# eth-cscs/conflux

Measured on NVIDIA H100. Metric: LU GFLOP/s (FP64, (2/3)N^3), higher is better.
Workload: dtype f64

## Files before the change

conflux_b200/__init__.py:

```python
import ctypes

import numpy as np

from ._lib import ConfluxError, LIB_PATH, SYMBOLS, ShareLayout, check, lib

__all__ = ["pinned_empty", "pinned_free", "Comm", "lu_params", "LU_rep", "LU_rep_fixed", "rbt_multipliers", "LU_rep_rbt", "lu_rbt_solve", "lu_rbt_apply_local", "residual", "validate", "lu_solve", "lu_rcond", "lu_refine", "lu_refine_x", "lu_equilibrate", "lu_svx", "lu_equilibrate_b", "lu_svxx", "lu_inverse", "lu_det", "rhs_local_cols", "lu_solve_local", "timeline", "auto_grid", "lu_dims", "init_matrix_host", "ConfluxError", "dbg", "cholesky", "chol_dims", "chol_auto_grid"]


def auto_grid(M, N, P):
    px, py, pz = ctypes.c_int(), ctypes.c_int(), ctypes.c_int()
    check(lib().cflx_auto_grid(int(M), int(N), int(P), ctypes.byref(px), ctypes.byref(py), ctypes.byref(pz)), "auto_grid")
    return px.value, py.value, pz.value


def lu_dims(M, N, v, Px, Py, Pz):
    o = (ctypes.c_int * 8)()
    check(lib().cflx_lu_dims(int(M), int(N), int(v), int(Px), int(Py), int(Pz), o), "lu_dims")
    return dict(M=o[0], N=o[1], Ml=o[2], Nl=o[3], Nt=o[4], nlayr=o[5], Mt=o[6], P=o[7])


def init_matrix_host(M, N, v, Px, Py, Pz, rank, seed=42, out=None):
    d = lu_dims(M, N, v, Px, Py, Pz)
    if out is None:
        out = np.empty((d["Ml"], d["Nl"]), dtype=np.float64)
# ... 540 lines not shown
            self.finalize()
        except Exception:
            pass


def chol_dims(N, v, Px, Py, Pz):
    o = (ctypes.c_int * 6)()
    check(lib().cflx_chol_dims(int(N), int(v), int(Px), int(Py), int(Pz), o), "chol_dims")
    return dict(N=o[0], Kappa=o[1], Ml=o[2], Nl=o[3], l=o[4], P=o[5])


def chol_auto_grid(P, N):
    g = (ctypes.c_int * 3)()
    check(lib().cflx_chol_auto_grid(int(P), int(N), g), "chol_auto_grid")
    return tuple(g)


def _ptr(a):
    return a.ctypes.data if a is not None else None


def _tiles(n, v):
    return int(n) // max(int(v), 1)


def _share(v, Ml, Nl, grid=(1, 1), pos=(0, 0), Kappa=None, M=None):
    Px, Py = (int(x) for x in grid)
    M = int(M) if M is not None else _tiles(Ml, v) * Px * int(v)
    return ShareLayout(M, int(v), int(Kappa if Kappa is not None else 1 << 30), int(Ml), int(Nl), Px, Py, int(pos[0]),
                       int(pos[1]))


class dbg:

    @staticmethod
    def gemm_tn(AT, B, C=None, alpha=1.0, beta=0.0, reps=1):
        AT = np.asarray(AT, dtype=np.float64)
        B = np.asarray(B, dtype=np.float64)
        K, M = AT.shape
        N = B.shape[1]
        M2, N2 = M + (M & 1), N + (N & 1)
        ATp = np.zeros((K, M2))
        ATp[:, :M] = AT
        Bp = np.zeros((K, N2))
        Bp[:, :N] = B
        Cp = np.zeros((M, N2))
        if C is not None:
            Cp[:, :N] = C
        D, _, ms = dbg.gemm_tn_window(ATp, Bp, Cp, M, N2, K, alpha, beta, in_place=False, reps=reps)
        return D[:, :N], ms

    @staticmethod
    def gemm_tn_window(AT, B, C, M, N, K, alpha=1.0, beta=0.0, at_off=(0, 0), b_off=(0, 0), c_off=(0, 0), in_place=True,
                       reps=1):
        AT = np.ascontiguousarray(AT, dtype=np.float64)
        B = np.ascontiguousarray(B, dtype=np.float64)
        C = np.ascontiguousarray(C, dtype=np.float64)
        D = np.empty_like(C)
        Cout = D if in_place else np.empty_like(C)
        ms = ctypes.c_double()
        check(lib().cflx_dbg_gemm_tn(int(M), int(N), int(K), AT.ctypes.data, AT.shape[0], AT.shape[1],
                                     at_off[0] * AT.shape[1] + at_off[1], B.ctypes.data, B.shape[0], B.shape[1],
                                     b_off[0] * B.shape[1] + b_off[1], C.ctypes.data, C.shape[0], C.shape[1],
                                     int(c_off[0]), int(c_off[1]), float(alpha), float(beta), 1 if in_place else 0,
                                     D.ctypes.data, Cout.ctypes.data, int(reps), ctypes.byref(ms)), "dbg_gemm_tn")
        return D, Cout, ms.value

    @staticmethod
    def gemm_narrow(A, B, C=None, alpha=1.0, beta=0.0, reps=1, out=None):
        A = np.ascontiguousarray(A, dtype=np.float64)
        B = np.ascontiguousarray(B, dtype=np.float64)
        M, K = A.shape
        N = B.shape[1]
        Cp = None
        if C is not None:
            assert C.dtype == np.float64 and C.flags.c_contiguous and C.shape == (M, N)
            Cp = C.ctypes.data
        D = np.empty((M, N)) if out is None else out
        assert D.dtype == np.float64 and D.flags.c_contiguous and D.shape == (M, N)
        ms = ctypes.c_double()
        check(lib().cflx_dbg_gemm_narrow(M, N, K, A.ctypes.data, B.ctypes.data, Cp, float(alpha), float(beta), D.ctypes.data,
                                         int(reps), ctypes.byref(ms)), "dbg_gemm_narrow")
        return D, ms.value

    @staticmethod
    def gemm_narrow_tn(AT, B, C=None, alpha=1.0, beta=0.0, reps=1, out=None):
        AT = np.ascontiguousarray(AT, dtype=np.float64)
        B = np.ascontiguousarray(B, dtype=np.float64)
        K, M = AT.shape
        if B.ndim != 2 or B.shape[0] != K:
            raise ValueError(f"gemm_narrow_tn: B must have {K} rows, got shape {B.shape}")
        N = B.shape[1]
        Cp = None
        if C is not None:
            assert C.dtype == np.float64 and C.flags.c_contiguous and C.shape == (M, N)
            Cp = C.ctypes.data
        D = np.empty((M, N)) if out is None else out
        assert D.dtype == np.float64 and D.flags.c_contiguous and D.shape == (M, N)
        ms = ctypes.c_double()
        check(lib().cflx_dbg_gemm_narrow_tn(M, N, K, AT.ctypes.data, B.ctypes.data, Cp, float(alpha), float(beta),
                                            D.ctypes.data, int(reps), ctypes.byref(ms)), "dbg_gemm_narrow_tn")
        return D, ms.value

    @staticmethod
    def gemm_narrow_window(A, B, C, M, N, K, alpha=1.0, beta=0.0, a_off=(0, 0), b_off=(0, 0), c_off=(0, 0), trans=False,
                           in_place=True):
        A = np.ascontiguousarray(A, dtype=np.float64)
        B = np.ascontiguousarray(B, dtype=np.float64)
        C = np.ascontiguousarray(C, dtype=np.float64)
        D = np.empty_like(C)
        Cout = D if in_place else np.empty_like(C)
        check(lib().cflx_dbg_gemm_narrow_window(
            1 if trans else 0, int(M), int(N), int(K), A.ctypes.data, A.shape[0], A.shape[1], int(a_off[0]),
            int(a_off[1]), B.ctypes.data, B.shape[0], B.shape[1], int(b_off[0]), int(b_off[1]), C.ctypes.data,
            C.shape[0], C.shape[1], int(c_off[0]), int(c_off[1]), float(alpha), float(beta), 1 if in_place else 0,
            D.ctypes.data, Cout.ctypes.data), "dbg_gemm_narrow_window")
        return D, Cout
# ... 250 lines not shown
              "dbg_potrf_tile")
        return L, LT, info.value

    @staticmethod
    def ldlt_tile(A, tiny=0.0, variant=0):
        A = np.ascontiguousarray(A, dtype=np.float64)
        v = A.shape[0]
        R, SRT, sg = np.empty((v, v)), np.empty((v, v)), np.empty(v)
        nrepl, info = ctypes.c_int(), ctypes.c_int()
        inertia = (ctypes.c_int * 3)()
        check(lib().cflx_dbg_ldlt_tile(v, A.ctypes.data, float(tiny), R.ctypes.data, SRT.ctypes.data, sg.ctypes.data,
                                       ctypes.byref(nrepl), inertia, ctypes.byref(info), int(variant)), "dbg_ldlt_tile")
        return dict(R=R, SRT=SRT, s=sg, nrepl=nrepl.value, inertia=tuple(inertia), info=info.value)

    @staticmethod
    def solve_signs(Z, sgn, v, grid=(1, 1), pos=(0, 0), M=None):
        Z = np.array(Z, dtype=np.float64, order="C")
        sg = np.ascontiguousarray(sgn, dtype=np.float64)
        Nl, ldn = Z.shape
        lay = _share(v, v, Nl, grid, pos, M=M if M is not None else len(sg))
        check(lib().cflx_dbg_solve_signs(ctypes.byref(lay), int(ldn), sg.ctypes.data, Z.ctypes.data), "dbg_solve_signs")
        return Z

    @staticmethod
    def getrf_nopiv_tile(A, tiny=0.0, variant=0):
        A = np.ascontiguousarray(A, dtype=np.float64)
        v = A.shape[0]
        LU = np.empty((v, v))
        nrepl, info = ctypes.c_int(), ctypes.c_int()
        check(lib().cflx_dbg_getrf_nopiv_tile(v, A.ctypes.data, float(tiny), LU.ctypes.data, ctypes.byref(nrepl),
                                              ctypes.byref(info), int(variant)), "dbg_getrf_nopiv_tile")
        return LU, nrepl.value, info.value

    @staticmethod
    def ozaki_gemm(AT, B, C=None, reps=1, want_planes=False, row0=0, col0=0, max_ctas=0):
        AT = np.ascontiguousarray(AT, dtype=np.float64)
        B = np.ascontiguousarray(B, dtype=np.float64)
        K, Ma = AT.shape
        Nb = B.shape[1]
        M, N = Ma - row0, Nb - col0
        D = np.empty((M, N))
        Cp = np.ascontiguousarray(C, dtype=np.float64) if C is not None else None
        pa = np.zeros((8, Ma, K), dtype=np.int8) if want_planes else None
        pb = np.zeros((8, Nb, K), dtype=np.int8) if want_planes else None
        ea = np.zeros(Ma, dtype=np.int32) if want_planes else None
        eb = np.zeros(Nb, dtype=np.int32) if want_planes else None
        ms, sms = ctypes.c_double(), ctypes.c_double()
        check(lib().cflx_dbg_ozaki_gemm(M, N, K, int(row0), int(col0), int(max_ctas), AT.ctypes.data, B.ctypes.data,
                                        _ptr(Cp), D.ctypes.data, _ptr(pa), _ptr(pb), _ptr(ea), _ptr(eb), int(reps),
                                        ctypes.byref(ms), ctypes.byref(sms)), "dbg_ozaki_gemm")
        return dict(D=D, ms=ms.value, split_ms=sms.value, pa=pa, pb=pb, ea=ea, eb=eb)

    @staticmethod
    def push_pivots(A, pivot_rows, fnpr):
        A = np.array(A, dtype=np.float64, order="C")
        piv = np.ascontiguousarray(pivot_rows, dtype=np.int32)
        gri = np.zeros(A.shape[0], dtype=np.int32)
        a01 = np.zeros((max(1, len(piv)), A.shape[1]))
        check(lib().cflx_dbg_push_pivots(A.shape[0], A.shape[1], A.ctypes.data, len(piv), piv.ctypes.data, int(fnpr),
                                         gri.ctypes.data, a01.ctypes.data), "dbg_push_pivots")
        return A, gri, a01[:len(piv)]

    @staticmethod
    def wgmma_peak(n):
        t = ctypes.c_double()
        check(lib().cflx_dbg_wgmma_peak(int(n), ctypes.byref(t)), "dbg_wgmma_peak")
        return t.value

    @staticmethod
    def fp64_peak_ex(which):
        a, b = ctypes.c_double(), ctypes.c_double()
        check(lib().cflx_dbg_fp64_peak_ex(int(which), ctypes.byref(a), ctypes.byref(b)), "dbg_fp64_peak_ex")
        return a.value, b.value

    @staticmethod
    def fp64_peak(which):
        tf = ctypes.c_double()
        check(lib().cflx_dbg_fp64_peak(int(which), ctypes.byref(tf)), "dbg_fp64_peak")
        return tf.value
```

conflux_b200/_lib.py:

```python
import ctypes
import os

_HERE = os.path.dirname(os.path.abspath(__file__))
LIB_PATH = os.path.join(_HERE, "libconflux_b200.so")
_lib = None

c_double_p = ctypes.POINTER(ctypes.c_double)
c_int_p = ctypes.POINTER(ctypes.c_int)


class ConfluxError(RuntimeError):
    pass


class ShareLayout(ctypes.Structure):
    _fields_ = [(f, ctypes.c_int) for f in ("M", "v", "Kappa", "Ml", "Nl", "Px", "Py", "pi", "pj")]


SYMBOLS = [
    "cflx_last_error", "cflx_version", "cflx_device_count", "cflx_get_unique_id", "cflx_comm_create",
    "cflx_comm_barrier", "cflx_comm_destroy", "cflx_host_alloc", "cflx_host_free", "cflx_auto_grid", "cflx_lu_dims", "cflx_init_matrix_host",
    "cflx_lu_create", "cflx_lu_info", "cflx_lu_set_local", "cflx_lu_queue_next_local", "cflx_lu_factor", "cflx_lu_factor_fixed", "cflx_rbt_multipliers", "cflx_lu_rbt", "cflx_lu_rbt_solve", "cflx_lu_rbt_apply_local", "cflx_lu_get_factors",
    "cflx_lu_get_permutation", "cflx_lu_residual", "cflx_lu_validate", "cflx_lu_solve", "cflx_lu_solve_trans", "cflx_rhs_local_cols", "cflx_lu_solve_local", "cflx_lu_rcond", "cflx_lu_refine", "cflx_lu_refine_x", "cflx_lu_equilibrate", "cflx_lu_svx", "cflx_lu_equilibrate_b", "cflx_lu_svxx", "cflx_lu_inverse", "cflx_lu_det", "cflx_lu_launch_count", "cflx_lu_uses_ozaki", "cflx_lu_set_profiling", "cflx_lu_phase_ms", "cflx_lu_timeline",
    "cflx_lu_set_kernel_timing", "cflx_lu_trailing_stats", "cflx_lu_destroy", "cflx_chol_auto_grid", "cflx_chol_auto_tile", "cflx_chol_dims", "cflx_chol_init_matrix_host",
    "cflx_chol_create", "cflx_chol_info", "cflx_chol_set_local", "cflx_chol_factor", "cflx_chol_factor_ldlt", "cflx_chol_rbt", "cflx_chol_rbt_solve", "cflx_chol_rbt_apply_local", "cflx_chol_get_signs", "cflx_chol_get_input", "cflx_chol_get_local", "cflx_chol_validate",
    "cflx_chol_solve", "cflx_chol_solve_local", "cflx_chol_rcond", "cflx_chol_refine", "cflx_chol_refine_x", "cflx_chol_equilibrate", "cflx_chol_svx", "cflx_chol_equilibrate_b", "cflx_chol_svxx", "cflx_chol_inverse", "cflx_chol_det", "cflx_chol_launch_count", "cflx_chol_destroy", "cflx_dbg_gemm_tn", "cflx_dbg_gemm_narrow", "cflx_dbg_gemm_narrow_tn", "cflx_dbg_gemm_narrow_window", "cflx_dbg_diag_solve", "cflx_dbg_residual", "cflx_dbg_residual_x", "cflx_dbg_equil", "cflx_dbg_growth_cols", "cflx_dbg_inverse_share", "cflx_dbg_solve_local_share", "cflx_dbg_norm_share", "cflx_dbg_rbt_share", "cflx_dbg_chol_validate_share", "cflx_dbg_lu_validate_share", "cflx_dbg_chol_gather_cols", "cflx_dbg_refine_assemble", "cflx_dbg_refine_columns", "cflx_dbg_det", "cflx_dbg_panel", "cflx_dbg_trsm", "cflx_dbg_diag_inverse", "cflx_dbg_potrf_tile", "cflx_dbg_ldlt_tile", "cflx_dbg_solve_signs", "cflx_dbg_getrf_nopiv_tile", "cflx_dbg_push_pivots", "cflx_dbg_ozaki_gemm", "cflx_dbg_wgmma_peak", "cflx_dbg_fp64_peak", "cflx_dbg_fp64_peak_ex",
]


def _preload_nccl():
    import sys
    for d in sys.path:
        cand = os.path.join(d, "nvidia", "nccl", "lib", "libnccl.so.2")
        if os.path.exists(cand):
            try:
                ctypes.CDLL(cand, mode=ctypes.RTLD_GLOBAL)
                return cand
            except OSError:
                pass
    return None


def lib():
    global _lib
    if _lib is None:
        if not os.path.exists(LIB_PATH):
            raise ConfluxError(
                f"{LIB_PATH} is missing: build it with `python -c 'import __graft_entry__ as g; g.build()'` "
                "(conflux_b200 has no CPU fallback)")
        _preload_nccl()
        L = ctypes.CDLL(LIB_PATH)
        L.cflx_last_error.restype = ctypes.c_char_p
        L.cflx_version.restype = ctypes.c_char_p
        L.cflx_comm_destroy.restype = None
        L.cflx_lu_destroy.restype = None
        L.cflx_comm_destroy.argtypes = [ctypes.c_void_p]
        L.cflx_lu_destroy.argtypes = [ctypes.c_void_p]
        L.cflx_comm_barrier.argtypes = [ctypes.c_void_p]
        L.cflx_comm_create.argtypes = [ctypes.c_int, ctypes.c_int, ctypes.c_void_p, ctypes.c_int,
                                       ctypes.POINTER(ctypes.c_void_p)]
        L.cflx_lu_create.argtypes = [ctypes.c_void_p] + [ctypes.c_int] * 6 + [ctypes.POINTER(ctypes.c_void_p)]
        L.cflx_host_alloc.argtypes = [ctypes.c_size_t, ctypes.POINTER(ctypes.c_void_p)]
        L.cflx_host_free.argtypes = [ctypes.c_void_p]
        L.cflx_lu_info.argtypes = [ctypes.c_void_p, c_int_p]
        L.cflx_lu_set_local.argtypes = [ctypes.c_void_p, ctypes.c_void_p]
        L.cflx_lu_queue_next_local.argtypes = [ctypes.c_void_p, ctypes.c_void_p]
        L.cflx_lu_factor.argtypes = [ctypes.c_void_p, c_double_p]
        L.cflx_lu_factor_fixed.argtypes = [ctypes.c_void_p, ctypes.c_void_p, ctypes.c_double] + [ctypes.c_void_p] * 3
        L.cflx_rbt_multipliers.argtypes = [ctypes.c_int, ctypes.c_int, ctypes.c_uint64, ctypes.c_void_p, ctypes.c_void_p]
        L.cflx_lu_rbt.argtypes = [ctypes.c_void_p, ctypes.c_int, ctypes.c_uint64, ctypes.c_void_p, ctypes.c_void_p]
        L.cflx_lu_rbt_solve.argtypes = [ctypes.c_void_p, ctypes.c_int, ctypes.c_int, ctypes.c_void_p, ctypes.c_int,
                                        ctypes.c_void_p, ctypes.c_int, ctypes.c_int, ctypes.c_void_p, ctypes.c_void_p]
        L.cflx_lu_rbt_apply_local.argtypes = [ctypes.c_void_p, ctypes.c_int, ctypes.c_int, ctypes.c_void_p, ctypes.c_int]
        L.cflx_lu_get_factors.argtypes = [ctypes.c_void_p, ctypes.c_void_p, ctypes.c_void_p]
        L.cflx_lu_get_permutation.argtypes = [ctypes.c_void_p, ctypes.c_void_p]
        L.cflx_lu_residual.argtypes = [ctypes.c_void_p, c_double_p]
        L.cflx_lu_validate.argtypes = [ctypes.c_void_p, c_double_p, c_double_p]
        L.cflx_lu_solve.argtypes = [ctypes.c_void_p, ctypes.c_int, ctypes.c_void_p, ctypes.c_int, ctypes.c_void_p, ctypes.c_int]
        L.cflx_lu_solve_trans.argtypes = [ctypes.c_void_p, ctypes.c_int, ctypes.c_void_p, ctypes.c_int, ctypes.c_void_p,
# ... 10 lines not shown
        L.cflx_lu_svx.argtypes = [ctypes.c_void_p, ctypes.c_int, ctypes.c_int, ctypes.c_void_p, ctypes.c_int, ctypes.c_void_p,
                                  ctypes.c_int] + [ctypes.c_void_p] * 6
        L.cflx_lu_equilibrate_b.argtypes = [ctypes.c_void_p, ctypes.c_int] + [ctypes.c_void_p] * 7
        L.cflx_lu_svxx.argtypes = [ctypes.c_void_p, ctypes.c_int, ctypes.c_int, ctypes.c_void_p, ctypes.c_int,
                                   ctypes.c_void_p, ctypes.c_int] + [ctypes.c_void_p] * 7
        L.cflx_lu_inverse.argtypes = [ctypes.c_void_p, ctypes.c_void_p, c_int_p]
        L.cflx_lu_det.argtypes = [ctypes.c_void_p, ctypes.c_int] + [ctypes.c_void_p] * 5
        L.cflx_lu_uses_ozaki.argtypes = [ctypes.c_void_p]
        L.cflx_lu_launch_count.argtypes = [ctypes.c_void_p, ctypes.POINTER(ctypes.c_int64), ctypes.c_int]
        L.cflx_lu_set_profiling.argtypes = [ctypes.c_void_p, ctypes.c_int]
        L.cflx_lu_phase_ms.argtypes = [ctypes.c_void_p, c_double_p]
        L.cflx_lu_timeline.argtypes = [ctypes.c_void_p, ctypes.c_char_p, ctypes.c_int]
        L.cflx_lu_set_kernel_timing.argtypes = [ctypes.c_void_p, ctypes.c_int]
        L.cflx_lu_trailing_stats.argtypes = [ctypes.c_void_p, c_double_p, c_double_p]
        L.cflx_chol_destroy.restype = None
        L.cflx_chol_destroy.argtypes = [ctypes.c_void_p]
        L.cflx_chol_auto_grid.argtypes = [ctypes.c_int, ctypes.c_int, c_int_p]
        L.cflx_chol_auto_tile.argtypes = [ctypes.c_int] * 3
        L.cflx_chol_dims.argtypes = [ctypes.c_int] * 5 + [c_int_p]
        L.cflx_chol_init_matrix_host.argtypes = [ctypes.c_int] * 6 + [ctypes.c_void_p]
        L.cflx_chol_create.argtypes = [ctypes.c_void_p] + [ctypes.c_int] * 5 + [ctypes.POINTER(ctypes.c_void_p)]
        L.cflx_chol_info.argtypes = [ctypes.c_void_p, c_int_p]
        L.cflx_chol_set_local.argtypes = [ctypes.c_void_p, ctypes.c_void_p]
        L.cflx_chol_factor.argtypes = [ctypes.c_void_p, c_double_p]
        L.cflx_chol_factor_ldlt.argtypes = [ctypes.c_void_p, ctypes.c_double] + [ctypes.c_void_p] * 4
        L.cflx_chol_rbt.argtypes = [ctypes.c_void_p, ctypes.c_int, ctypes.c_uint64, ctypes.c_void_p]
        L.cflx_chol_rbt_solve.argtypes = [ctypes.c_void_p, ctypes.c_int, ctypes.c_void_p, ctypes.c_int, ctypes.c_void_p,
                                          ctypes.c_int, ctypes.c_int, ctypes.c_void_p, ctypes.c_void_p]
        L.cflx_chol_rbt_apply_local.argtypes = [ctypes.c_void_p, ctypes.c_int, ctypes.c_int, ctypes.c_void_p, ctypes.c_int]
        L.cflx_chol_get_signs.argtypes = [ctypes.c_void_p, ctypes.c_void_p]
        L.cflx_chol_get_input.argtypes = [ctypes.c_void_p, ctypes.c_void_p]
        L.cflx_chol_get_local.argtypes = [ctypes.c_void_p, ctypes.c_void_p]
        L.cflx_chol_validate.argtypes = [ctypes.c_void_p, c_double_p, c_double_p]
        L.cflx_chol_solve.argtypes = [ctypes.c_void_p, ctypes.c_int, ctypes.c_void_p, ctypes.c_int, ctypes.c_void_p, ctypes.c_int]
        L.cflx_chol_solve_local.argtypes = [ctypes.c_void_p, ctypes.c_int, ctypes.c_void_p, ctypes.c_int, ctypes.c_void_p,
                                            ctypes.c_int]
        L.cflx_chol_rcond.argtypes = [ctypes.c_void_p, c_double_p, c_double_p]
        L.cflx_chol_refine.argtypes = [ctypes.c_void_p, ctypes.c_int, ctypes.c_void_p, ctypes.c_int, ctypes.c_void_p, ctypes.c_int,
                                       ctypes.c_void_p, ctypes.c_void_p]
        L.cflx_chol_refine_x.argtypes = [ctypes.c_void_p, ctypes.c_int, ctypes.c_void_p, ctypes.c_int, ctypes.c_void_p,
                                         ctypes.c_int] + [ctypes.c_void_p] * 5
        L.cflx_chol_equilibrate.argtypes = [ctypes.c_void_p, ctypes.c_int] + [ctypes.c_void_p] * 5
        L.cflx_chol_svx.argtypes = [ctypes.c_void_p, ctypes.c_int, ctypes.c_void_p, ctypes.c_int, ctypes.c_void_p, ctypes.c_int
                                    ] + [ctypes.c_void_p] * 5
        L.cflx_chol_equilibrate_b.argtypes = [ctypes.c_void_p, ctypes.c_int] + [ctypes.c_void_p] * 5
        L.cflx_chol_svxx.argtypes = [ctypes.c_void_p, ctypes.c_int, ctypes.c_void_p, ctypes.c_int, ctypes.c_void_p,
                                     ctypes.c_int] + [ctypes.c_void_p] * 7
        L.cflx_chol_inverse.argtypes = [ctypes.c_void_p, ctypes.c_void_p]
        L.cflx_chol_det.argtypes = [ctypes.c_void_p, ctypes.c_int] + [ctypes.c_void_p] * 3
        L.cflx_chol_launch_count.argtypes = [ctypes.c_void_p, ctypes.POINTER(ctypes.c_int64), ctypes.c_int]
        L.cflx_init_matrix_host.argtypes = [ctypes.c_int] * 8 + [ctypes.c_void_p]
        _buf = [ctypes.c_void_p, ctypes.c_int, ctypes.c_int64]
        L.cflx_dbg_gemm_tn.argtypes = [ctypes.c_int] * 3 + _buf + [ctypes.c_int64] + _buf + [ctypes.c_int64] + _buf + [
            ctypes.c_int] * 2 + [ctypes.c_double] * 2 + [ctypes.c_int, ctypes.c_void_p, ctypes.c_void_p, ctypes.c_int,
                                                          c_double_p]
        L.cflx_dbg_gemm_narrow.argtypes = [ctypes.c_int] * 3 + [ctypes.c_void_p] * 3 + [ctypes.c_double] * 2 + [
            ctypes.c_void_p, ctypes.c_int, c_double_p]
        L.cflx_dbg_gemm_narrow_tn.argtypes = [ctypes.c_int] * 3 + [ctypes.c_void_p] * 3 + [ctypes.c_double] * 2 + [
            ctypes.c_void_p, ctypes.c_int, c_double_p]
        _blk = [ctypes.c_void_p, ctypes.c_int, ctypes.c_int64, ctypes.c_int, ctypes.c_int]
        L.cflx_dbg_gemm_narrow_window.argtypes = [ctypes.c_int] * 4 + _blk * 3 + [ctypes.c_double] * 2 + [
            ctypes.c_int, ctypes.c_void_p, ctypes.c_void_p]
        L.cflx_dbg_diag_solve.argtypes = [ctypes.c_int] * 4 + [ctypes.c_void_p, ctypes.c_int, ctypes.c_int64] + [
            ctypes.c_int] * 3 + [ctypes.c_void_p] * 3
        share = ctypes.POINTER(ShareLayout)
        L.cflx_dbg_residual.argtypes = [ctypes.c_int, share, ctypes.c_void_p, ctypes.c_int] + [ctypes.c_void_p] * 4 + [
            ctypes.c_int, c_double_p]
        L.cflx_dbg_residual_x.argtypes = [ctypes.c_int, share, ctypes.c_void_p, ctypes.c_int] + [
            ctypes.c_void_p] * 6 + [ctypes.c_int, c_double_p]
        L.cflx_dbg_equil.argtypes = [share] + [ctypes.c_void_p] * 3 + [ctypes.c_char, ctypes.c_int] + [
            ctypes.c_void_p] * 7
        L.cflx_dbg_growth_cols.argtypes = [ctypes.c_int, share, ctypes.c_int] + [ctypes.c_void_p] * 4
        L.cflx_dbg_inverse_share.argtypes = [ctypes.c_int, share] + [ctypes.c_int] * 3 + [
            ctypes.c_void_p, ctypes.c_int] + [ctypes.c_void_p] * 3 + [ctypes.c_int]
        L.cflx_dbg_solve_local_share.argtypes = [ctypes.c_int, share] + [ctypes.c_int] * 3 + [
            ctypes.c_void_p, ctypes.c_int] + [ctypes.c_void_p] * 3 + [ctypes.c_int]
        L.cflx_dbg_norm_share.argtypes = [ctypes.c_int, share] + [ctypes.c_void_p] * 2
        L.cflx_dbg_rbt_share.argtypes = [ctypes.c_int, share, ctypes.c_int] + [ctypes.c_void_p] * 2 + [
            ctypes.c_int, ctypes.c_void_p, ctypes.c_int]
        L.cflx_dbg_chol_validate_share.argtypes = [share, ctypes.c_void_p, ctypes.c_int] + [ctypes.c_void_p] * 2
        L.cflx_dbg_lu_validate_share.argtypes = [share, ctypes.c_void_p, ctypes.c_int] + [ctypes.c_void_p] * 2
        L.cflx_dbg_chol_gather_cols.argtypes = [share, ctypes.c_int] + [ctypes.c_void_p] * 2
        L.cflx_dbg_refine_assemble.argtypes = [ctypes.c_int] * 12 + [ctypes.c_void_p] * 6
        L.cflx_dbg_refine_columns.argtypes = [ctypes.c_int] * 3 + [ctypes.c_void_p] * 10
        L.cflx_dbg_det.argtypes = [ctypes.c_int] + [ctypes.c_void_p] * 3 + [ctypes.c_int] + [ctypes.c_void_p] * 5
        L.cflx_dbg_panel.argtypes = [ctypes.c_int, ctypes.c_int] + [ctypes.c_void_p] * 4 + [ctypes.c_int, c_double_p]
        L.cflx_dbg_trsm.argtypes = [ctypes.c_int] * 3 + [ctypes.c_int64] + [ctypes.c_void_p] * 5
        L.cflx_dbg_diag_inverse.argtypes = [ctypes.c_int, ctypes.c_int] + [ctypes.c_void_p] * 3
        L.cflx_dbg_potrf_tile.argtypes = [ctypes.c_int] + [ctypes.c_void_p] * 4 + [ctypes.c_int]
        L.cflx_dbg_solve_signs.argtypes = [share, ctypes.c_int, ctypes.c_void_p, ctypes.c_void_p]
        L.cflx_dbg_ldlt_tile.argtypes = ([ctypes.c_int, ctypes.c_void_p, ctypes.c_double] + [ctypes.c_void_p] * 6 +
                                         [ctypes.c_int])
        L.cflx_dbg_getrf_nopiv_tile.argtypes = [ctypes.c_int, ctypes.c_void_p, ctypes.c_double] + [ctypes.c_void_p] * 3 + [
            ctypes.c_int]
        L.cflx_dbg_push_pivots.argtypes = [ctypes.c_int, ctypes.c_int, ctypes.c_void_p, ctypes.c_int, ctypes.c_void_p, ctypes.c_int,
                                           ctypes.c_void_p, ctypes.c_void_p]
        L.cflx_dbg_ozaki_gemm.argtypes = [ctypes.c_int] * 6 + [ctypes.c_void_p] * 8 + [ctypes.c_int, c_double_p, c_double_p]
        L.cflx_dbg_wgmma_peak.argtypes = [ctypes.c_int, c_double_p]
        L.cflx_dbg_fp64_peak.argtypes = [ctypes.c_int, c_double_p]
        L.cflx_dbg_fp64_peak_ex.argtypes = [ctypes.c_int, c_double_p, c_double_p]
        _lib = L
    return _lib


def check(rc, what=""):
    if rc != 0:
        msg = lib().cflx_last_error().decode(errors="replace")
        raise ConfluxError(f"{what} failed with status {rc}: {msg}")
```

conflux_b200/csrc/chol.cu:

```cuda
#include <climits>
#include <cmath>
#include <cstdlib>
#include <cstring>
#include <numeric>

#include "lu_state.h"

using namespace cflx;

struct cflx_chol : Handle {
    DevBuf<double> PT, LT, G , Bc , D, A00, W, Uinv, LinvT, acc;
    DevBuf<double> Q;
    DevBuf<int> info;
    int64_t ldp = 0, ldb = 0;
    bool ldlt = false;
    double tiny = 0.0;
    DevBuf<double> sgn;
    Events<2> ev_col, ev_panel;
    SubComm j_comm;
    ~cflx_chol();
};

namespace {

// ... 352 lines not shown
                                      (size_t)v * sizeof(double), cudaMemcpyDeviceToDevice, s));
    } else {
        CFLX_CUDA(cudaMemcpyAsync(G, ch->LT, (size_t)v * piece_ld(ch, gfirst, 0) * sizeof(double), cudaMemcpyDeviceToDevice, s));
    }
    const int lj0 = first_local_tile(jmin, ch->pj, Py);
    const int ntc = Nl / v - lj0;
    if (ntc <= 0) return CFLX_OK;
    CFLX_TRY(launch_gather_cols(G, piece_stride, Bc, ch->ldb, v, Px, Py, ch->pj, lj0, ntc, gfirst, Ml, s,
                                ch->ldlt ? ch->sgn + (int64_t)t * v : nullptr));
    ch->launches++;
    return CFLX_OK;
}
static int chol_leave_sms() {
    static int leave = -1;
    if (leave < 0) {
        const char* e = getenv("CFLX_CHOL_LEAVE");
        leave = e ? atoi(e) : 8;
        if (leave < 0) leave = 0;
        if (leave > 100) leave = 100;
    }
    return leave;
}

int update_columns(cflx_chol* ch, int gfirst, int jmin, int buf, double* X, int lj_lo, int lj_hi, cudaStream_t s, int planes_buf = -1) {
    const int v = ch->v, Px = ch->Px, Py = ch->Py, Ml = ch->Ml, Nl = ch->Nl;
    const int pi = ch->pi, pj = ch->pj, pk = ch->pk;
    const int64_t piece_stride = (int64_t)v * ch->ldp;
    const double* G = ch->G + (int64_t)buf * Px * piece_stride;
    const double* Bc = ch->Bc + (int64_t)buf * v * ch->ldb;
    const int lj0 = first_local_tile(jmin, pj, Py);
    const int my_first = first_local_tile(gfirst, pi, Px);
    const int64_t ldg = piece_ld(ch, gfirst, pi);
    const int lj_end = std::min(lj_hi, Nl / v);
    const int my_rows = Ml - my_first * v;
    for (int lj = std::max(lj_lo, lj0); lj < lj_end;) {
        const int j = lj * Py + pj;
        const int li = first_local_tile(j, pi, Px);
        const int M = Ml - li * v;
        if (M <= 0) break;
        int gcols = std::max(1, (8192 + M - 1) / M);
        gcols = std::min(gcols, lj_end - lj);
        GemmArgs g{};
        g.M = M; g.N = gcols * v; g.K = ch->nlayr;
        g.AT = G + (int64_t)pi * piece_stride + (int64_t)pk * ch->nlayr * ldg + (int64_t)(li - my_first) * v;
        g.ldat = ldg;
        g.B = Bc + (int64_t)pk * ch->nlayr * ch->ldb + (int64_t)(lj - lj0) * v;
        g.ldb = ch->ldb;
        g.C = X + (int64_t)li * v * Nl + (int64_t)lj * v;
        g.ldc = Nl;
        g.D = const_cast<double*>(g.C);
        g.ldd = Nl;
        g.alpha = -1.0; g.beta = 1.0;
        if (ch->use_ozaki && planes_buf == buf)
            CFLX_TRY(launch_ozaki_gemm(&ch->oz, M, g.N, (li - my_first) * v, (lj - lj0) * v, g.D, Nl, ch->oz.sms - chol_leave_sms(), s));
        else
            CFLX_TRY(launch_gemm_tn(g, s));
        ch->launches++;
        lj += gcols;
    }
    (void)my_rows;
    return CFLX_OK;
}
int split_planes(cflx_chol* ch, int gfirst, int jmin, int buf, cudaStream_t s);
int split_planes(cflx_chol* ch, int gfirst, int jmin, int buf, cudaStream_t s) {
    if (!ch->use_ozaki) return CFLX_OK;
    const int v = ch->v, Px = ch->Px;
    const int64_t piece_stride = (int64_t)v * ch->ldp;
    const double* G = ch->G + (int64_t)buf * Px * piece_stride;
    const double* Bc = ch->Bc + (int64_t)buf * v * ch->ldb;
    const int my_first = first_local_tile(gfirst, ch->pi, Px);
    const int rows = ch->Ml - my_first * v;
    const int ncols = ch->Nl - first_local_tile(jmin, ch->pj, ch->Py) * v;
    const int64_t ldg = piece_ld(ch, gfirst, ch->pi);
    if (rows > 0) CFLX_TRY(ozaki_split_a(&ch->oz, G + (int64_t)ch->pi * piece_stride + (int64_t)ch->pk * ch->nlayr * ldg, ldg, rows, s));
    if (ncols > 0) CFLX_TRY(ozaki_split_b(&ch->oz, Bc + (int64_t)ch->pk * ch->nlayr * ch->ldb, ch->ldb, 0, ncols, s));
    ch->launches += 2;
    return CFLX_OK;
}
int broadcast_and_update(cflx_chol* ch, int t, int jmin, bool below_only, double* X, cudaStream_t s) {
    const int gfirst = below_only ? t + 1 : t;
    CFLX_TRY(broadcast_pieces(ch, t, gfirst, jmin, 0, s));
    return update_columns(ch, gfirst, jmin, 0, X, 0, ch->Nl / ch->v, s);
}

size_t potrf_tile_smem(int v) { return ((size_t)PB * (PB + 1) + (size_t)v * (PB + 1)) * sizeof(double); }
}

namespace cflx {
size_t potrf_tile_scratch(int v) { return (v % QBK == 0 && v >= 2 * QBK) ? (size_t)3 * QBK * QBK + (size_t)2 * QBK * v : 0; }

int potrf_setup(int v) {
    static PerDeviceMax tile_cfg, blk_cfg;
    CFLX_CUDA(tile_cfg.raise(potrf_tile_smem(v), [&] {
        cudaError_t e = cudaFuncSetAttribute(potrf_tile_kernel<false>, cudaFuncAttributeMaxDynamicSharedMemorySize, (int)potrf_tile_smem(v));
        if (e == cudaSuccess)
            e = cudaFuncSetAttribute(potrf_tile_kernel<true>, cudaFuncAttributeMaxDynamicSharedMemorySize, (int)potrf_tile_smem(v));
        return e;
    }));
    CFLX_CUDA(blk_cfg.raise(QBK * QPITCH * sizeof(double), [&] {
        cudaError_t e = cudaFuncSetAttribute(potrf128_kernel<false>, cudaFuncAttributeMaxDynamicSharedMemorySize, (int)(QBK * QPITCH * sizeof(double)));
        if (e == cudaSuccess)
            e = cudaFuncSetAttribute(potrf128_kernel<true>, cudaFuncAttributeMaxDynamicSharedMemorySize, (int)(QBK * QPITCH * sizeof(double)));
        return e;
    }));
    return CFLX_OK;
}

// ... 796 lines not shown
```

conflux_b200/csrc/dbg.cu:

```cuda
#include <algorithm>
#include <climits>
#include <limits>
#include <vector>

#include "../../include/conflux_b200.h"
#include "common.cuh"
#include "kernels.h"
#include "lu_state.h"

using namespace cflx;

namespace {
int check_device() {
    int n = 0;
    if (cudaGetDeviceCount(&n) != cudaSuccess || n == 0) {
        cudaGetLastError();
        set_last_error("no CUDA device visible: conflux_b200 has no CPU fallback");
        return CFLX_ERR_NO_DEVICE;
    }
    return CFLX_OK;
}

enum : unsigned { TILED = 1, COVERED = 2, NONEMPTY = 4 };

// ... 136 lines not shown

int cflx_dbg_fp64_peak_ex(int which, double* burst_out, double* sustained_out) {
    CFLX_TRY(check_device());
    if (which == 0) which = 3;
    if (which < 1 || which > 5) {
        set_last_error("fp64_peak: unknown probe %d", which);
        return CFLX_ERR_ARG;
    }
    int dev = 0, sms = 0;
    CFLX_CUDA(cudaGetDevice(&dev));
    CFLX_CUDA(cudaDeviceGetAttribute(&sms, cudaDevAttrMultiProcessorCount, dev));
    const int threads = 256, blocks = sms * 4;
    DevBuf<> out;
    CFLX_TRY(out.alloc(sizeof(double) * threads * blocks));
    Events<2> ev;
    CFLX_TRY(ev.create());
    const double per_warp_instr = which == 2 ? 1024.0 : which == 3 ? 2048.0 : which == 4 ? 4096.0 : 512.0;
    const int shrink = which == 1 ? 1 : (int)(per_warp_instr / 512.0);
    auto run = [&](int iters, double* tf) -> int {
        iters /= shrink;
        CFLX_CUDA(cudaEventRecord(ev[0]));
        switch (which) {
            case 1: dfma_peak_kernel<<<blocks, threads>>>(out.as<double>(), iters); break;
            case 2: dmma16x8_peak_kernel<4><<<blocks, threads>>>(out.as<double>(), iters); break;
            case 3: dmma16x8_peak_kernel<8><<<blocks, threads>>>(out.as<double>(), iters); break;
            case 4: dmma16x8_peak_kernel<16><<<blocks, threads>>>(out.as<double>(), iters); break;
            default: dmma_peak_kernel<<<blocks, threads>>>(out.as<double>(), iters); break;
        }
        CFLX_CUDA(cudaGetLastError());
        CFLX_CUDA(cudaEventRecord(ev[1]));
        CFLX_CUDA(cudaEventSynchronize(ev[1]));
        float ms = 0;
        CFLX_CUDA(cudaEventElapsedTime(&ms, ev[0], ev[1]));
        const double flop = which == 1 ? (double)blocks * threads * iters * 16 * 2.0
                                       : (double)blocks * (threads / 32) * iters * 16 * per_warp_instr;
        *tf = flop / (ms * 1e-3) / 1e12;
        return CFLX_OK;
    };
    double burst = 0, tf = 0;
    for (int rep = 0; rep < 4; ++rep) {
        CFLX_TRY(run(1024, &tf));
        if (rep > 0 && tf > burst) burst = tf;
    }
    double sustained = 0;
    CFLX_TRY(run(262144, &sustained));
    if (burst_out) *burst_out = burst;
    if (sustained_out) *sustained_out = sustained;
    return CFLX_OK;
}
int cflx_dbg_fp64_peak(int which, double* tflops_out) { return cflx_dbg_fp64_peak_ex(which, tflops_out, nullptr); }

int cflx_dbg_gemm_tn(int M, int N, int K, const double* AT, int at_rows, int64_t ldat, int64_t at_off, const double* B,
                     int b_rows, int64_t ldb, int64_t b_off, const double* C, int c_rows, int64_t ldc, int row_off,
                     int col_off, double alpha, double beta, int in_place, double* D_out, double* C_out, int reps,
                     double* ms_out) {
    CFLX_TRY(check_device());
    REFUSE_IF(M <= 0 || N <= 0 || K <= 0);
    REFUSE_IF(!AT || !B || !C);
    REFUSE_IF(at_rows <= 0 || b_rows <= 0 || c_rows <= 0 || ldat <= 0 || ldb <= 0 || ldc <= 0);
    REFUSE_IF(at_off < 0 || b_off < 0 || row_off < 0 || col_off < 0);
    if ((at_off & 1) || (b_off & 1) || (col_off & 1) || at_off + (K - 1) * ldat + round_up(M, 2) > (int64_t)at_rows * ldat ||
        b_off + (K - 1) * ldb + N > (int64_t)b_rows * ldb || row_off + M > c_rows || col_off + N > ldc)
        return refuse(__func__, "window outside the buffers or misaligned");
    const size_t a_n = (size_t)at_rows * ldat, b_n = (size_t)b_rows * ldb, c_n = (size_t)c_rows * ldc;
    DevBuf<> dA, dB, dC, dC0, dD;
    CFLX_TRY(stage(dA, a_n, AT));
    CFLX_TRY(stage(dB, b_n, B));
    CFLX_TRY(stage(dC, c_n));
    CFLX_TRY(stage(dC0, c_n, C));
    CFLX_TRY(stage(dD, c_n));
    auto restore = [&]() -> int {
        CFLX_CUDA(cudaMemcpy(dC.p, dC0.p, sizeof(double) * c_n, cudaMemcpyDeviceToDevice));
        CFLX_CUDA(cudaMemcpy(dD.p, dC0.p, sizeof(double) * c_n, cudaMemcpyDeviceToDevice));
        return CFLX_OK;
    };
    const int64_t c_at = (int64_t)row_off * ldc + col_off;
    GemmArgs g{};
    g.M = M; g.N = N; g.K = K;
    g.AT = dA.as<double>() + at_off; g.ldat = ldat;
    g.B = dB.as<double>() + b_off; g.ldb = ldb;
    g.C = dC.as<double>() + c_at; g.ldc = ldc;
    g.D = (in_place ? dC.as<double>() : dD.as<double>()) + c_at; g.ldd = ldc;
    g.alpha = alpha; g.beta = beta;
    CFLX_TRY(restore());
    CFLX_TRY(time_reps([&] { return launch_gemm_tn(g, 0); }, reps, ms_out));
    CFLX_TRY(restore());
    CFLX_TRY(launch_gemm_tn(g, 0));
    CFLX_TRY(fetch(D_out, in_place ? dC.p : dD.p, c_n));
    CFLX_TRY(fetch(C_out, dC.p, c_n));
    CFLX_CUDA(cudaDeviceSynchronize());
    return CFLX_OK;
}

int cflx_dbg_gemm_narrow(int M, int N, int K, const double* A, const double* B, const double* C, double alpha, double beta,
                         double* D, int reps, double* ms_out) {
    CFLX_TRY(check_device());
    REFUSE_IF(M <= 0 || N <= 0 || K < 0);
    REFUSE_IF(K & 3);
    REFUSE_IF(!A || !B);
    DevBuf<> dA, dB;
    CFLX_TRY(stage(dA, (size_t)M * K, A));
    CFLX_TRY(stage(dB, (size_t)K * N, B));
    return narrow_gemm((size_t)M * N, C, D, reps, ms_out, [&](const double* c, double* out) {
        return launch_gemm_narrow(M, N, K, dA.as<double>(), K, dB.as<double>(), N, c, N, out, N, alpha, beta, 0);
    });
}

int cflx_dbg_gemm_narrow_tn(int M, int N, int K, const double* AT, const double* B, const double* C, double alpha,
                            double beta, double* D, int reps, double* ms_out) {
    CFLX_TRY(check_device());
    REFUSE_IF(M <= 0 || N <= 0 || K < 0);
    REFUSE_IF(!AT || !B);
    const int64_t ldat = round_up(M, 2);
    DevBuf<> dA, dB;
    CFLX_TRY(stage(dA, K * ldat));
    CFLX_TRY(stage(dB, (size_t)K * N, B));
    if (K > 0) CFLX_CUDA(cudaMemcpy2D(dA.p, ldat * 8, AT, (size_t)M * 8, (size_t)M * 8, K, cudaMemcpyHostToDevice));
    return narrow_gemm((size_t)M * N, C, D, reps, ms_out, [&](const double* c, double* out) {
        return launch_gemm_narrow_tn(M, N, K, dA.as<double>(), ldat, dB.as<double>(), N, c, N, out, N, alpha, beta, 0);
    });
}

int cflx_dbg_gemm_narrow_window(int trans, int M, int N, int K, const double* A, int a_rows, int64_t lda, int a_row,
                                int a_col, const double* B, int b_rows, int64_t ldb, int b_row, int b_col, const double* C,
                                int c_rows, int64_t ldc, int c_row, int c_col, double alpha, double beta, int in_place,
                                double* D_out, double* C_out) {
    CFLX_TRY(check_device());
    const char* who = __func__;
    if (M < 1 || N < 1 || K < 0) return refuse(who, "M < 1, N < 1 or K < 0");
    if (!A || !B || !C) return refuse(who, "A, B or C is null");
    if (a_rows < 1 || b_rows < 1 || c_rows < 1 || lda < 1 || ldb < 1 || ldc < 1)
        return refuse(who, "a buffer with no rows or a leading dimension < 1");
    if (a_row < 0 || a_col < 0 || b_row < 0 || b_col < 0 || c_row < 0 || c_col < 0) return refuse(who, "negative offset");
    if (!trans && (K & 3)) return refuse(who, "K not a multiple of 4");
// ... 687 lines not shown
    CFLX_CUDA(cudaDeviceSynchronize());
    if (nrepl_out) *nrepl_out = cnt[0];
    if (inertia_out)
        for (int i = 0; i < 3; ++i) inertia_out[i] = cnt[1 + i];
    return CFLX_OK;
}

int cflx_dbg_getrf_nopiv_tile(int v, const double* A, double tiny, double* LU_out, int* nrepl_out, int* info_out,
                              int variant) {
    CFLX_TRY(check_device());
    REFUSE_IF(!A || !LU_out || !info_out);
    REFUSE_IF(variant != 0 && variant != 1);
    REFUSE_IF(v < 4 || v > 1024 || v % 4 != 0);
    REFUSE_IF(variant == 1 && !getrf_nopiv_blocked(v));
    REFUSE_IF(!(tiny >= 0.0));
    const size_t vv = (size_t)v * v;
    std::vector<double> At(vv);
    for (int i = 0; i < v; ++i)
        for (int c = 0; c < v; ++c) At[(size_t)c * v + i] = A[(size_t)i * v + c];
    DevBuf<> dB, dA, drec, dws;
    CFLX_TRY(stage(dB, vv, At.data()));
    CFLX_TRY(stage(dA, vv));
    CFLX_TRY(stage<int>(drec, 4));
    const size_t ws = getrf_nopiv_scratch(v, variant == 1);
    if (ws) CFLX_TRY(stage(dws, ws));
    CFLX_CUDA(cudaMemset(drec.p, 0, 4 * sizeof(int)));
    if (variant == 1) CFLX_TRY(gemm_tn_setup());
    int64_t launches = 0;
    CFLX_TRY(launch_getrf_nopiv_tile(dB.as<double>(), v, tiny, dA.as<double>(), nullptr, nullptr, nullptr, drec.as<int>(),
                                     0, variant == 1, ws ? dws.as<double>() : nullptr, 0, &launches));
    int rec[4];
    CFLX_TRY(fetch(LU_out, dA.p, vv));
    CFLX_TRY(fetch(rec, drec.p, 4));
    CFLX_CUDA(cudaDeviceSynchronize());
    if (nrepl_out) *nrepl_out = rec[0];
    *info_out = rec[1];
    return CFLX_OK;
}

int cflx_dbg_push_pivots(int n_rows, int n_cols, double* A_inout, int npiv, const int* pivot_rows, int fnpr, int* gri_out,
                         double* a01_out) {
    CFLX_TRY(check_device());
    REFUSE_IF(n_rows <= 0 || n_cols <= 0 || (n_cols & 1));
    REFUSE_IF(npiv < 0 || fnpr < 0 || npiv > n_rows - fnpr);
    if (npiv == 0) {
        if (gri_out) for (int i = 0; i < n_rows; ++i) gri_out[i] = i;
        return CFLX_OK;
    }
    REFUSE_IF(!A_inout || !pivot_rows);
    const int v = npiv;
    const size_t a_n = (size_t)n_rows * n_cols;
    DevBuf<> dA, dtmp, da01, dplan, dgp, dgri, dgrit, digri;
    CFLX_TRY(stage(dA, a_n, A_inout));
    CFLX_TRY(stage(dtmp, (size_t)v * n_cols));
    CFLX_TRY(stage(da01, (size_t)v * n_cols));
    CFLX_TRY(stage<int>(dplan, 6 * (size_t)v + 8 + n_rows));
    CFLX_TRY(stage(dgp, v, pivot_rows));
    CFLX_TRY(stage<int>(dgri, n_rows));
    CFLX_TRY(stage<int>(dgrit, n_rows));
    CFLX_TRY(stage<int>(digri, n_rows));
    MovePlan plan{};
    int* pm = dplan.as<int>();
    plan.npiv = pm; plan.nel = pm + 4; pm += 8;
    plan.cur_piv = pm; pm += v;
    plan.order = pm; pm += v;
    plan.slot2piv = pm; pm += v;
    plan.early = pm; pm += v;
    plan.late = pm; pm += 2 * v;
    plan.rowsrc = pm;
    CFLX_TRY(launch_iota_gri(dgri.as<int>(), digri.as<int>(), n_rows, n_rows, 1, 0, 0));
    CFLX_TRY(launch_plan_moves(dgp.as<int>(), v, 1, 0, fnpr, n_rows, digri.as<int>(), plan, 0));
    CFLX_TRY(launch_push_phase1(dA.as<double>(), n_cols, n_cols, 0, plan, v, dtmp.as<double>(), da01.as<double>(), n_cols, 0, 0));
    CFLX_TRY(launch_push_phase2(dA.as<double>(), n_cols, n_cols, 0, plan, v, 0));
    CFLX_TRY(launch_push_phase3(dA.as<double>(), n_cols, n_cols, 0, fnpr, plan, v, dtmp.as<double>(), 0));
    CFLX_TRY(launch_update_gri(dgri.as<int>(), dgrit.as<int>(), digri.as<int>(), plan.rowsrc, fnpr, n_rows, n_rows, 1, 0));
    CFLX_TRY(fetch(A_inout, dA.p, a_n));
    CFLX_TRY(fetch(gri_out, dgri.p, n_rows));
    CFLX_TRY(fetch(a01_out, da01.p, (size_t)v * n_cols));
    CFLX_CUDA(cudaDeviceSynchronize());
    return CFLX_OK;
}

int cflx_dbg_ozaki_gemm(int M, int N, int K, int row0, int col0, int max_ctas, const double* AT, const double* B,
                        const double* C, double* D, signed char* planesA_out, signed char* planesB_out, int* ea_out,
                        int* eb_out, int reps, double* ms_out, double* split_ms_out) {
    CFLX_TRY(check_device());
    REFUSE_IF(M <= 0 || N <= 0 || K <= 0 || (N & 1));
    REFUSE_IF(row0 < 0 || col0 < 0 || max_ctas < 0);
    REFUSE_IF(!AT || !B);
    const int Ma = row0 + M, Nb = col0 + N;
    const int64_t ldat = round_up(Ma, 2), ldb = Nb, ldc = N;
    const size_t c_n = (size_t)M * ldc;
    DevBuf<> dA, dB, dC, dC0;
    CFLX_TRY(stage(dA, K * ldat));
    CFLX_TRY(stage(dB, K * ldb, B));
    CFLX_TRY(stage(dC, c_n));
    CFLX_TRY(stage(dC0, c_n, C));
    CFLX_CUDA(cudaMemset(dA.p, 0, sizeof(double) * K * ldat));
    CFLX_CUDA(cudaMemcpy2D(dA.p, ldat * 8, AT, (size_t)Ma * 8, (size_t)Ma * 8, K, cudaMemcpyHostToDevice));
    if (!C) CFLX_CUDA(cudaMemset(dC0.p, 0, sizeof(double) * c_n));
    Events<3> ev;
    CFLX_TRY(ev.create());
    OzakiWorkspace ws;
    int rc = ozaki_workspace_create(&ws, Ma, Nb, K);
    if (reps < 1) reps = 1;
    float ms = 0, ms_split = 0;
    for (int r = 0; r < reps + 1 && rc == CFLX_OK; ++r) {
        cudaMemcpyAsync(dC.p, dC0.p, sizeof(double) * c_n, cudaMemcpyDeviceToDevice, 0);
        cudaEventRecord(ev[0]);
        rc = ozaki_split_a(&ws, dA.as<double>(), ldat, Ma, 0);
        if (!rc && col0 > 0) rc = ozaki_split_b(&ws, dB.as<double>(), ldb, 0, col0, 0);
        if (!rc) rc = ozaki_split_b(&ws, dB.as<double>(), ldb, col0, N, 0);
        cudaEventRecord(ev[1]);
        if (!rc) rc = launch_ozaki_gemm(&ws, M, N, row0, col0, dC.as<double>(), ldc, max_ctas, 0);
        cudaEventRecord(ev[2]);
        if (cudaEventSynchronize(ev[2]) != cudaSuccess) {
            set_last_error("ozaki kernel failed: %s", cudaGetErrorString(cudaGetLastError()));
            rc = CFLX_ERR_CUDA;
        }
        float a = 0, b = 0;
        cudaEventElapsedTime(&a, ev[0], ev[1]);
        cudaEventElapsedTime(&b, ev[1], ev[2]);
        if (r > 0) {
            ms_split += a;
            ms += b;
        }
    }
    if (rc == CFLX_OK) rc = fetch(D, dC.p, c_n);
    for (int s = 0; s < 8 && rc == CFLX_OK; ++s) {
        if (planesA_out) rc = fetch(planesA_out + (size_t)s * Ma * K, ws.planesA + (size_t)s * ws.cap_a * K, (size_t)Ma * K);
        if (planesB_out && rc == CFLX_OK)
            rc = fetch(planesB_out + (size_t)s * Nb * K, ws.planesB + (size_t)s * ws.cap_b * K, (size_t)Nb * K);
    }
    if (rc == CFLX_OK) rc = fetch(ea_out, ws.ea, Ma);
    if (rc == CFLX_OK) rc = fetch(eb_out, ws.eb, Nb);
    if (rc == CFLX_OK && cudaDeviceSynchronize() != cudaSuccess) rc = CFLX_ERR_CUDA;
    if (ms_out) *ms_out = ms / reps;
    if (split_ms_out) *split_ms_out = ms_split / reps;
    return rc;
}

int cflx_dbg_wgmma_peak(int n, double* tmacs_out) {
    CFLX_TRY(check_device());
    REFUSE_IF(!tmacs_out);
    return wgmma_peak_probe(n, tmacs_out);
}

}
```

conflux_b200/csrc/gemm.cu:

```cuda
#include <cstdlib>

#include "common.cuh"
#include "kernels.h"

namespace cflx {

namespace {
constexpr int BK = 16, STAGES = 4;

template <int WM, int WN>
struct Cfg {
    static constexpr int BM = 64 * WM, BN = 32 * WN;
    static constexpr int LDA = BM + 4, LDB = BN + 4;
    static constexpr int NCONS = WM * WN, NTHREADS = (NCONS + 1) * 32;
    static constexpr bool STAGE_C = (WM == 2);
    static constexpr int NBAR = 2 * STAGES + (STAGE_C ? WM * STAGES : 0);
    static constexpr size_t SMEM = (size_t)STAGES * BK * (LDA + LDB) * sizeof(double) + NBAR * sizeof(uint64_t);
    static_assert(!STAGE_C || (LDA == LDB && 64 / 16 == STAGES), "one slab per warp row and stage, in both parts");
};

__device__ __forceinline__ double2 ld_c2(const double* p) {
    double2 v;
    asm("ld.global.v2.f64 {%0, %1}, [%2];" : "=d"(v.x), "=d"(v.y) : "l"(p));
    return v;
}

template <int LDA, int LDB, int SA, int SB>
__device__ __forceinline__ void load_operands(const GemmArgs& g, int kt0, int kt1, int m0, int n0, int wm, int wn,
                                              double* a_ring, double* b_ring, uint64_t* full, uint64_t* empty, int lane) {
    const int rr = lane & 15;
    for (int kt = kt0; kt < kt1; ++kt) {
        const int s = kt % STAGES, u = kt / STAGES;
        if (u > 0) mbar_wait(&empty[s], (u - 1) & 1);
        const int rows = min(BK, g.K - kt * BK);
        if (lane == 0) mbar_arrive_expect_tx(&full[s], (uint32_t)(rows * (wm + wn) * sizeof(double)));
        __syncwarp();
        if (rr < rows) {
            const int64_t k = (int64_t)kt * BK + rr;
            if (lane < 16)
                bulk_g2s(a_ring + s * SA + rr * LDA, g.AT + k * g.ldat + m0, (uint32_t)(wm * sizeof(double)), &full[s]);
            else
                bulk_g2s(b_ring + s * SB + rr * LDB, g.B + k * g.ldb + n0, (uint32_t)(wn * sizeof(double)), &full[s]);
        }
    }
}

template <int MI, int LDA, int LDB, int SA, int SB>
__device__ __forceinline__ int mma_loop(const GemmArgs& g, double (&acc)[MI][4][4], const double* a_ring,
                                        const double* b_ring, uint64_t* full, uint64_t* empty, int wm_off, int wn_off,
                                        int lane) {
    const int g4 = lane >> 2, t4 = lane & 3;
#pragma unroll
    for (int i = 0; i < MI; ++i)
#pragma unroll
        for (int j = 0; j < 4; ++j) acc[i][j][0] = acc[i][j][1] = acc[i][j][2] = acc[i][j][3] = 0.0;

    int kt = 0;
    for (; kt * BK < g.K; ++kt) {
        const int s = kt % STAGES, u = kt / STAGES;
        mbar_wait(&full[s], u & 1);
        const double* a_s = a_ring + s * SA + wm_off + g4;
        const double* b_s = b_ring + s * SB + wn_off + g4;
        const int rows = min(BK, g.K - kt * BK);
#pragma unroll
        for (int kk = 0; kk < BK; kk += 8) {
            if (kk < rows) {
                const bool hi = kk + 4 < rows;
                const double* a_k = a_s + (kk + t4) * LDA;
                const double* b_k = b_s + (kk + t4) * LDB;
                double b[4][2];
#pragma unroll
                for (int j = 0; j < 4; ++j) {
                    b[j][0] = b_k[8 * j];
                    b[j][1] = hi ? b_k[4 * LDB + 8 * j] : 0.0;
                }
#pragma unroll
                for (int i = 0; i < MI; ++i) {
                    const double a[4] = {a_k[16 * i], a_k[16 * i + 8], hi ? a_k[4 * LDA + 16 * i] : 0.0,
                                         hi ? a_k[4 * LDA + 16 * i + 8] : 0.0};
#pragma unroll
                    for (int j = 0; j < 4; ++j) dmma16x8x8(acc[i][j], a, b[j]);
                }
            }
        }
        __syncwarp();
        if (lane == 0) mbar_arrive(&empty[s]);
    }
    return kt;
}

template <int WM, int WN, int MINB>
__global__ void __launch_bounds__(Cfg<WM, WN>::NTHREADS, MINB) gemm_tn_kernel(GemmArgs g) {
    using C = Cfg<WM, WN>;
    constexpr int BM = C::BM, BN = C::BN, LDA = C::LDA, LDB = C::LDB, NCONS = C::NCONS;
    extern __shared__ __align__(128) unsigned char smem_raw[];
    double* sA = reinterpret_cast<double*>(smem_raw);
    double* sB = sA + STAGES * BK * LDA;
    uint64_t* full = reinterpret_cast<uint64_t*>(sB + STAGES * BK * LDB);
    uint64_t* empty = full + STAGES;
    uint64_t* cfull = empty + STAGES;

    const int warp = threadIdx.x >> 5, lane = threadIdx.x & 31;
    const int m0 = blockIdx.y * BM, n0 = blockIdx.x * BN;

    if (threadIdx.x == 0) {
        for (int s = 0; s < STAGES; ++s) {
            mbar_init(&full[s], 1);
            mbar_init(&empty[s], NCONS);
        }
        if constexpr (C::STAGE_C)
            for (int b = 0; b < WM * STAGES; ++b) mbar_init(&cfull[b], 1);
        fence_barrier_init();
    }
    __syncthreads();

    if (warp == NCONS) {
        int wm = g.M - m0;
        wm = wm > BM ? BM : ((wm + 1) & ~1);
        int wn = g.N - n0;
        wn = wn > BN ? BN : ((wn + 1) & ~1);
        const int rr = lane & 15;
        const int nkt = (g.K + BK - 1) / BK;
        const bool use_c = (g.beta != 0.0);
        for (int kt = 0; kt < nkt; ++kt) {
            const int s = kt % STAGES, u = kt / STAGES;
            if (u > 0) mbar_wait(&empty[s], (u - 1) & 1);
            const int rows = min(BK, g.K - kt * BK);
            if (lane == 0) mbar_arrive_expect_tx(&full[s], (uint32_t)(rows * (wm + wn) * sizeof(double)));
            __syncwarp();
            if (rr < rows) {
                const int64_t k = (int64_t)kt * BK + rr;
                if (lane < 16)
                    bulk_g2s(sA + (s * BK + rr) * LDA, g.AT + k * g.ldat + m0, (uint32_t)(wm * sizeof(double)), &full[s]);
                else
                    bulk_g2s(sB + (s * BK + rr) * LDB, g.B + k * g.ldb + n0, (uint32_t)(wn * sizeof(double)), &full[s]);
            }
        }
        if constexpr (C::STAGE_C) {
            if (use_c)
                for (int i = 0; i < STAGES; ++i) {
                    const int s = (nkt + i) % STAGES, kt = nkt + i - STAGES;
                    if (kt >= 0) mbar_wait(&empty[s], (kt / STAGES) & 1);
                    const int wr = lane >> 4, r0 = m0 + 64 * wr + 16 * i;
                    const int rows = max(0, min(16, g.M - r0));
                    uint64_t* bar = &cfull[wr * STAGES + i];
                    if (rr == 0) mbar_arrive_expect_tx(bar, (uint32_t)(rows * wn * sizeof(double)));
                    __syncwarp();
                    if (rr < rows)
                        bulk_g2s(sA + (wr * STAGES + s) * BK * LDA + rr * LDA + 4 * (rr & 1),
                                 g.C + (int64_t)(r0 + rr) * g.ldc + n0, (uint32_t)(wn * sizeof(double)), bar);
                }
        }
        return;
    }

    const int wm_off = (warp / WN) * 64, wn_off = (warp % WN) * 32;
    const int g4 = lane >> 2, t4 = lane & 3;
    double acc[4][4][4];
#pragma unroll
    for (int i = 0; i < 4; ++i)
#pragma unroll
        for (int j = 0; j < 4; ++j) acc[i][j][0] = acc[i][j][1] = acc[i][j][2] = acc[i][j][3] = 0.0;

    int kt = 0;
    for (; kt * BK < g.K; ++kt) {
        const int s = kt % STAGES, u = kt / STAGES;
        mbar_wait(&full[s], u & 1);
        const double* a_s = sA + s * BK * LDA + wm_off + g4;
        const double* b_s = sB + s * BK * LDB + wn_off + g4;
        const int rows = min(BK, g.K - kt * BK);
#pragma unroll
        for (int kk = 0; kk < BK; kk += 8) {
            if (kk < rows) {
                const bool hi = kk + 4 < rows;
                const double* a_k = a_s + (kk + t4) * LDA;
                const double* b_k = b_s + (kk + t4) * LDB;
                double b[4][2];
#pragma unroll
                for (int j = 0; j < 4; ++j) {
                    b[j][0] = b_k[8 * j];
                    b[j][1] = hi ? b_k[4 * LDB + 8 * j] : 0.0;
                }
#pragma unroll
                for (int i = 0; i < 4; ++i) {
                    const double a[4] = {a_k[16 * i], a_k[16 * i + 8], hi ? a_k[4 * LDA + 16 * i] : 0.0,
                                         hi ? a_k[4 * LDA + 16 * i + 8] : 0.0};
#pragma unroll
                    for (int j = 0; j < 4; ++j) dmma16x8x8(acc[i][j], a, b[j]);
                }
            }
        }
        __syncwarp();
        if (lane == 0) mbar_arrive(&empty[s]);
    }

    const double alpha = g.alpha, beta = g.beta;
    const bool use_c = (beta != 0.0);
    const int row0 = m0 + wm_off + g4, col0 = n0 + wn_off + 2 * t4;
    if constexpr (C::STAGE_C) {
        const int wr = warp / WN, nkt = kt;
#pragma unroll
        for (int i = 0; i < 4; ++i) {
            const double* cs = sA + (wr * STAGES + (nkt + i) % STAGES) * BK * LDA + 4 * (g4 & 1) + wn_off + 2 * t4;
            if (use_c) mbar_wait(&cfull[wr * STAGES + i], 0);
#pragma unroll
            for (int h = 0; h < 2; ++h) {
                const int row = row0 + 16 * i + 8 * h;
#pragma unroll
                for (int j = 0; j < 4; ++j) {
                    const int col = col0 + 8 * j;
                    if (row < g.M && col < g.N) {
                        double2 cv = make_double2(0.0, 0.0);
                        if (use_c) cv = *reinterpret_cast<const double2*>(cs + (g4 + 8 * h) * LDA + 8 * j);
                        double2 out;
                        out.x = fma(alpha, acc[i][j][2 * h], beta * cv.x);
                        out.y = fma(alpha, acc[i][j][2 * h + 1], beta * cv.y);
                        *reinterpret_cast<double2*>(g.D + (int64_t)row * g.ldd + col) = out;
                    }
                }
            }
        }
    } else {
#pragma unroll
        for (int sl = 0; sl < 8; ++sl) {
            const int row = row0 + 8 * sl;
            double2 cv[4];
#pragma unroll
            for (int j = 0; j < 4; ++j) {
                const int col = col0 + 8 * j;
                cv[j] = make_double2(0.0, 0.0);
                if (use_c && row < g.M && col < g.N) cv[j] = ld_c2(g.C + (int64_t)row * g.ldc + col);
            }
#pragma unroll
            for (int j = 0; j < 4; ++j) {
                const int col = col0 + 8 * j;
                if (row < g.M && col < g.N) {
                    double2 out;
                    out.x = fma(alpha, acc[sl / 2][j][2 * (sl & 1)], beta * cv[j].x);
                    out.y = fma(alpha, acc[sl / 2][j][2 * (sl & 1) + 1], beta * cv[j].y);
                    *reinterpret_cast<double2*>(g.D + (int64_t)row * g.ldd + col) = out;
                }
            }
        }
    }
}

struct Wide {
    static constexpr int WM = 2, WN = 4, MI = 6;
    static constexpr int BM = 16 * MI * WM, BN = 32 * WN;
    static constexpr int LDA = BM + 4, LDB = BN + 4, LDC = BN + 4;
    static constexpr int NPROD = 4, NCONS = WM * WN, NTHREADS = (NPROD + NCONS) * 32;
    static constexpr int PROD_REGS = 24, CONS_REGS = 240, LAUNCH_REGS = 65536 / NTHREADS / 8 * 8;
    static constexpr int NSLAB = BM / 16, SLAB = 16 * LDC, STAGE = BK * (LDA + LDB);
    static constexpr int NBAR = 2 * STAGES + NSLAB;
    static constexpr int SMEM_MAX = 227 * 1024;
    static constexpr int RING_OFF = (SMEM_MAX - NBAR * 8 - STAGES * STAGE * 8) / 128 * 128;
    static constexpr int BAR_OFF = RING_OFF + STAGES * STAGE * 8;
    static constexpr int SMEM = BAR_OFF + NBAR * 8;
    __host__ __device__ static constexpr uint32_t slab_stages(int j) {
        uint32_t m = 0;
        for (int s = 0; s < STAGES; ++s) {
            const int lo = RING_OFF + s * STAGE * 8, hi = lo + STAGE * 8;
            if (j * SLAB * 8 < hi && (j + 1) * SLAB * 8 > lo) m |= 1u << s;
        }
        return m;
    }
    static_assert(LDA % 16 == 4 && LDB % 16 == 4 && LDC % 16 == 4, "conflict-free strides");
    static_assert(NPROD * 32 * PROD_REGS + NCONS * 32 * CONS_REGS <= NTHREADS * LAUNCH_REGS, "register rebalance");
    static_assert(NSLAB * SLAB * 8 <= BAR_OFF && SMEM <= SMEM_MAX, "C tile below the barriers");
};

template <int N>
__device__ __forceinline__ void setmaxnreg_dec() {
    asm volatile("setmaxnreg.dec.sync.aligned.u32 %0;" ::"n"(N));
}
template <int N>
__device__ __forceinline__ void setmaxnreg_inc() {
    asm volatile("setmaxnreg.inc.sync.aligned.u32 %0;" ::"n"(N));
}

__global__ void __launch_bounds__(Wide::NTHREADS, 1) gemm_tn_wide_kernel(GemmArgs g) {
    using W = Wide;
    extern __shared__ __align__(128) unsigned char smem_raw[];
    double* ctile = reinterpret_cast<double*>(smem_raw);
    double* ring = reinterpret_cast<double*>(smem_raw + W::RING_OFF);
    uint64_t* full = reinterpret_cast<uint64_t*>(smem_raw + W::BAR_OFF);
    uint64_t* empty = full + STAGES;
    uint64_t* cfull = empty + STAGES;

    const int warp = threadIdx.x >> 5, lane = threadIdx.x & 31;
    const int m0 = blockIdx.y * W::BM, n0 = blockIdx.x * W::BN;

    if (threadIdx.x == 0) {
        for (int s = 0; s < STAGES; ++s) {
            mbar_init(&full[s], 1);
            mbar_init(&empty[s], W::NCONS);
        }
        for (int j = 0; j < W::NSLAB; ++j) mbar_init(&cfull[j], 1);
        fence_barrier_init();
    }
    __syncthreads();

    if (warp < W::NPROD) {
        setmaxnreg_dec<W::PROD_REGS>();
        if (warp != 0) return;
        int wm = g.M - m0;
        wm = wm > W::BM ? W::BM : ((wm + 1) & ~1);
        int wn = g.N - n0;
        wn = wn > W::BN ? W::BN : ((wn + 1) & ~1);
        const int nkt = (g.K + BK - 1) / BK;
        double* b_ring = ring + BK * W::LDA;
        load_operands<W::LDA, W::LDB, W::STAGE, W::STAGE>(g, 0, min(nkt, STAGES), m0, n0, wm, wn, ring, b_ring, full,
                                                          empty, lane);
        if (g.beta == 0.0) {
            load_operands<W::LDA, W::LDB, W::STAGE, W::STAGE>(g, STAGES, nkt, m0, n0, wm, wn, ring, b_ring, full, empty,
                                                              lane);
            return;
        }
        uint32_t drained = ~0u << min(nkt, STAGES), issued = 0;
        auto issue_ready = [&] {
#pragma unroll 1
            for (int j = 0; j < W::NSLAB; ++j) {
                if (((issued >> j) & 1) || (W::slab_stages(j) & ~drained)) continue;
                issued |= 1u << j;
                const int r0 = m0 + 16 * j, rows = max(0, min(16, g.M - r0));
                if (lane == 0) mbar_arrive_expect_tx(&cfull[j], (uint32_t)(rows * wn * sizeof(double)));
                __syncwarp();
                if (lane < rows)
                    bulk_g2s(ctile + j * W::SLAB + lane * W::LDC + 4 * (lane & 1), g.C + (int64_t)(r0 + lane) * g.ldc + n0,
                             (uint32_t)(wn * sizeof(double)), &cfull[j]);
            }
        };
        issue_ready();
        load_operands<W::LDA, W::LDB, W::STAGE, W::STAGE>(g, STAGES, nkt, m0, n0, wm, wn, ring, b_ring, full, empty,
                                                          lane);
        for (int kt = max(nkt - STAGES, 0); kt < nkt; ++kt) {
            mbar_wait(&empty[kt % STAGES], (kt / STAGES) & 1);
            drained |= 1u << (kt % STAGES);
            issue_ready();
        }
        return;
    }

    setmaxnreg_inc<W::CONS_REGS>();
    const int cw = warp - W::NPROD, wr = cw / W::WN;
    const int wm_off = wr * 16 * W::MI, wn_off = (cw % W::WN) * 32;
    const int g4 = lane >> 2, t4 = lane & 3;
    double acc[W::MI][4][4];
    mma_loop<W::MI, W::LDA, W::LDB, W::STAGE, W::STAGE>(g, acc, ring, ring + BK * W::LDA, full, empty, wm_off, wn_off,
                                                        lane);

    const double alpha = g.alpha, beta = g.beta;
    const bool use_c = (beta != 0.0);
    const int row0 = m0 + wm_off + g4, col0 = n0 + wn_off + 2 * t4;
#pragma unroll
    for (int i = 0; i < W::MI; ++i) {
        const int j = wr * W::MI + i;
        const double* cs = ctile + j * W::SLAB + 4 * (g4 & 1) + wn_off + 2 * t4;
        if (use_c) mbar_wait(&cfull[j], 0);
#pragma unroll
        for (int h = 0; h < 2; ++h) {
            const int row = row0 + 16 * i + 8 * h;
#pragma unroll
            for (int jj = 0; jj < 4; ++jj) {
                const int col = col0 + 8 * jj;
                if (row < g.M && col < g.N) {
                    double2 cv = make_double2(0.0, 0.0);
                    if (use_c) cv = *reinterpret_cast<const double2*>(cs + (g4 + 8 * h) * W::LDC + 8 * jj);
                    double2 out;
                    out.x = fma(alpha, acc[i][jj][2 * h], beta * cv.x);
                    out.y = fma(alpha, acc[i][jj][2 * h + 1], beta * cv.y);
                    *reinterpret_cast<double2*>(g.D + (int64_t)row * g.ldd + col) = out;
                }
            }
        }
    }
}
}

namespace {
template <int WM, int WN, int MINB>
int setup_one() {
// ... 71 lines not shown
```

conflux_b200/csrc/kernels.h:

```cpp
#pragma once
#include <cuda_runtime.h>

#include <cstdint>
#include <memory>

#include "common.cuh"

namespace cflx {

struct GemmArgs {
    int M, N, K;
    const double* AT;
    int64_t ldat;
    const double* B;
    int64_t ldb;
    const double* C;
    int64_t ldc;
    double* D;
    int64_t ldd;
    double alpha, beta;
};
int gemm_tn_setup();
int launch_gemm_tn(const GemmArgs& g, cudaStream_t stream);

struct OzakiWorkspace {
    struct Maps;
    DevBuf<int8_t> planesA;
    DevBuf<int8_t> planesB;
    DevBuf<int> ea;
    DevBuf<int> eb;
    std::unique_ptr<Maps> maps;
    int K = 0, cap_a = 0, cap_b = 0, sms = 0;
    OzakiWorkspace();
    ~OzakiWorkspace();
};
int ozaki_workspace_create(OzakiWorkspace* ws, int max_rows, int max_cols, int K);
int ozaki_split_a(OzakiWorkspace* ws, const double* LT, int64_t ld, int n, cudaStream_t s);
int ozaki_split_b(OzakiWorkspace* ws, const double* U, int64_t ld, int col0, int n, cudaStream_t s);
int wgmma_peak_probe(int n, double* tmacs_out);
int launch_ozaki_gemm(OzakiWorkspace* ws, int M, int N, int row0, int col0, double* C, int64_t ldc, int max_ctas, cudaStream_t s);

struct PanelWorkspace {
    DevBuf<uint2> slot_hdr;
    DevBuf<uint2> slot_rows;
    int epoch;
    int max_ctas;
    int cta_cap;
    DevBuf<unsigned> sk_flags;
    DevBuf<int> sk_ppos;
    DevBuf<unsigned> sk_ticket;
    unsigned sk_epoch, sk_ticket_count;
    int sk_enabled;
};
int panel_workspace_create(PanelWorkspace* ws);
int launch_panel_getrf(double* W, int64_t ldw, int n, int v, int* perm_out, PanelWorkspace* ws, cudaStream_t stream);
int launch_panel_getrf_a00(double* W, int64_t ldw, int n, int v, int* perm_out, double* A00, int* nb_used,
                           PanelWorkspace* ws, cudaStream_t stream);

int launch_extract_panel_T(const double* A, int64_t lda, int64_t row0, int64_t col0, int n, int v, double* PT,
                           int64_t ldp, cudaStream_t stream);
int launch_store_panel_T(double* A, int64_t lda, int64_t row0, int64_t col0, int n, int v, const double* LT,
                         int64_t ldp, cudaStream_t stream);
int launch_gather_winners(const double* PT, int64_t ldp, const int* tags, int n_valid, const int* perm, int v,
                          double* out_vals, int64_t ldo, int* out_tags, int dst0, cudaStream_t stream);
int launch_gather_a00(const double* W, int64_t ldw, const int* perm, int v, int nb, double* A00, double* A00T,
                      cudaStream_t stream);

struct MovePlan {
    int* npiv;
    int* cur_piv;
    int* order;
    int* slot2piv;
    int* early;
    int* late;
    int* nel;
    int* rowsrc;
};
int launch_plan_moves(const int* gpivots, int v, int Px, int pi, int fnpr, int Ml, const int* igri, MovePlan plan,
                      cudaStream_t stream);
int launch_push_phase1(const double* A, int64_t lda, int ncols, int col_lo, MovePlan plan, int v, double* tmp,
                       double* a01raw, int64_t ld01, int c0, cudaStream_t stream);
int launch_push_phase2(double* A, int64_t lda, int ncols, int col_lo, MovePlan plan, int v, cudaStream_t stream);
int launch_push_phase3(double* A, int64_t lda, int ncols, int col_lo, int fnpr, MovePlan plan, int v,
                       const double* tmp, cudaStream_t stream);
int launch_update_gri(int* gri, int* gri_tmp, int* igri, const int* rowsrc, int fnpr, int Ml, int v, int Px,
                      cudaStream_t stream);
int launch_compact_panel(const double* PT, int64_t ldp, double* PT2, int64_t ldp2, const int* rowsrc, int fnpr_old,
                         const int* npiv, int Ml, int v, cudaStream_t stream);
int launch_store_u_rows(double* A, int64_t lda, int fnpr_old, MovePlan plan, const double* U, int64_t ldu, int c0,
                        int ncols, int v, cudaStream_t stream);
int launch_store_diag(double* A, int64_t lda, int fnpr_old, MovePlan plan, const double* A00, int loff, int v,
                      cudaStream_t stream);
int launch_split_factors(const double* F, int64_t ldf, int n, double* LT, double* U, cudaStream_t stream);
int launch_gather_perm_rows(const double* A, int64_t lda, const int* perm, int n, double* out, cudaStream_t stream);
constexpr int SUMSQ_PARTIALS = 1184;
int launch_sumsq(const double* X, int64_t count, double* out, double* partials, cudaStream_t stream);
int launch_sum_partials(const double* partials, int n, double* out, cudaStream_t stream);
int launch_fill(double* p, int64_t n, double val, cudaStream_t stream);
int launch_iota_gri(int* gri, int* igri, int Ml, int v, int Px, int pi, cudaStream_t stream);
int launch_pack_bcast(const double* A00, const int* tags, int v, double* buf, cudaStream_t stream);
int launch_unpack_bcast(const double* buf, int v, double* A00, double* A00T, int* gpivots, cudaStream_t stream);
int launch_record_pivots(const int* gpivots, int v, int* hist, int k, cudaStream_t stream);

int launch_diag_inverses(const double* A00, int v, int nb, double* Uinv, double* LinvT, cudaStream_t stream);
int trsm_right_upper_T(const double* A00, const double* Uinv, int v, int nb, double* PT, double* LT, int64_t ld,
                       int n, cudaStream_t stream);
int trsm_left_lower_unit(const double* A00T, const double* LinvT, int v, int nb, double* R, double* U, int64_t ld,
                         int n, cudaStream_t stream);

size_t potrf_tile_scratch(int v);
int potrf_setup(int v);
struct LdltArgs {
    double tiny;
    double* sg;
    int* cnt;
};
int potrf_tile(double* D, double* UT, double* Q, int* info, int col0, int v, cudaStream_t stream, int64_t* launches,
               const LdltArgs* sa = nullptr);
int potrf_block128(double* D, int ldd, double* UT, int ldu, double* Uc, int* info, int col0, cudaStream_t stream,
                   const LdltArgs* sa = nullptr);

bool getrf_nopiv_blocked(int v);
size_t getrf_nopiv_scratch(int v, bool blocked);
int launch_getrf_nopiv_tile(const double* Bt, int v, double tiny, double* A, double* AT, const int* tags_in, int* tags_out,
                            int* rec, int col0, bool blocked, double* scratch, cudaStream_t stream, int64_t* launches);
int launch_fixed_locate(const int* rows, int v, int Px, int pi, int fnpr, int n_old, const int* igri, int* pos,
                        cudaStream_t stream);
int launch_fixed_info_operand(int* rec, cudaStream_t stream);

int launch_gather_rows(const double* A, int64_t lda, const int* src_rows, int nrows, int ncols, double* out,
                       cudaStream_t stream);

int launch_gemm_narrow(int M, int N, int K, const double* A, int64_t lda, const double* B, int64_t ldb, const double* C,
                       int64_t ldc, double* D, int64_t ldd, double alpha, double beta, cudaStream_t stream);
int launch_gemm_narrow_tn(int M, int N, int K, const double* AT, int64_t ldat, const double* B, int64_t ldb,
                          const double* C, int64_t ldc, double* D, int64_t ldd, double alpha, double beta,
// ... 6 lines not shown
```

conflux_b200/csrc/lu.cu:

```cuda
#include <algorithm>
#include <climits>
#include <cmath>
#include <cstdarg>
#include <cstdlib>
#include <cstring>
#include <random>
#include <string>
#include <vector>

#include <nvtx3/nvToolsExt.h>

#include "lu_state.h"

namespace cflx {
static thread_local char g_err[1024] = "";
void set_last_error(const char* fmt, ...) {
    va_list ap;
    va_start(ap, fmt);
    vsnprintf(g_err, sizeof(g_err), fmt, ap);
    va_end(ap);
}
}

using namespace cflx;
// ... 206 lines not shown
        CFLX_NCCL(ncclSend(st, v, ncclInt, ppi, lu->i_comm.c, s));
    }
    if (!self) {
        CFLX_NCCL(ncclRecv(recv, hv, ncclDouble, src, lu->i_comm.c, s));
        CFLX_NCCL(ncclRecv(recv_t, v, ncclInt, src, lu->i_comm.c, s));
    }
    CFLX_NCCL(ncclGroupEnd());
    return CFLX_OK;
}

__global__ void stack_kernel(const double* __restrict__ candH, const int* __restrict__ tagsH, int v, double* __restrict__ S,
                             double* __restrict__ W2, int* __restrict__ tagsS) {
    const int64_t e = (int64_t)blockIdx.x * blockDim.x + threadIdx.x;
    const int64_t tot = (int64_t)2 * v * v;
    if (e < tot) {
        const int c = (int)(e / (2 * v)), hi = (int)(e % (2 * v));
        const int h = hi / v, i = hi % v;
        const double x = candH[(size_t)h * v * v + (size_t)c * v + i];
        S[e] = x;
        W2[e] = x;
    }
    if (e < 2 * v) tagsS[e] = tagsH[e];
}

int fixed_panel(cflx_lu* lu, int k, int fnpr, int n_old, int64_t ldk, double* A00, double* A00T, cudaStream_t s) {
    const int v = lu->v, Px = lu->Px;
    const int* rows = lu->fix_perm + (size_t)k * v;
    {
        PhaseTimer t(lu, RG_step1_rowpermute, s);
        CFLX_TRY(launch_fixed_locate(rows, v, Px, lu->pi, fnpr, n_old, lu->igri, lu->perm, s));
        CFLX_TRY(launch_gather_winners(lu->PT, ldk, lu->gri + fnpr, n_old, lu->perm, v, lu->candH, v, lu->tagsS, 0, s));
        lu->launches += 2;
    }
    if (Px > 1) {
        PhaseTimer t(lu, RG_step1_pivoting, s);
        CFLX_NCCL(ncclReduce(lu->candH, lu->candH, (size_t)v * v, ncclUint64, ncclSum, k % Px, lu->i_comm.c, s));
    }
    if (lu->pi != k % Px) return CFLX_OK;
    PhaseTimer t(lu, RG_step1_lup, s);
    return launch_getrf_nopiv_tile(lu->candH, v, lu->fix_tiny, A00, A00T, rows, lu->tagsH, lu->fix_rec, k * v,
                                   getrf_nopiv_blocked(v), lu->fix_ws.p, s, &lu->launches);
}
int panel_phase(cflx_lu* lu, int k, int fnpr, cudaStream_t s) {
    const int v = lu->v, Px = lu->Px, Py = lu->Py, Pz = lu->Pz, Ml = lu->Ml, Nl = lu->Nl;
    const int pi = lu->pi, pj = lu->pj, pk = lu->pk;
    const int loff = (k / Py) * v, pjk = k % Py;
    if (pj != pjk) return CFLX_OK;
    double* A00 = lu->A00 + (size_t)(k & 1) * v * v;
    double* A00T = lu->A00T + (size_t)(k & 1) * v * v;
    const int n_old = Ml - fnpr;
    const int64_t ldk = std::max<int64_t>(2, round_up(n_old, 2));
    int nR = 0;
    while ((1 << nR) < Px) ++nR;
    {
        PhaseTimer t(lu, RG_step0_copy, s);
        CFLX_TRY(launch_extract_panel_T(lu->A11, Nl, fnpr, loff, n_old, v, lu->PT, ldk, s));
        lu->launches++;
    }
    if (Pz > 1 && n_old > 0) {
        PhaseTimer t(lu, RG_step0_reduce, s);
        CFLX_NCCL(ncclReduce(lu->PT, lu->PT, (size_t)v * ldk, ncclDouble, ncclSum, 0, lu->k_comm.c, s));
    }
    if (pk != 0) return CFLX_OK;
    if (lu->fixed) return fixed_panel(lu, k, fnpr, n_old, ldk, A00, A00T, s);
    int my_half = 0;
    {
        PhaseTimer t(lu, RG_step1_A10copy, s);
        CFLX_CUDA(cudaMemcpyAsync(lu->W, lu->PT, (size_t)v * ldk * sizeof(double), cudaMemcpyDeviceToDevice, s));
    }
    {
        PhaseTimer t(lu, RG_step1_lup, s);
        int nb_used = 0;
        if (nR == 0) {
            CFLX_TRY(launch_panel_getrf_a00(lu->W, ldk, n_old, v, lu->perm, A00, &nb_used, &lu->pws, s));
            CFLX_TRY(launch_gather_a00(lu->W, ldk, lu->perm, v, nb_used, A00, A00T, s));
            lu->launches += 2;
        } else {
            CFLX_TRY(launch_panel_getrf(lu->W, ldk, n_old, v, lu->perm, &lu->pws, s));
            lu->launches++;
        }
    }
    {
        PhaseTimer t(lu, RG_step1_rowpermute, s);
        int first_partner = flipbit(pi, 0);
        if (first_partner > Px - 1) first_partner = Px - 1;
        my_half = first_partner < pi ? 1 : 0;
        CFLX_TRY(launch_gather_winners(lu->PT, ldk, lu->gri + fnpr, n_old, lu->perm, v,
                                       lu->candH + (size_t)my_half * v * v, v, lu->tagsH + my_half * v, 0, s));
        lu->launches++;
    }
    PhaseTimer t(lu, RG_step1_pivoting, s);
    for (int r = 0; r < nR; ++r) {
        CFLX_TRY(tournament_exchange(lu, r, my_half, s));
        const int64_t tot = (int64_t)2 * v * v;
        stack_kernel<<<(unsigned)((tot + 255) / 256), 256, 0, s>>>(lu->candH, lu->tagsH, v, lu->S, lu->W2, lu->tagsS);
        CFLX_CUDA(cudaGetLastError());
        const bool last = (r == nR - 1);
        int nb_used = 0;
        if (last) {
            CFLX_TRY(launch_panel_getrf_a00(lu->W2, 2 * v, 2 * v, v, lu->perm, A00, &nb_used, &lu->pws, s));
            CFLX_TRY(launch_gather_a00(lu->W2, 2 * v, lu->perm, v, nb_used, A00, A00T, s));
            lu->launches++;
            my_half = 0;
        } else {
            CFLX_TRY(launch_panel_getrf(lu->W2, 2 * v, 2 * v, v, lu->perm, &lu->pws, s));
            my_half = butterfly_pair(pi, r + 1, Px) < pi ? 1 : 0;
        }
        CFLX_TRY(launch_gather_winners(lu->S, 2 * v, lu->tagsS, 2 * v, lu->perm, v, lu->candH + (size_t)my_half * v * v,
                                       v, lu->tagsH + my_half * v, 0, s));
        lu->launches += 3;
    }
    return CFLX_OK;
}

int ozaki_planes_a(cflx_lu* lu, int n_act, int64_t ld2, cudaStream_t s) {
    if (!lu->use_ozaki || n_act <= 0) return CFLX_OK;
    PhaseTimer t(lu, RG_step6_dgemm, s);
    lu->launches++;
    return ozaki_split_a(&lu->oz, lu->LT + (int64_t)lu->pk * lu->nlayr * ld2, ld2, n_act, s);
}
int ozaki_planes_b(cflx_lu* lu, int col0, int n, int64_t ldu, cudaStream_t s) {
    if (!lu->use_ozaki || n <= 0) return CFLX_OK;
    PhaseTimer t(lu, RG_step6_dgemm, s);
    lu->launches++;
    return ozaki_split_b(&lu->oz, lu->U + (int64_t)lu->pk * lu->nlayr * ldu, ldu, col0, n, s);
}

int trailing_gemm(cflx_lu* lu, int k, int part, int fnpr, int n_act, int col_lo, int ncols, int64_t ld2, int64_t ldu,
                  int u_col_off, cudaStream_t s, int max_ctas = 0) {
    if (n_act <= 0 || ncols <= 0) return CFLX_OK;
    PhaseTimer t(lu, RG_step6_dgemm, s);
    GemmArgs g{};
    g.M = n_act;
    g.N = ncols;
    g.K = lu->nlayr;
    g.AT = lu->LT + (int64_t)lu->pk * lu->nlayr * ld2;
    g.ldat = ld2;
    g.B = lu->U + (int64_t)lu->pk * lu->nlayr * ldu + u_col_off;
    g.ldb = ldu;
    g.C = lu->A11 + (int64_t)fnpr * lu->Nl + col_lo;
    g.ldc = lu->Nl;
    g.D = lu->A11 + (int64_t)fnpr * lu->Nl + col_lo;
    g.ldd = lu->Nl;
    g.alpha = -1.0;
    g.beta = 1.0;
    const int e = 4 * k + 2 * part;
    if (lu->time_gemm) CFLX_CUDA(cudaEventRecord(lu->ev[e], s));
    if (lu->use_ozaki) CFLX_TRY(launch_ozaki_gemm(&lu->oz, g.M, g.N, 0, u_col_off, g.D, g.ldd, max_ctas, s));
    else CFLX_TRY(launch_gemm_tn(g, s));
    if (lu->time_gemm) CFLX_CUDA(cudaEventRecord(lu->ev[e + 1], s));
    lu->ev_used[e / 2] = lu->time_gemm;
    lu->gemm_flops += 2.0 * g.M * (double)g.N * g.K;
    lu->launches++;
    return CFLX_OK;
}

int finish_step(cflx_lu* lu, int k, int& fnpr) {
    cudaStream_t s = lu->comm->stream;
    const int v = lu->v, Px = lu->Px, Py = lu->Py, Pz = lu->Pz, Ml = lu->Ml, Nl = lu->Nl;
    const int pi = lu->pi, pj = lu->pj, pk = lu->pk;
    const int loff = (k / Py) * v, pjk = k % Py, pik = k % Px;
    const bool on_col = (pj == pjk), on_row = (pi == pik), layer0 = (pk == 0);
    const int c0 = loff + (pj <= pjk ? v : 0);
    const int ncols = Nl - c0;
    const int fnpr_old = fnpr;
    const int n_old = Ml - fnpr_old;
    const int64_t ldk = std::max<int64_t>(2, round_up(n_old, 2));
    int nR = 0;
    while ((1 << nR) < Px) ++nR;
    double* A00 = lu->A00 + (size_t)(k & 1) * v * v;
    double* A00T = lu->A00T + (size_t)(k & 1) * v * v;
    {
        PhaseTimer t(lu, RG_step1_A00Buff_bcast, s);
        if (lu->P > 1) {
            const int root = (pik * Py + pjk) * Pz;
            if (lu->rank == root) {
                CFLX_TRY(launch_pack_bcast(A00, lu->tagsH, v, lu->bcast, s));
                lu->launches++;
            }
            CFLX_NCCL(ncclBroadcast(lu->bcast, lu->bcast, (size_t)v * v + v, ncclDouble, root, lu->comm->world, s));
            CFLX_TRY(launch_unpack_bcast(lu->bcast, v, A00, A00T, lu->gpivots, s));
            lu->launches++;
        } else {
            CFLX_CUDA(cudaMemcpyAsync(lu->gpivots, lu->tagsH, v * sizeof(int), cudaMemcpyDeviceToDevice, s));
        }
        CFLX_TRY(launch_record_pivots(lu->gpivots, v, lu->hist, k, s));
        lu->launches++;
    }
    {
        PhaseTimer t(lu, RG_step2_pushingpivots, s);
        CFLX_TRY(launch_plan_moves(lu->gpivots, v, Px, pi, fnpr_old, Ml, lu->igri, lu->plan, s));
        lu->launches++;
        if (Px > 1 && !lu->fixed) {
            CFLX_CUDA(cudaMemcpyAsync(lu->h_npiv, lu->plan.npiv, sizeof(int), cudaMemcpyDeviceToHost, s));
            CFLX_CUDA(cudaEventRecord(lu->ev_npiv, s));
        }
        const int col_lo = layer0 ? 0 : loff;
        const int64_t ldu0 = std::max(2, ncols);
        CFLX_TRY(launch_push_phase1(lu->A11, Nl, Nl, col_lo, lu->plan, v, lu->tmp, ncols > 0 ? lu->A01raw.p : nullptr, ldu0,
                                    c0, s));
        CFLX_TRY(launch_push_phase2(lu->A11, Nl, Nl, col_lo, lu->plan, v, s));
        CFLX_TRY(launch_push_phase3(lu->A11, Nl, Nl, col_lo, fnpr_old, lu->plan, v, lu->tmp, s));
        CFLX_TRY(launch_update_gri(lu->gri, lu->gri_tmp, lu->igri, lu->plan.rowsrc, fnpr_old, Ml, v, Px, s));
        lu->launches += 5;
    }
    const int64_t ldu = std::max(2, ncols);
    const bool fused_l = (nR == 0) && !lu->fixed;
    if (ncols > 0 && Px * Pz > 1) {
        PhaseTimer t(lu, RG_step2_reduce, s);
        CFLX_NCCL(ncclReduce(lu->A01raw, lu->A01raw, (size_t)v * ldu, ncclDouble, ncclSum, pik * Pz, lu->ik_comm.c, s));
    }
    if (layer0 && ((on_col && !fused_l) || on_row)) {
        PhaseTimer t(lu, RG_step5_dtrsm, s);
        CFLX_TRY(launch_diag_inverses(A00, v, lu->nb, lu->Uinv, lu->LinvT, s));
        lu->launches++;
    }
    const bool split_u = (lu->P == 1) && (k + 1 < lu->Nt) && ncols > v;
    const int ncols_a = split_u ? v : ncols;
    if (on_row && layer0 && ncols > 0) {
        PhaseTimer t(lu, RG_step5_dtrsm, s);
        CFLX_TRY(trsm_left_lower_unit(A00T, lu->LinvT, v, lu->nb, lu->A01raw, lu->U, ldu, ncols_a, s));
        lu->launches += 2 * (v / lu->nb) - 1;
    }
    if (Px * Pz > 1 && ncols > 0) {
        PhaseTimer t(lu, RG_step5_comm, s);
        CFLX_NCCL(ncclBroadcast(lu->U, lu->U, (size_t)v * ldu, ncclDouble, pik * Pz, lu->ik_comm.c, s));
    }
    auto store_factors = [&]() -> int {
        if (!layer0) return CFLX_OK;
        PhaseTimer t(lu, RG_storingresults, s);
        if (ncols > 0) {
            CFLX_TRY(launch_store_u_rows(lu->A11, Nl, fnpr_old, lu->plan, lu->U, ldu, c0, ncols, v, s));
            lu->launches++;
        }
        if (on_col) {
            CFLX_TRY(launch_store_diag(lu->A11, Nl, fnpr_old, lu->plan, A00, loff, v, s));
            lu->launches++;
        }
        return CFLX_OK;
    };
    if (!split_u) CFLX_TRY(store_factors());
    int npiv = v;
    if (lu->fixed) {
        npiv = lu->fix_npiv[k];
    } else if (Px > 1) {
        CFLX_CUDA(cudaEventSynchronize(lu->ev_npiv));
        npiv = *lu->h_npiv;
    }
    if (npiv < 0 || npiv > v || fnpr_old + npiv > Ml) {
        set_last_error("step %d: inconsistent pivot count %d (fnpr %d, Ml %d)", k, npiv, fnpr_old, Ml);
        return CFLX_ERR_STATE;
    }
    fnpr = fnpr_old + npiv;
    const int n_act = Ml - fnpr;
    const int64_t ld2 = std::max<int64_t>(2, round_up(n_act, 2));
    if (on_col && layer0 && n_act > 0) {
        {
            PhaseTimer t(lu, RG_step4_reshuffling, s);
            CFLX_TRY(launch_compact_panel(fused_l ? lu->W : lu->PT, ldk, fused_l ? lu->LT : lu->PT2, ld2, lu->plan.rowsrc,
                                          fnpr_old, lu->plan.npiv, Ml, v, s));
            lu->launches++;
        }
        if (!fused_l) {
            PhaseTimer t(lu, RG_step4_dtrsm, s);
            CFLX_TRY(trsm_right_upper_T(A00, lu->Uinv, v, lu->nb, lu->PT2, lu->LT, ld2, n_act, s));
            lu->launches += 2 * (v / lu->nb) - 1;
        }
        PhaseTimer t(lu, RG_storingresults, s);
        CFLX_TRY(launch_store_panel_T(lu->A11, Nl, fnpr, loff, n_act, v, lu->LT, ld2, s));
        lu->launches++;
    }
    if (Py * Pz > 1 && n_act > 0) {
        PhaseTimer t(lu, RG_step4_comm, s);
        CFLX_NCCL(ncclBroadcast(lu->LT, lu->LT, (size_t)v * ld2, ncclDouble, pjk * Pz, lu->jk_comm.c, s));
    }
    const bool next_col = (k + 1 < lu->Nt) && (pj == (k + 1) % Py);
    CFLX_TRY(ozaki_planes_a(lu, n_act, ld2, s));
    if (n_act > 0) CFLX_TRY(ozaki_planes_b(lu, 0, split_u ? std::min(v, ncols) : ncols, ldu, s));
    if (next_col) {
        const int w = std::min(v, ncols);
        CFLX_TRY(trailing_gemm(lu, k, 0, fnpr, n_act, c0, w, ld2, ldu, 0, s));
        cudaStream_t side = (lu->prof_mode == 1) ? nullptr : lu->side.s;
        cudaStream_t sp = side ? side : s;
        if (side) {
            CFLX_CUDA(cudaEventRecord(lu->ev_fork, s));
            CFLX_CUDA(cudaStreamWaitEvent(sp, lu->ev_fork, 0));
        }
        CFLX_TRY(panel_phase(lu, k + 1, fnpr, sp));
        if (side) CFLX_CUDA(cudaEventRecord(lu->ev_join, sp));
        if (split_u) {
            PhaseTimer t(lu, RG_step5_dtrsm, s);
            CFLX_TRY(trsm_left_lower_unit(A00T, lu->LinvT, v, lu->nb, lu->A01raw + v, lu->U + v, ldu, ncols - v, s));
            lu->launches += 2 * (v / lu->nb) - 1;
        }
        if (split_u) CFLX_TRY(store_factors());
        if (split_u && n_act > 0) CFLX_TRY(ozaki_planes_b(lu, w, ncols - w, ldu, s));
        const int leave = (side && lu->use_ozaki) ? lu->pws.cta_cap : 0;
        CFLX_TRY(trailing_gemm(lu, k, 1, fnpr, n_act, c0 + w, ncols - w, ld2, ldu, w, s, leave > 0 ? lu->oz.sms - leave : 0));
        if (side) CFLX_CUDA(cudaStreamWaitEvent(s, lu->ev_join, 0));
    } else {
        CFLX_TRY(trailing_gemm(lu, k, 0, fnpr, n_act, c0, ncols, ld2, ldu, 0, s));
    }
    return CFLX_OK;
}

SolveFactor lu_solve_factor(cflx_lu* lu) { return SolveFactor{*lu, lu->Cbuf, lu->Ml, &lu->jk_comm, &lu->ik_comm, lu->Pz}; }

int lu_permutation(cflx_lu* lu, std::vector<int>* perm) {
    perm->resize(lu->M);
    CFLX_CUDA(cudaMemcpyAsync(perm->data(), lu->hist, sizeof(int) * lu->M, cudaMemcpyDeviceToHost, lu->comm->stream));
    CFLX_CUDA(cudaStreamSynchronize(lu->comm->stream));
    return CFLX_OK;
}

int lu_solve_prepare(cflx_lu* lu) {
    cudaStream_t s = lu->comm->stream;
    const int v = lu->v, Px = lu->Px, Ml = lu->Ml;
    std::vector<int> hist;
    CFLX_TRY(lu_permutation(lu, &hist));
    if (lu->pk == 0) {
        lu->sv.inv.reset();
        if (!lu->Cbuf) CFLX_TRY(lu->Cbuf.alloc((size_t)Ml * lu->Nl));
        int rc = redistribute_pivoted_rows(lu, hist, true, lu->A11, lu->Cbuf);
        lu->xbuf.reset();
        if (rc) return rc;
        CFLX_TRY(solve_inverses(&lu->sv, lu_solve_factor(lu), false));
        if (lu->pj == 0) {
            std::vector<int> rows(Ml, 0);
            for (int q = 0; q < lu->M; ++q) {
                const int k = q / v;
                if (k % Px == lu->pi) rows[(k / Px) * v + q % v] = hist[q];
            }
            CFLX_TRY(solve_set_rows(&lu->sv.rows, rows, s));
        }
    }
    lu->sv.ready = true;
    lu->sv.trans_ready = false;
    return CFLX_OK;
}

int lu_solve_prepare_trans(cflx_lu* lu) {
    cudaStream_t s = lu->comm->stream;
    const int v = lu->v, Px = lu->Px, Py = lu->Py;
    std::vector<int> hist;
    CFLX_TRY(lu_permutation(lu, &hist));
    std::vector<int> unperm(lu->M);
    for (int q = 0; q < lu->M; ++q) unperm[hist[q]] = q;
    CFLX_TRY(solve_set_rows(&lu->sv.unperm, unperm, s));
    if (lu->pk == 0 && lu->pj == 0) {
        std::vector<int> rows(lu->Ml, 0);
        for (int q = 0; q < lu->M; ++q)
            if ((q / v) % Px == lu->pi) rows[(q / v / Px) * v + q % v] = q;
        CFLX_TRY(solve_set_rows(&lu->sv.rows_id, rows, s));
    }
// ... 222 lines not shown
            for (int lr = 0; lr < Ml; ++lr)
                for (int lc = 0; lc < Nl; ++lc) out[(size_t)lr * Nl + lc] = tab[(size_t)L.row(lr) * n + L.col(lc)];
            return CFLX_OK;
        }
    }
    std::mt19937_64 eng((unsigned long long)(seed + rank));
    std::uniform_real_distribution<double> dist;
    for (int lti = 0; lti < Ml / v; ++lti)
        for (int ltj = 0; ltj < Nl / v; ++ltj)
            for (int li = 0; li < v; ++li)
                for (int lj = 0; lj < v; ++lj) out[(size_t)(lti * v + li) * Nl + ltj * v + lj] = 5 + dist(eng);
    return CFLX_OK;
}

int cflx_lu_create(cflx_comm* c, int M, int N, int v, int Px, int Py, int Pz, cflx_lu** out) {
    REFUSE_IF(!c);
    REFUSE_IF(!out);
    REFUSE_IF(M <= 0);
    REFUSE_IF(N <= 0);
    REFUSE_IF(v <= 0);
    CFLX_CUDA(cudaSetDevice(c->device));
    if (Px <= 0 || Py <= 0 || Pz <= 0) auto_grid(M, N, c->world_size, &Px, &Py, &Pz);
    if (Px != Py) {
        set_last_error("%s: grid %dx%dx%d: the CONFLUX LU path requires Px == Py (SURVEY.md fact 6)", __func__, Px, Py, Pz);
        return CFLX_ERR_UNSUPPORTED;
    }
    if (Px * Py * Pz != c->world_size) {
        set_last_error("%s: grid %dx%dx%d does not match the %d ranks of the communicator", __func__, Px, Py, Pz,
                       c->world_size);
        return CFLX_ERR_ARG;
    }
    if (v % 4 != 0 || v % Pz != 0 || (v / Pz) % 4 != 0 || pick_nb(v) == 0) {
        set_last_error("%s: tile size v=%d unsupported: need v %% 4 == 0 and (v / Pz) %% 4 == 0", __func__, v);
        return CFLX_ERR_UNSUPPORTED;
    }
    int d[8];
    CFLX_TRY(lu_dims(__func__, M, N, v, Px, Py, Pz, d));
    if (d[0] != d[1]) {
        set_last_error("%s: only square matrices are supported (the miniapp passes M = N)", __func__);
        return CFLX_ERR_UNSUPPORTED;
    }
    std::unique_ptr<cflx_lu> lu(new cflx_lu);
    lu->M = d[0]; lu->N = d[1]; lu->Ml = d[2]; lu->Nl = d[3]; lu->Nt = d[4]; lu->nlayr = d[5]; lu->Mt = d[6];
    lu->v = v;
    lu->nb = pick_nb(v);
    CFLX_TRY(handle_init(lu.get(), &kLuTexts, c, Px, Py, Pz));
    CFLX_TRY(make_sub(c, lu->pi, lu->pj * Pz + lu->pk, Py * Pz, &lu->jk_comm));
    CFLX_TRY(make_sub(c, lu->pj, lu->pi * Pz + lu->pk, Px * Pz, &lu->ik_comm));

    const int64_t ldp = round_up(lu->Ml, 2) + 2;
    lu->ldp_max = ldp;
    const size_t pan = (size_t)v * ldp, upan = (size_t)v * (lu->Nl + 2), vv = (size_t)v * v;
    CFLX_TRY(lu->PT.alloc(pan)); CFLX_TRY(lu->PT2.alloc(pan)); CFLX_TRY(lu->W.alloc(pan)); CFLX_TRY(lu->LT.alloc(pan));
    CFLX_TRY(lu->A01raw.alloc(upan)); CFLX_TRY(lu->U.alloc(upan)); CFLX_TRY(lu->tmp.alloc((size_t)v * lu->Nl));
    CFLX_TRY(lu->A00.alloc(2 * vv)); CFLX_TRY(lu->A00T.alloc(2 * vv)); CFLX_TRY(lu->Uinv.alloc(vv));
    CFLX_TRY(lu->LinvT.alloc(vv)); CFLX_TRY(lu->candH.alloc(2 * vv)); CFLX_TRY(lu->S.alloc(2 * vv));
    CFLX_TRY(lu->W2.alloc(2 * vv)); CFLX_TRY(lu->bcast.alloc(vv + v));
    CFLX_TRY(lu->gri.alloc(lu->Ml)); CFLX_TRY(lu->gri_tmp.alloc(lu->Ml)); CFLX_TRY(lu->igri.alloc(lu->Ml));
    CFLX_TRY(lu->perm.alloc(2 * v)); CFLX_TRY(lu->gpivots.alloc(v)); CFLX_TRY(lu->tagsH.alloc(2 * v));
    CFLX_TRY(lu->tagsS.alloc(2 * v)); CFLX_TRY(lu->hist.alloc(lu->M));
    CFLX_TRY(lu->plan_mem.alloc(6 * (size_t)v + 8 + lu->Ml));
    int* pm = lu->plan_mem;
    lu->plan.npiv = pm; lu->plan.nel = pm + 4; pm += 8;
    lu->plan.cur_piv = pm; pm += v;
    lu->plan.order = pm; pm += v;
    lu->plan.slot2piv = pm; pm += v;
    lu->plan.early = pm; pm += v;
    lu->plan.late = pm; pm += v;
    pm += v;
    lu->plan.rowsrc = pm;
    CFLX_TRY(lu->h_npiv.alloc(1));
    CFLX_TRY(lu->ev_npiv.create(cudaEventDisableTiming));
    CFLX_TRY(panel_workspace_create(&lu->pws));
    CFLX_TRY(handle_update_setup(lu.get()));
    {
        const char* e = getenv("CFLX_LOOKAHEAD");
        const char* em = getenv("CFLX_LOOKAHEAD_MULTI");
        const bool want = (e ? atoi(e) != 0 : true) && (lu->P == 1 || !em || atoi(em) != 0);
        if (want) {
            CFLX_TRY(handle_side_stream(lu.get()));
            CFLX_TRY(lu->ev_fork.create(cudaEventDisableTiming));
            CFLX_TRY(lu->ev_join.create(cudaEventDisableTiming));
            const char* c = getenv("CFLX_PANEL_CTAS");
            lu->pws.cta_cap = c ? atoi(c) : (lu->P == 1 ? 32 : (lu->Px == 1 ? 48 : 64));
        }
    }
    cudaMemsetAsync(lu->PT, 0, pan * sizeof(double), c->stream);
    cudaMemsetAsync(lu->PT2, 0, pan * sizeof(double), c->stream);
    cudaMemsetAsync(lu->LT, 0, pan * sizeof(double), c->stream);
    cudaMemsetAsync(lu->W, 0, pan * sizeof(double), c->stream);
    cudaMemsetAsync(lu->A01raw, 0, upan * sizeof(double), c->stream);
    cudaMemsetAsync(lu->U, 0, upan * sizeof(double), c->stream);
    cudaMemsetAsync(lu->A0, 0, (size_t)lu->Ml * lu->Nl * sizeof(double), c->stream);
    CFLX_CUDA(cudaStreamSynchronize(c->stream));
    *out = lu.release();
    return CFLX_OK;
}

int cflx_lu_info(const cflx_lu* lu, int* o) {
    REFUSE_IF(!lu);
    REFUSE_IF(!o);
    const int vals[16] = {lu->M, lu->N, lu->Ml, lu->Nl, lu->Nt, lu->nlayr, lu->P, lu->Px, lu->Py, lu->Pz, lu->pi, lu->pj,
                          lu->pk, lu->rank, lu->v, 0};
    std::memcpy(o, vals, sizeof(vals));
    return CFLX_OK;
}

// ... 615 lines not shown
```

conflux_b200/csrc/ozaki.cu:

```cuda
#include <cuda.h>

#include <algorithm>
#include <cstdlib>
#include <cstring>

#include "common.cuh"
#include "kernels.h"

namespace cflx {

namespace {
constexpr int OZ_S = 8;
constexpr int OZ_BM = 128, OZ_BN = 64, OZ_KC = 64;
constexpr int OZ_GP = 3;
constexpr int OZ_NPASS = (OZ_S + OZ_GP - 1) / OZ_GP;
constexpr int OZ_STAGES = 2;
constexpr int OZ_A_BYTES = OZ_BM * OZ_KC, OZ_B_BYTES = OZ_BN * OZ_KC;
constexpr int OZ_STAGE_BYTES = OZ_S * (OZ_A_BYTES + OZ_B_BYTES);
constexpr int OZ_CONS_WARPS = 8;
constexpr int OZ_THREADS = 32 * OZ_CONS_WARPS + 32;
constexpr size_t OZ_SMEM = 1024  + (size_t)OZ_STAGES * OZ_STAGE_BYTES + 64 ;
constexpr int OZ_SPLIT_KC = 128;

__device__ __forceinline__ void tma_load_3d(void* smem_dst, const CUtensorMap* map, int c0, int c1, int c2, uint64_t* bar) {
// ... 15 lines not shown
    asm volatile(
        "{\n\t.reg .pred p;\n\tsetp.ne.b32 p, %34, 0;\n\t"
        "wgmma.mma_async.sync.aligned.m64n64k32.s32.s8.s8 {%0, %1, %2, %3, %4, %5, %6, %7, %8, %9, %10, %11, %12, %13, %14, %15, %16, %17, %18, %19, %20, %21, %22, %23, %24, %25, %26, %27, %28, %29, %30, %31}, %32, %33, p;\n\t}"
        : "+r"(d[0]), "+r"(d[1]), "+r"(d[2]), "+r"(d[3]), "+r"(d[4]), "+r"(d[5]), "+r"(d[6]), "+r"(d[7]), "+r"(d[8]), "+r"(d[9]), "+r"(d[10]), "+r"(d[11]), "+r"(d[12]), "+r"(d[13]), "+r"(d[14]), "+r"(d[15]), "+r"(d[16]), "+r"(d[17]), "+r"(d[18]), "+r"(d[19]), "+r"(d[20]), "+r"(d[21]), "+r"(d[22]), "+r"(d[23]), "+r"(d[24]), "+r"(d[25]), "+r"(d[26]), "+r"(d[27]), "+r"(d[28]), "+r"(d[29]), "+r"(d[30]), "+r"(d[31])
        : "l"(da), "l"(db), "r"(1)
        : "memory");
}
__device__ __forceinline__ void wgmma_s8_n128(int* d, uint64_t da, uint64_t db) {
    asm volatile(
        "{\n\t.reg .pred p;\n\tsetp.ne.b32 p, %66, 0;\n\t"
        "wgmma.mma_async.sync.aligned.m64n128k32.s32.s8.s8 {%0, %1, %2, %3, %4, %5, %6, %7, %8, %9, %10, %11, %12, %13, %14, %15, %16, %17, %18, %19, %20, %21, %22, %23, %24, %25, %26, %27, %28, %29, %30, %31, %32, %33, %34, %35, %36, %37, %38, %39, %40, %41, %42, %43, %44, %45, %46, %47, %48, %49, %50, %51, %52, %53, %54, %55, %56, %57, %58, %59, %60, %61, %62, %63}, %64, %65, p;\n\t}"
        : "+r"(d[0]), "+r"(d[1]), "+r"(d[2]), "+r"(d[3]), "+r"(d[4]), "+r"(d[5]), "+r"(d[6]), "+r"(d[7]), "+r"(d[8]), "+r"(d[9]), "+r"(d[10]), "+r"(d[11]), "+r"(d[12]), "+r"(d[13]), "+r"(d[14]), "+r"(d[15]), "+r"(d[16]), "+r"(d[17]), "+r"(d[18]), "+r"(d[19]), "+r"(d[20]), "+r"(d[21]), "+r"(d[22]), "+r"(d[23]), "+r"(d[24]), "+r"(d[25]), "+r"(d[26]), "+r"(d[27]), "+r"(d[28]), "+r"(d[29]), "+r"(d[30]), "+r"(d[31]), "+r"(d[32]), "+r"(d[33]), "+r"(d[34]), "+r"(d[35]), "+r"(d[36]), "+r"(d[37]), "+r"(d[38]), "+r"(d[39]), "+r"(d[40]), "+r"(d[41]), "+r"(d[42]), "+r"(d[43]), "+r"(d[44]), "+r"(d[45]), "+r"(d[46]), "+r"(d[47]), "+r"(d[48]), "+r"(d[49]), "+r"(d[50]), "+r"(d[51]), "+r"(d[52]), "+r"(d[53]), "+r"(d[54]), "+r"(d[55]), "+r"(d[56]), "+r"(d[57]), "+r"(d[58]), "+r"(d[59]), "+r"(d[60]), "+r"(d[61]), "+r"(d[62]), "+r"(d[63])
        : "l"(da), "l"(db), "r"(1)
        : "memory");
}
__device__ __forceinline__ void wgmma_s8_n192(int* d, uint64_t da, uint64_t db) {
    asm volatile(
        "{\n\t.reg .pred p;\n\tsetp.ne.b32 p, %98, 0;\n\t"
        "wgmma.mma_async.sync.aligned.m64n192k32.s32.s8.s8 {%0, %1, %2, %3, %4, %5, %6, %7, %8, %9, %10, %11, %12, %13, %14, %15, %16, %17, %18, %19, %20, %21, %22, %23, %24, %25, %26, %27, %28, %29, %30, %31, %32, %33, %34, %35, %36, %37, %38, %39, %40, %41, %42, %43, %44, %45, %46, %47, %48, %49, %50, %51, %52, %53, %54, %55, %56, %57, %58, %59, %60, %61, %62, %63, %64, %65, %66, %67, %68, %69, %70, %71, %72, %73, %74, %75, %76, %77, %78, %79, %80, %81, %82, %83, %84, %85, %86, %87, %88, %89, %90, %91, %92, %93, %94, %95}, %96, %97, p;\n\t}"
        : "+r"(d[0]), "+r"(d[1]), "+r"(d[2]), "+r"(d[3]), "+r"(d[4]), "+r"(d[5]), "+r"(d[6]), "+r"(d[7]), "+r"(d[8]), "+r"(d[9]), "+r"(d[10]), "+r"(d[11]), "+r"(d[12]), "+r"(d[13]), "+r"(d[14]), "+r"(d[15]), "+r"(d[16]), "+r"(d[17]), "+r"(d[18]), "+r"(d[19]), "+r"(d[20]), "+r"(d[21]), "+r"(d[22]), "+r"(d[23]), "+r"(d[24]), "+r"(d[25]), "+r"(d[26]), "+r"(d[27]), "+r"(d[28]), "+r"(d[29]), "+r"(d[30]), "+r"(d[31]), "+r"(d[32]), "+r"(d[33]), "+r"(d[34]), "+r"(d[35]), "+r"(d[36]), "+r"(d[37]), "+r"(d[38]), "+r"(d[39]), "+r"(d[40]), "+r"(d[41]), "+r"(d[42]), "+r"(d[43]), "+r"(d[44]), "+r"(d[45]), "+r"(d[46]), "+r"(d[47]), "+r"(d[48]), "+r"(d[49]), "+r"(d[50]), "+r"(d[51]), "+r"(d[52]), "+r"(d[53]), "+r"(d[54]), "+r"(d[55]), "+r"(d[56]), "+r"(d[57]), "+r"(d[58]), "+r"(d[59]), "+r"(d[60]), "+r"(d[61]), "+r"(d[62]), "+r"(d[63]), "+r"(d[64]), "+r"(d[65]), "+r"(d[66]), "+r"(d[67]), "+r"(d[68]), "+r"(d[69]), "+r"(d[70]), "+r"(d[71]), "+r"(d[72]), "+r"(d[73]), "+r"(d[74]), "+r"(d[75]), "+r"(d[76]), "+r"(d[77]), "+r"(d[78]), "+r"(d[79]), "+r"(d[80]), "+r"(d[81]), "+r"(d[82]), "+r"(d[83]), "+r"(d[84]), "+r"(d[85]), "+r"(d[86]), "+r"(d[87]), "+r"(d[88]), "+r"(d[89]), "+r"(d[90]), "+r"(d[91]), "+r"(d[92]), "+r"(d[93]), "+r"(d[94]), "+r"(d[95])
        : "l"(da), "l"(db), "r"(1)
        : "memory");
}
__device__ __forceinline__ void wgmma_s8_n256(int* d, uint64_t da, uint64_t db) {
    asm volatile(
        "{\n\t.reg .pred p;\n\tsetp.ne.b32 p, %130, 0;\n\t"
        "wgmma.mma_async.sync.aligned.m64n256k32.s32.s8.s8 {%0, %1, %2, %3, %4, %5, %6, %7, %8, %9, %10, %11, %12, %13, %14, %15, %16, %17, %18, %19, %20, %21, %22, %23, %24, %25, %26, %27, %28, %29, %30, %31, %32, %33, %34, %35, %36, %37, %38, %39, %40, %41, %42, %43, %44, %45, %46, %47, %48, %49, %50, %51, %52, %53, %54, %55, %56, %57, %58, %59, %60, %61, %62, %63, %64, %65, %66, %67, %68, %69, %70, %71, %72, %73, %74, %75, %76, %77, %78, %79, %80, %81, %82, %83, %84, %85, %86, %87, %88, %89, %90, %91, %92, %93, %94, %95, %96, %97, %98, %99, %100, %101, %102, %103, %104, %105, %106, %107, %108, %109, %110, %111, %112, %113, %114, %115, %116, %117, %118, %119, %120, %121, %122, %123, %124, %125, %126, %127}, %128, %129, p;\n\t}"
        : "+r"(d[0]), "+r"(d[1]), "+r"(d[2]), "+r"(d[3]), "+r"(d[4]), "+r"(d[5]), "+r"(d[6]), "+r"(d[7]), "+r"(d[8]), "+r"(d[9]), "+r"(d[10]), "+r"(d[11]), "+r"(d[12]), "+r"(d[13]), "+r"(d[14]), "+r"(d[15]), "+r"(d[16]), "+r"(d[17]), "+r"(d[18]), "+r"(d[19]), "+r"(d[20]), "+r"(d[21]), "+r"(d[22]), "+r"(d[23]), "+r"(d[24]), "+r"(d[25]), "+r"(d[26]), "+r"(d[27]), "+r"(d[28]), "+r"(d[29]), "+r"(d[30]), "+r"(d[31]), "+r"(d[32]), "+r"(d[33]), "+r"(d[34]), "+r"(d[35]), "+r"(d[36]), "+r"(d[37]), "+r"(d[38]), "+r"(d[39]), "+r"(d[40]), "+r"(d[41]), "+r"(d[42]), "+r"(d[43]), "+r"(d[44]), "+r"(d[45]), "+r"(d[46]), "+r"(d[47]), "+r"(d[48]), "+r"(d[49]), "+r"(d[50]), "+r"(d[51]), "+r"(d[52]), "+r"(d[53]), "+r"(d[54]), "+r"(d[55]), "+r"(d[56]), "+r"(d[57]), "+r"(d[58]), "+r"(d[59]), "+r"(d[60]), "+r"(d[61]), "+r"(d[62]), "+r"(d[63]), "+r"(d[64]), "+r"(d[65]), "+r"(d[66]), "+r"(d[67]), "+r"(d[68]), "+r"(d[69]), "+r"(d[70]), "+r"(d[71]), "+r"(d[72]), "+r"(d[73]), "+r"(d[74]), "+r"(d[75]), "+r"(d[76]), "+r"(d[77]), "+r"(d[78]), "+r"(d[79]), "+r"(d[80]), "+r"(d[81]), "+r"(d[82]), "+r"(d[83]), "+r"(d[84]), "+r"(d[85]), "+r"(d[86]), "+r"(d[87]), "+r"(d[88]), "+r"(d[89]), "+r"(d[90]), "+r"(d[91]), "+r"(d[92]), "+r"(d[93]), "+r"(d[94]), "+r"(d[95]), "+r"(d[96]), "+r"(d[97]), "+r"(d[98]), "+r"(d[99]), "+r"(d[100]), "+r"(d[101]), "+r"(d[102]), "+r"(d[103]), "+r"(d[104]), "+r"(d[105]), "+r"(d[106]), "+r"(d[107]), "+r"(d[108]), "+r"(d[109]), "+r"(d[110]), "+r"(d[111]), "+r"(d[112]), "+r"(d[113]), "+r"(d[114]), "+r"(d[115]), "+r"(d[116]), "+r"(d[117]), "+r"(d[118]), "+r"(d[119]), "+r"(d[120]), "+r"(d[121]), "+r"(d[122]), "+r"(d[123]), "+r"(d[124]), "+r"(d[125]), "+r"(d[126]), "+r"(d[127])
        : "l"(da), "l"(db), "r"(1)
        : "memory");
}

template <int PLANES>
__device__ __forceinline__ void wgmma_s8(int* acc, uint64_t da, uint64_t db) {
    if constexpr (PLANES == 1) wgmma_s8_n64(acc, da, db);
    else if constexpr (PLANES == 2) wgmma_s8_n128(acc, da, db);
    else if constexpr (PLANES == 3) wgmma_s8_n192(acc, da, db);
    else wgmma_s8_n256(acc, da, db);
}

__host__ __device__ constexpr double pow2c(int e) {
    double x = 1.0;
    for (int i = 0; i < -e; ++i) x *= 0.5;
    return x;
}
__device__ __forceinline__ double pow2i(int e) { return __longlong_as_double((long long)(1023 + e) << 52); }

struct OzArgs {
    int M, N, K;
    int a_row0;
    int b_row0;
    double* C;
    int64_t ldc;
    const int* ea;
    const int* eb;
    int tiles_m, tiles_n;
};

template <int G0, int S>
__device__ __forceinline__ void pass_products(int* acc, uint32_t a_base, uint32_t b_base) {
    constexpr int G1 = (G0 + OZ_GP < OZ_S ? G0 + OZ_GP : OZ_S) - 1;
    if constexpr (S <= G1) {
        constexpr int T_LO = G0 - S > 0 ? G0 - S : 0;
        constexpr int PLANES = G1 - S - T_LO + 1;
#pragma unroll
        for (int k = 0; k < OZ_KC / 32; ++k)
            wgmma_s8<PLANES>(acc + 32 * (S + T_LO - G0), smem_desc_sw64(a_base + S * OZ_A_BYTES + 32 * k),
                             smem_desc_sw64(b_base + T_LO * OZ_B_BYTES + 32 * k));
        pass_products<G0, S + 1>(acc, a_base, b_base);
    }
}

template <int P>
__device__ __forceinline__ void consume_pass(const OzArgs& g, uint64_t* full, uint64_t* empty, uint32_t sbase, int wg, int lane,
                                             uint32_t& q, double (&sum)[32]) {
    if constexpr (P < OZ_NPASS) {
        constexpr int G0 = P * OZ_GP;
        constexpr int NG = (G0 + OZ_GP < OZ_S ? OZ_GP : OZ_S - G0);
        int acc[OZ_GP * 32];
#pragma unroll
        for (int i = 0; i < OZ_GP * 32; ++i) acc[i] = 0;
        const int KC = g.K / OZ_KC;
        for (int kc = 0; kc < KC; ++kc, ++q) {
            const int st = q % OZ_STAGES;
            mbar_wait(&full[st], (q / OZ_STAGES) & 1);
            const uint32_t a_base = sbase + st * OZ_STAGE_BYTES + wg * (64 * OZ_KC);
            const uint32_t b_base = sbase + st * OZ_STAGE_BYTES + OZ_S * OZ_A_BYTES;
            wgmma_fence();
            pass_products<G0, 0>(acc, a_base, b_base);
            wgmma_commit();
            wgmma_wait<0>();
            __syncwarp();
            if (lane == 0) mbar_arrive(&empty[st]);
        }
#pragma unroll
        for (int gi = 0; gi < NG; ++gi) {
            const double w = pow2c(-7 * (G0 + gi));
#pragma unroll
            for (int i = 0; i < 32; ++i) {
                const double x = __hiloint2double(0x43300000, acc[32 * gi + i] ^ 0x80000000) - 4503601774854144.0;
                sum[i] = fma(x, w, sum[i]);
            }
        }
        consume_pass<P + 1>(g, full, empty, sbase, wg, lane, q, sum);
    }
}
// ... 8 lines not shown
    const int warp = threadIdx.x >> 5, lane = threadIdx.x & 31;
    const int ntiles = g.tiles_m * g.tiles_n;
    const int KC = g.K / OZ_KC;

    if (threadIdx.x == 0) {
        for (int i = 0; i < OZ_STAGES; ++i) {
            mbar_init(&full[i], 1);
            mbar_init(&empty[i], OZ_CONS_WARPS);
        }
        fence_barrier_init();
    }
    __syncthreads();

    if (warp == OZ_CONS_WARPS) {
        if (lane == 0) {
            uint32_t q = 0;
            for (int tile = blockIdx.x; tile < ntiles; tile += gridDim.x) {
                const int m0 = (tile / g.tiles_n) * OZ_BM, n0 = (tile % g.tiles_n) * OZ_BN;
                for (int p = 0; p < OZ_NPASS; ++p) {
                    const int np = (p + 1) * OZ_GP < OZ_S ? (p + 1) * OZ_GP : OZ_S;
                    for (int kc = 0; kc < KC; ++kc, ++q) {
                        const int st = q % OZ_STAGES;
                        const uint32_t use = q / OZ_STAGES;
                        if (use > 0) mbar_wait(&empty[st], (use - 1) & 1);
                        unsigned char* sa = base + (size_t)st * OZ_STAGE_BYTES;
                        unsigned char* sb = sa + OZ_S * OZ_A_BYTES;
                        mbar_arrive_expect_tx(&full[st], (uint32_t)(np * (OZ_A_BYTES + OZ_B_BYTES)));
                        for (int t = 0; t < np; ++t) {
                            tma_load_3d(sa + t * OZ_A_BYTES, &mapA, kc * OZ_KC, g.a_row0 + m0, t, &full[st]);
                            tma_load_3d(sb + t * OZ_B_BYTES, &mapB, kc * OZ_KC, g.b_row0 + n0, t, &full[st]);
                        }
                    }
                }
            }
        }
        return;
    }

    const int wg = warp >> 2;
    const uint32_t sbase = smem_u32(base);
    uint32_t q = 0;
    for (int tile = blockIdx.x; tile < ntiles; tile += gridDim.x) {
        const int m0 = (tile / g.tiles_n) * OZ_BM, n0 = (tile % g.tiles_n) * OZ_BN;
        double sum[32];
#pragma unroll
        for (int i = 0; i < 32; ++i) sum[i] = 0.0;
        consume_pass<0>(g, full, empty, sbase, wg, lane, q, sum);
        const int r0 = m0 + 64 * wg + 16 * (warp & 3) + (lane >> 2);
#pragma unroll
        for (int h = 0; h < 2; ++h) {
            const int row = r0 + 8 * h;
            if (row >= g.M) continue;
            const double sr = -pow2i(g.ea[g.a_row0 + row] - 12);
            double* crow = g.C + (int64_t)row * g.ldc;
#pragma unroll
            for (int j = 0; j < 8; ++j) {
                const int col = n0 + 8 * j + 2 * (lane & 3);
                if (col >= g.N) continue;
                double2 c = *reinterpret_cast<const double2*>(crow + col);
                c.x += (sum[4 * j + 2 * h] * sr) * pow2i(g.eb[g.b_row0 + col]);
                c.y += (sum[4 * j + 2 * h + 1] * sr) * pow2i(g.eb[g.b_row0 + col + 1]);
                *reinterpret_cast<double2*>(crow + col) = c;
            }
        }
    }
}

template <int PLANES>
__global__ void __launch_bounds__(256, 1) wgmma_peak_kernel(int iters, int* sink) {
    extern __shared__ unsigned char pk_smem_raw[];
    unsigned char* base = reinterpret_cast<unsigned char*>(((uintptr_t)pk_smem_raw + 1023) & ~(uintptr_t)1023);
    for (int i = threadIdx.x; i < (4096 + 16384) / 4; i += blockDim.x) reinterpret_cast<uint32_t*>(base)[i] = 0x01010101u * (i & 3);
    fence_proxy_async();
    __syncthreads();
    int acc[32 * PLANES];
#pragma unroll
    for (int i = 0; i < 32 * PLANES; ++i) acc[i] = 0;
    const uint32_t a = smem_u32(base), b = smem_u32(base + 4096);
    wgmma_fence();
    for (int it = 0; it < iters; ++it) {
#pragma unroll
        for (int k = 0; k < 2; ++k) wgmma_s8<PLANES>(acc, smem_desc_sw64(a + 32 * k), smem_desc_sw64(b + 32 * k));
        wgmma_commit();
        wgmma_wait<1>();
    }
    wgmma_wait<0>();
    int x = 0;
#pragma unroll
    for (int i = 0; i < 32 * PLANES; ++i) x ^= acc[i];
    if (x == 0x7fffffff) *sink = x;
}

constexpr int OZ_SPLIT_OUT = 32;
__global__ void __launch_bounds__(256) ozaki_split_kernel(const double* __restrict__ src, int64_t ld, int n_outer, int K,
                                                          int8_t* __restrict__ planes, int64_t plane_stride, int o0,
                                                          int* __restrict__ exps) {
    constexpr int PITCH = OZ_SPLIT_KC + 4;
    __shared__ __align__(16) unsigned char tile[OZ_S][OZ_SPLIT_OUT][PITCH];
    __shared__ double red[8][OZ_SPLIT_OUT];
    __shared__ int s_exp[OZ_SPLIT_OUT];
    const int tx = threadIdx.x & 31, ty = threadIdx.x >> 5;
    const int o = blockIdx.x * OZ_SPLIT_OUT + tx;
    const bool valid = o < n_outer;
    double mx = 0.0;
    if (valid)
        for (int k = ty; k < K; k += 8) mx = fmax(mx, fabs(src[(int64_t)k * ld + o]));
    red[ty][tx] = mx;
    __syncthreads();
    if (ty == 0) {
#pragma unroll
        for (int i = 1; i < 8; ++i) mx = fmax(mx, red[i][tx]);
        int e = 0;
        if (mx > 0.0) frexp(mx, &e);
        s_exp[tx] = e;
        if (valid) exps[o0 + o] = e;
// ... 88 lines not shown
    CFLX_CUDA(cfg.raise(OZ_SMEM, [&] {
        return cudaFuncSetAttribute(ozaki_gemm_kernel, cudaFuncAttributeMaxDynamicSharedMemorySize, (int)OZ_SMEM);
    }));
    int dev = 0;
    CFLX_CUDA(cudaGetDevice(&dev));
    CFLX_CUDA(cudaDeviceGetAttribute(&ws->sms, cudaDevAttrMultiProcessorCount, dev));
    return CFLX_OK;
}

int wgmma_peak_probe(int n, double* tmacs_out) {
    void (*kern)(int, int*) = n == 64 ? wgmma_peak_kernel<1> : n == 128 ? wgmma_peak_kernel<2> : n == 192 ? wgmma_peak_kernel<3>
                            : n == 256 ? wgmma_peak_kernel<4> : nullptr;
    if (!kern) return CFLX_ERR_ARG;
    int dev = 0, sms = 0;
    CFLX_CUDA(cudaGetDevice(&dev));
    CFLX_CUDA(cudaDeviceGetAttribute(&sms, cudaDevAttrMultiProcessorCount, dev));
    const size_t smem = 1024 + 4096 + 16384;
    CFLX_CUDA(cudaFuncSetAttribute(kern, cudaFuncAttributeMaxDynamicSharedMemorySize, (int)smem));
    DevBuf<> sink;
    CFLX_TRY(sink.alloc(sizeof(int)));
    Events<2> ev;
    CFLX_TRY(ev.create());
    const int iters = 20000;
    double best = 0;
    for (int rep = 0; rep < 3; ++rep) {
        CFLX_CUDA(cudaEventRecord(ev[0]));
        kern<<<sms, 256, smem>>>(iters, sink.as<int>());
        CFLX_CUDA(cudaEventRecord(ev[1]));
        CFLX_CUDA(cudaEventSynchronize(ev[1]));
        float ms = 0;
        CFLX_CUDA(cudaEventElapsedTime(&ms, ev[0], ev[1]));
        const double macs = (double)sms * 2 * iters * 2 * 64.0 * n * 32.0;
        best = std::max(best, macs / (ms * 1e-3) / 1e12);
    }
    CFLX_CUDA(cudaGetLastError());
    *tmacs_out = best;
    return CFLX_OK;
}

int ozaki_split_a(OzakiWorkspace* ws, const double* LT, int64_t ld, int n, cudaStream_t s) {
    if (n <= 0) return CFLX_OK;
    if (n > ws->cap_a) return CFLX_ERR_ARG;
    ozaki_split_kernel<<<(n + OZ_SPLIT_OUT - 1) / OZ_SPLIT_OUT, 256, 0, s>>>(LT, ld, n, ws->K, ws->planesA, (int64_t)ws->cap_a * ws->K, 0, ws->ea);
    CFLX_CUDA(cudaGetLastError());
    return CFLX_OK;
}
int ozaki_split_b(OzakiWorkspace* ws, const double* U, int64_t ld, int col0, int n, cudaStream_t s) {
    if (n <= 0) return CFLX_OK;
    if (col0 < 0 || col0 + n > ws->cap_b) return CFLX_ERR_ARG;
    ozaki_split_kernel<<<(n + OZ_SPLIT_OUT - 1) / OZ_SPLIT_OUT, 256, 0, s>>>(U + col0, ld, n, ws->K, ws->planesB, (int64_t)ws->cap_b * ws->K, col0, ws->eb);
    CFLX_CUDA(cudaGetLastError());
    return CFLX_OK;
}
int launch_ozaki_gemm(OzakiWorkspace* ws, int M, int N, int row0, int col0, double* C, int64_t ldc, int max_ctas, cudaStream_t s) {
    if (M <= 0 || N <= 0) return CFLX_OK;
    if ((N & 1) || (ldc & 1) || col0 < 0 || row0 < 0 || row0 + M > ws->cap_a || col0 + N > ws->cap_b) {
        set_last_error("ozaki_gemm: unsupported window M=%d N=%d row0=%d col0=%d ldc=%lld", M, N, row0, col0, (long long)ldc);
        return CFLX_ERR_UNSUPPORTED;
    }
    OzArgs g{};
    g.M = M; g.N = N; g.K = ws->K;
    g.a_row0 = row0;
    g.b_row0 = col0;
    g.C = C; g.ldc = ldc;
    g.ea = ws->ea; g.eb = ws->eb;
    g.tiles_m = (M + OZ_BM - 1) / OZ_BM;
    g.tiles_n = (N + OZ_BN - 1) / OZ_BN;
    int grid = g.tiles_m * g.tiles_n;
    int cap = ws->sms;
    if (max_ctas > 0 && max_ctas < cap) cap = max_ctas;
    if (grid > cap) grid = cap;
    ozaki_gemm_kernel<<<grid, OZ_THREADS, OZ_SMEM, s>>>(ws->maps->a, ws->maps->b, g);
    CFLX_CUDA(cudaGetLastError());
    return CFLX_OK;
}

}
```

conflux_b200/csrc/rows.cu:

```cuda
#include <algorithm>

#include "common.cuh"
#include "kernels.h"

namespace cflx {

namespace {

__global__ void extract_panel_T_kernel(const double* __restrict__ A, int64_t lda, int64_t row0, int64_t col0, int n,
                                       int v, double* __restrict__ PT, int64_t ldp) {
    __shared__ double tile[32][33];
    const int r0 = blockIdx.x * 32, c0 = blockIdx.y * 32;
    for (int dy = threadIdx.y; dy < 32; dy += blockDim.y) {
        const int r = r0 + dy, c = c0 + threadIdx.x;
        if (r < n && c < v) tile[dy][threadIdx.x] = A[(row0 + r) * lda + col0 + c];
    }
    __syncthreads();
    for (int dy = threadIdx.y; dy < 32; dy += blockDim.y) {
        const int c = c0 + dy, r = r0 + threadIdx.x;
        if (r < n && c < v) PT[(int64_t)c * ldp + r] = tile[threadIdx.x][dy];
    }
}
__global__ void store_panel_T_kernel(double* __restrict__ A, int64_t lda, int64_t row0, int64_t col0, int n, int v,
                                     const double* __restrict__ LT, int64_t ldp) {
    __shared__ double tile[32][33];
    const int r0 = blockIdx.x * 32, c0 = blockIdx.y * 32;
    for (int dy = threadIdx.y; dy < 32; dy += blockDim.y) {
        const int c = c0 + dy, r = r0 + threadIdx.x;
        if (r < n && c < v) tile[dy][threadIdx.x] = LT[(int64_t)c * ldp + r];
    }
    __syncthreads();
    for (int dy = threadIdx.y; dy < 32; dy += blockDim.y) {
        const int r = r0 + dy, c = c0 + threadIdx.x;
        if (r < n && c < v) A[(row0 + r) * lda + col0 + c] = tile[threadIdx.x][dy];
    }
}

__global__ void gather_winners_kernel(const double* __restrict__ PT, int64_t ldp, const int* __restrict__ tags,
                                      int n_valid, const int* __restrict__ perm, int v, double* __restrict__ out,
                                      int64_t ldo, int* __restrict__ out_tags, int dst0) {
    const int64_t e = (int64_t)blockIdx.x * blockDim.x + threadIdx.x;
    if (e >= (int64_t)v * v) return;
    const int c = (int)(e / v), i = (int)(e % v);
    const int src = perm[i];
    out[(int64_t)c * ldo + dst0 + i] = src < n_valid ? PT[(int64_t)c * ldp + src] : 0.0;
    if (c == 0) out_tags[dst0 + i] = src < n_valid ? tags[src] : 0;
}
__global__ void gather_a00_kernel(const double* __restrict__ W, int64_t ldw, const int* __restrict__ perm, int v, int nb,
                                  double* __restrict__ A00, double* __restrict__ A00T) {
    const int64_t e = (int64_t)blockIdx.x * blockDim.x + threadIdx.x;
    if (e >= (int64_t)v * v) return;
    const int i = (int)(e / v), c = (int)(e % v);
    double val;
    if (nb <= 0 || c < (i / nb) * nb) {
        val = W[(int64_t)c * ldw + perm[i]];
        A00[e] = val;
    } else {
        val = A00[e];
    }
    A00T[(int64_t)c * v + i] = val;
}

__global__ void __launch_bounds__(256) plan_moves_kernel(const int* __restrict__ gpivots, int v, int Px, int pi, int fnpr,
                                                         int Ml, const int* __restrict__ igri, MovePlan plan) {
    extern __shared__ int sm[];
    int* mine = sm;
    int* prow = sm + v;
    __shared__ int s_npiv, s_nel;
    const int t = threadIdx.x, T = blockDim.x;
    for (int i = t; i < v; i += T) mine[i] = ((gpivots[i] / v) % Px == pi) ? 1 : 0;
    for (int r = fnpr + t; r < Ml; r += T) plan.rowsrc[r] = r;
    __syncthreads();
    for (int i = t; i < v; i += T) {
        int rank = 0;
        for (int j = 0; j < i; ++j) rank += mine[j];
        if (mine[i]) {
            const int g = gpivots[i];
            const int lidx = (g / (v * Px)) * v + g % v;
            const int lrow = igri[lidx];
            plan.cur_piv[rank] = lrow;
            plan.order[rank] = i;
            plan.slot2piv[i] = rank;
            prow[rank] = lrow;
        } else {
            plan.slot2piv[i] = -1;
        }
        if (i == v - 1) s_npiv = rank + mine[i];
    }
    __syncthreads();
    const int npiv = s_npiv;
    for (int i = t; i < npiv; i += T) {
        const int r = fnpr + i;
        bool isp = false;
        for (int j = 0; j < npiv; ++j) isp = isp || (prow[j] == r);
        mine[i] = isp ? 0 : 1;
    }
    __syncthreads();
    for (int i = t; i < npiv; i += T) {
        if (mine[i]) {
            int rank = 0;
            for (int j = 0; j < i; ++j) rank += mine[j];
            plan.early[rank] = fnpr + i;
        }
        const int pr = prow[i];
        if (pr >= fnpr + npiv) {
            int rank = 0;
            for (int j = 0; j < npiv; ++j) rank += (prow[j] >= fnpr + npiv && prow[j] < pr) ? 1 : 0;
            plan.late[rank] = pr;
        }
    }
    if (t == 0) {
        int ne = 0;
        for (int j = 0; j < npiv; ++j) ne += mine[j];
        s_nel = ne;
        plan.npiv[0] = npiv;
        plan.nel[0] = ne;
    }
    __syncthreads();
    const int nel = s_nel;
    for (int i = t; i < nel; i += T) plan.rowsrc[plan.late[i]] = plan.early[i];
    for (int i = t; i < npiv; i += T) plan.rowsrc[fnpr + i] = prow[i];
}

__device__ __forceinline__ void copy_row_seg(double* __restrict__ dst, const double* __restrict__ src, int len, int chunk,
                                             int nchunks) {
    const int n2 = len >> 1;
    const int per = (n2 + nchunks - 1) / nchunks;
    const int b = chunk * per, e = min(n2, b + per);
    const double2* s2 = reinterpret_cast<const double2*>(src);
    double2* d2 = reinterpret_cast<double2*>(dst);
    for (int i = b + threadIdx.x; i < e; i += blockDim.x) d2[i] = s2[i];
}
__global__ void push_phase1_kernel(const double* __restrict__ A, int64_t lda, int ncols, int col_lo, MovePlan plan, int v,
                                   double* __restrict__ tmp, double* __restrict__ a01raw, int64_t ld01, int c0) {
    const int npiv = plan.npiv[0];
    const int y = blockIdx.y;
    if (y < v) {
        if (y >= npiv) return;
        const int src = plan.cur_piv[y];
        copy_row_seg(tmp + (int64_t)y * lda + col_lo, A + (int64_t)src * lda + col_lo, ncols - col_lo, blockIdx.x,
                     gridDim.x);
    } else if (a01raw != nullptr) {
        const int slot = y - v;
        const int p = plan.slot2piv[slot];
        const int len = ncols - c0;
        double* dst = a01raw + (int64_t)slot * ld01;
        if (p >= 0) {
            copy_row_seg(dst, A + (int64_t)plan.cur_piv[p] * lda + c0, len, blockIdx.x, gridDim.x);
        } else {
            const int n2 = len >> 1;
            const int per = (n2 + gridDim.x - 1) / gridDim.x;
            const int b = blockIdx.x * per, e = min(n2, b + per);
            double2* d2 = reinterpret_cast<double2*>(dst);
            for (int i = b + threadIdx.x; i < e; i += blockDim.x) d2[i] = make_double2(0.0, 0.0);
        }
    }
}
__global__ void push_phase2_kernel(double* __restrict__ A, int64_t lda, int ncols, int col_lo, MovePlan plan) {
    if ((int)blockIdx.y >= plan.nel[0]) return;
    const int src = plan.early[blockIdx.y], dst = plan.late[blockIdx.y];
    copy_row_seg(A + (int64_t)dst * lda + col_lo, A + (int64_t)src * lda + col_lo, ncols - col_lo, blockIdx.x, gridDim.x);
}
__global__ void push_phase3_kernel(double* __restrict__ A, int64_t lda, int ncols, int col_lo, int fnpr, MovePlan plan,
                                   const double* __restrict__ tmp) {
    if ((int)blockIdx.y >= plan.npiv[0]) return;
    copy_row_seg(A + (int64_t)(fnpr + blockIdx.y) * lda + col_lo, tmp + (int64_t)blockIdx.y * lda + col_lo, ncols - col_lo,
                 blockIdx.x, gridDim.x);
}

__global__ void gri_gather_kernel(const int* __restrict__ gri, int* __restrict__ gri_tmp, const int* __restrict__ rowsrc,
                                  int fnpr, int Ml) {
    const int r = fnpr + blockIdx.x * blockDim.x + threadIdx.x;
    if (r < Ml) gri_tmp[r] = gri[rowsrc[r]];
}
__global__ void gri_commit_kernel(int* __restrict__ gri, const int* __restrict__ gri_tmp, int* __restrict__ igri, int fnpr,
                                  int Ml, int v, int Px) {
    const int r = fnpr + blockIdx.x * blockDim.x + threadIdx.x;
    if (r < Ml) {
        const int g = gri_tmp[r];
        gri[r] = g;
        igri[(g / (v * Px)) * v + g % v] = r;
    }
}
__global__ void compact_panel_kernel(const double* __restrict__ PT, int64_t ldp, double* __restrict__ PT2, int64_t ldp2,
                                     const int* __restrict__ rowsrc, int fnpr_old, const int* __restrict__ npiv, int Ml) {
    const int fnpr_new = fnpr_old + npiv[0];
    const int rp = blockIdx.x * blockDim.x + threadIdx.x;
    const int c = blockIdx.y;
    if (fnpr_new + rp < Ml) PT2[(int64_t)c * ldp2 + rp] = PT[(int64_t)c * ldp + (rowsrc[fnpr_new + rp] - fnpr_old)];
}
__global__ void store_u_rows_kernel(double* __restrict__ A, int64_t lda, int fnpr_old, MovePlan plan,
                                    const double* __restrict__ U, int64_t ldu, int c0, int ncols) {
    if ((int)blockIdx.y >= plan.npiv[0]) return;
    const int i = blockIdx.y;
    copy_row_seg(A + (int64_t)(fnpr_old + i) * lda + c0, U + (int64_t)plan.order[i] * ldu, ncols, blockIdx.x, gridDim.x);
}
__global__ void store_diag_kernel(double* __restrict__ A, int64_t lda, int fnpr_old, MovePlan plan,
                                  const double* __restrict__ A00, int loff, int v) {
    if ((int)blockIdx.y >= plan.npiv[0]) return;
    const int i = blockIdx.y;
    const double* src = A00 + (int64_t)plan.order[i] * v;
    double* dst = A + (int64_t)(fnpr_old + i) * lda + loff;
    for (int c = threadIdx.x; c < v; c += blockDim.x) dst[c] = src[c];
}

__global__ void fill_kernel(double* p, int64_t n, double val) {
    const int64_t i = (int64_t)blockIdx.x * blockDim.x + threadIdx.x;
    if (i < n) p[i] = val;
}
__global__ void iota_gri_kernel(int* gri, int* igri, int Ml, int v, int Px, int pi) {
    const int i = blockIdx.x * blockDim.x + threadIdx.x;
    if (i < Ml) {
        gri[i] = (i % v) + ((i / v) * Px + pi) * v;
        igri[i] = i;
    }
}
__global__ void pack_bcast_kernel(const double* A00, const int* tags, int v, double* buf) {
    const int i = blockIdx.x * blockDim.x + threadIdx.x;
    if (i < v * v) buf[i] = A00[i];
    if (i < v) buf[v * v + i] = (double)tags[i];
// ... 40 lines not shown
__device__ __forceinline__ double block_sum(double s) {
    for (int o = 16; o > 0; o >>= 1) s += __shfl_xor_sync(0xffffffffu, s, o);
    __shared__ double w[32];
    if ((threadIdx.x & 31) == 0) w[threadIdx.x >> 5] = s;
    __syncthreads();
    if (threadIdx.x < 32) {
        s = threadIdx.x < (blockDim.x >> 5) ? w[threadIdx.x] : 0.0;
        for (int o = 16; o > 0; o >>= 1) s += __shfl_xor_sync(0xffffffffu, s, o);
    }
    return s;
}
__global__ void sumsq_partial_kernel(const double* __restrict__ X, int64_t count, double* __restrict__ partials) {
    double s = 0.0;
    for (int64_t i = (int64_t)blockIdx.x * blockDim.x + threadIdx.x; i < count; i += (int64_t)gridDim.x * blockDim.x)
        s = fma(X[i], X[i], s);
    s = block_sum(s);
    if (threadIdx.x == 0) partials[blockIdx.x] = s;
}
__global__ void sumsq_final_kernel(const double* __restrict__ partials, int n, double* __restrict__ out) {
    double s = 0.0;
    for (int i = threadIdx.x; i < n; i += blockDim.x) s += partials[i];
    s = block_sum(s);
    if (threadIdx.x == 0) *out += s;
}

inline int row_chunks(int len) {
    int c = (len / 2 + 2047) / 2048;
    return c < 1 ? 1 : (c > 64 ? 64 : c);
}
}

#define POST_LAUNCH()                     \
    do {                                  \
        CFLX_CUDA(cudaGetLastError());    \
        return CFLX_OK;                   \
    } while (0)

int launch_extract_panel_T(const double* A, int64_t lda, int64_t row0, int64_t col0, int n, int v, double* PT,
                           int64_t ldp, cudaStream_t s) {
    if (n <= 0) return CFLX_OK;
    dim3 grid((n + 31) / 32, (v + 31) / 32), block(32, 8);
    extract_panel_T_kernel<<<grid, block, 0, s>>>(A, lda, row0, col0, n, v, PT, ldp);
    POST_LAUNCH();
}
int launch_store_panel_T(double* A, int64_t lda, int64_t row0, int64_t col0, int n, int v, const double* LT, int64_t ldp,
                         cudaStream_t s) {
    if (n <= 0) return CFLX_OK;
    dim3 grid((n + 31) / 32, (v + 31) / 32), block(32, 8);
    store_panel_T_kernel<<<grid, block, 0, s>>>(A, lda, row0, col0, n, v, LT, ldp);
    POST_LAUNCH();
}
int launch_gather_winners(const double* PT, int64_t ldp, const int* tags, int n_valid, const int* perm, int v,
                          double* out_vals, int64_t ldo, int* out_tags, int dst0, cudaStream_t s) {
    const int64_t tot = (int64_t)v * v;
    gather_winners_kernel<<<(unsigned)((tot + 255) / 256), 256, 0, s>>>(PT, ldp, tags, n_valid, perm, v, out_vals, ldo,
                                                                        out_tags, dst0);
    POST_LAUNCH();
}
int launch_gather_a00(const double* W, int64_t ldw, const int* perm, int v, int nb, double* A00, double* A00T,
                      cudaStream_t s) {
    const int64_t tot = (int64_t)v * v;
    gather_a00_kernel<<<(unsigned)((tot + 255) / 256), 256, 0, s>>>(W, ldw, perm, v, nb, A00, A00T);
    POST_LAUNCH();
}
int launch_plan_moves(const int* gpivots, int v, int Px, int pi, int fnpr, int Ml, const int* igri, MovePlan plan,
                      cudaStream_t s) {
    plan_moves_kernel<<<1, 256, 2 * v * sizeof(int), s>>>(gpivots, v, Px, pi, fnpr, Ml, igri, plan);
    POST_LAUNCH();
}
int launch_push_phase1(const double* A, int64_t lda, int ncols, int col_lo, MovePlan plan, int v, double* tmp,
                       double* a01raw, int64_t ld01, int c0, cudaStream_t s) {
    dim3 grid(row_chunks(ncols), a01raw ? 2 * v : v);
    push_phase1_kernel<<<grid, 256, 0, s>>>(A, lda, ncols, col_lo, plan, v, tmp, a01raw, ld01, c0);
    POST_LAUNCH();
}
int launch_push_phase2(double* A, int64_t lda, int ncols, int col_lo, MovePlan plan, int v, cudaStream_t s) {
    dim3 grid(row_chunks(ncols), v);
    push_phase2_kernel<<<grid, 256, 0, s>>>(A, lda, ncols, col_lo, plan);
    POST_LAUNCH();
}
int launch_push_phase3(double* A, int64_t lda, int ncols, int col_lo, int fnpr, MovePlan plan, int v, const double* tmp,
                       cudaStream_t s) {
    dim3 grid(row_chunks(ncols), v);
    push_phase3_kernel<<<grid, 256, 0, s>>>(A, lda, ncols, col_lo, fnpr, plan, tmp);
    POST_LAUNCH();
}
int launch_update_gri(int* gri, int* gri_tmp, int* igri, const int* rowsrc, int fnpr, int Ml, int v, int Px,
                      cudaStream_t s) {
    const int n = Ml - fnpr;
    if (n <= 0) return CFLX_OK;
    gri_gather_kernel<<<(n + 255) / 256, 256, 0, s>>>(gri, gri_tmp, rowsrc, fnpr, Ml);
    gri_commit_kernel<<<(n + 255) / 256, 256, 0, s>>>(gri, gri_tmp, igri, fnpr, Ml, v, Px);
    POST_LAUNCH();
}
int launch_compact_panel(const double* PT, int64_t ldp, double* PT2, int64_t ldp2, const int* rowsrc, int fnpr_old,
                         const int* npiv, int Ml, int v, cudaStream_t s) {
    const int n = Ml - fnpr_old;
    if (n <= 0) return CFLX_OK;
    dim3 grid((n + 255) / 256, v);
    compact_panel_kernel<<<grid, 256, 0, s>>>(PT, ldp, PT2, ldp2, rowsrc, fnpr_old, npiv, Ml);
    POST_LAUNCH();
}
int launch_store_u_rows(double* A, int64_t lda, int fnpr_old, MovePlan plan, const double* U, int64_t ldu, int c0,
                        int ncols, int v, cudaStream_t s) {
    if (ncols <= 0) return CFLX_OK;
    dim3 grid(row_chunks(ncols), v);
    store_u_rows_kernel<<<grid, 256, 0, s>>>(A, lda, fnpr_old, plan, U, ldu, c0, ncols);
    POST_LAUNCH();
}
int launch_store_diag(double* A, int64_t lda, int fnpr_old, MovePlan plan, const double* A00, int loff, int v,
                      cudaStream_t s) {
    dim3 grid(1, v);
    store_diag_kernel<<<grid, 128, 0, s>>>(A, lda, fnpr_old, plan, A00, loff, v);
    POST_LAUNCH();
}
int launch_split_factors(const double* F, int64_t ldf, int n, double* LT, double* U, cudaStream_t s) {
    dim3 grid((n + 31) / 32, (n + 31) / 32), block(32, 8);
    split_factors_kernel<<<grid, block, 0, s>>>(F, ldf, n, LT, U);
    POST_LAUNCH();
}
int launch_gather_perm_rows(const double* A, int64_t lda, const int* perm, int n, double* out, cudaStream_t s) {
    dim3 grid(n, std::max(1, std::min(32, n / 256)));
    gather_perm_rows_kernel<<<grid, 256, 0, s>>>(A, lda, perm, n, out);
    POST_LAUNCH();
}
int launch_sumsq(const double* X, int64_t count, double* out, double* partials, cudaStream_t s) {
    sumsq_partial_kernel<<<SUMSQ_PARTIALS, 256, 0, s>>>(X, count, partials);
    CFLX_CUDA(cudaGetLastError());
    return launch_sum_partials(partials, SUMSQ_PARTIALS, out, s);
}
int launch_sum_partials(const double* partials, int n, double* out, cudaStream_t s) {
    sumsq_final_kernel<<<1, 1024, 0, s>>>(partials, n, out);
    POST_LAUNCH();
}
int launch_fill(double* p, int64_t n, double val, cudaStream_t s) {
    if (n <= 0) return CFLX_OK;
    fill_kernel<<<(unsigned)((n + 255) / 256), 256, 0, s>>>(p, n, val);
// ... 21 lines not shown
```

include/conflux_b200.h:

```cpp
#ifndef CONFLUX_B200_H
#define CONFLUX_B200_H

#include <stddef.h>
#include <stdint.h>

#ifdef __cplusplus
extern "C" {
#endif

typedef enum {
    CFLX_OK = 0,
    CFLX_ERR_ARG = -1,
    CFLX_ERR_CUDA = -2,
    CFLX_ERR_NCCL = -3,
    CFLX_ERR_UNSUPPORTED = -4,
    CFLX_ERR_STATE = -5,
    CFLX_ERR_NO_DEVICE = -6
} cflx_status;

typedef struct cflx_comm cflx_comm;
typedef struct cflx_lu cflx_lu;

#define CFLX_UNIQUE_ID_BYTES 128

// ... 49 lines not shown
int cflx_lu_inverse(cflx_lu*, double* Ainv_local, int* info_out);
int cflx_lu_det(cflx_lu*, int unscaled, double* sign_out, double* logabsdet_out, double* mant_out, int64_t* exp_out,
                int* info_out);
int cflx_lu_uses_ozaki(const cflx_lu*);
int cflx_lu_launch_count(cflx_lu*, int64_t* count_out, int reset);
int cflx_lu_set_profiling(cflx_lu*, int mode);
int cflx_lu_phase_ms(cflx_lu*, double* ms_out);
int cflx_lu_timeline(cflx_lu*, char* buf, int buf_len);
int cflx_lu_set_kernel_timing(cflx_lu*, int enabled);
int cflx_lu_trailing_stats(cflx_lu*, double* ms_out, double* flops_out);
void cflx_lu_destroy(cflx_lu*);

typedef struct cflx_chol cflx_chol;
int cflx_chol_auto_grid(int P, int N, int* grid3_out);
int cflx_chol_auto_tile(int N, int P, int Pz);
int cflx_chol_dims(int N, int v, int Px, int Py, int Pz, int* dims_out);
int cflx_chol_init_matrix_host(int N, int v, int Px, int Py, int Pz, int rank, double* local_out);
int cflx_chol_create(cflx_comm*, int N, int v, int Px, int Py, int Pz, cflx_chol** out);
int cflx_chol_info(const cflx_chol*, int* info_out);
int cflx_chol_set_local(cflx_chol*, const double* host_local);
int cflx_chol_factor(cflx_chol*, double* ms_out);
int cflx_chol_factor_ldlt(cflx_chol*, double tiny, int* nrepl_out, int64_t* inertia_out, int* info_out, double* ms_out);
int cflx_chol_rbt(cflx_chol*, int depth, uint64_t seed, double* u_out);
int cflx_chol_rbt_solve(cflx_chol*, int nrhs, const double* B, int ldb, double* X, int ldx, int refine, double* ferr_out,
                        double* berr_out);
int cflx_chol_rbt_apply_local(cflx_chol*, int op, int nrhs, double* B_local, int ldb);
int cflx_chol_get_signs(cflx_chol*, double* s_out);
int cflx_chol_get_input(cflx_chol*, double* A_host);
int cflx_chol_get_local(cflx_chol*, double* L_host);
int cflx_chol_validate(cflx_chol*, double* frob_abs_out, double* frob_rel_out);
int cflx_chol_solve(cflx_chol*, int nrhs, const double* B, int ldb, double* X, int ldx);
int cflx_chol_solve_local(cflx_chol*, int nrhs, const double* B_local, int ldb, double* X_local, int ldx);
int cflx_chol_rcond(cflx_chol*, double* rcond_out, double* anorm_out);
int cflx_chol_refine(cflx_chol*, int nrhs, const double* B, int ldb, double* X, int ldx, double* ferr_out,
                     double* berr_out);
int cflx_chol_refine_x(cflx_chol*, int nrhs, const double* B, int ldb, double* X, int ldx, double* rcond_out,
                       double* berr_out, double* err_bnds_norm_out, double* err_bnds_comp_out, int* info_out);
int cflx_chol_equilibrate(cflx_chol*, int apply, double* s_out, double* scond_out, double* amax_out, char* equed_out,
                          int* info_out);
int cflx_chol_svx(cflx_chol*, int nrhs, const double* B, int ldb, double* X, int ldx, double* rcond_out, double* ferr_out,
                  double* berr_out, char* equed_out, int* info_out);
int cflx_chol_equilibrate_b(cflx_chol*, int apply, double* s_out, double* scond_out, double* amax_out, char* equed_out,
                            int* info_out);
int cflx_chol_svxx(cflx_chol*, int nrhs, const double* B, int ldb, double* X, int ldx, double* rcond_out,
                   double* rpvgrw_out, double* berr_out, double* err_bnds_norm_out, double* err_bnds_comp_out,
                   char* equed_out, int* info_out);
int cflx_chol_inverse(cflx_chol*, double* Ainv_local);
int cflx_chol_det(cflx_chol*, int unscaled, double* logdet_out, double* mant_out, int64_t* exp_out);
int cflx_chol_launch_count(cflx_chol*, int64_t* count_out, int reset);
void cflx_chol_destroy(cflx_chol*);

int cflx_dbg_gemm_tn(int M, int N, int K, const double* AT, int at_rows, int64_t ldat, int64_t at_off, const double* B,
                     int b_rows, int64_t ldb, int64_t b_off, const double* C, int c_rows, int64_t ldc, int row_off,
                     int col_off, double alpha, double beta, int in_place, double* D_out, double* C_out, int reps,
                     double* ms_out);
int cflx_dbg_gemm_narrow(int M, int N, int K, const double* A, const double* B, const double* C, double alpha, double beta,
                         double* D, int reps, double* ms_out);
int cflx_dbg_gemm_narrow_tn(int M, int N, int K, const double* AT, const double* B, const double* C, double alpha,
                            double beta, double* D, int reps, double* ms_out);
int cflx_dbg_gemm_narrow_window(int trans, int M, int N, int K, const double* A, int a_rows, int64_t lda, int a_row,
                                int a_col, const double* B, int b_rows, int64_t ldb, int b_row, int b_col, const double* C,
                                int c_rows, int64_t ldc, int c_row, int c_col, double alpha, double beta, int in_place,
                                double* D_out, double* C_out);
int cflx_dbg_diag_solve(int tri, int lower, int v, int nb, const double* share, int rows, int64_t ld, int row0, int col0,
                        int ldn, const double* R, double* Y_out, double* inv_out);
typedef struct { int M, v, Kappa, Ml, Nl, Px, Py, pi, pj; } cflx_share_layout;
int cflx_dbg_residual(int mode, const cflx_share_layout* share, const double* A, int nrhs, const double* Xc,
                      const double* Xr, double* P_out, double* Q_out, int reps, double* ms_out);
int cflx_dbg_residual_x(int mode, const cflx_share_layout* share, const double* A, int nrhs, const double* Xc,
                        const double* Xct, const double* Xr, const double* Xrt, double* hi_out, double* lo_out, int reps,
                        double* ms_out);
int cflx_dbg_equil(const cflx_share_layout* share, const double* A, const double* r, const double* c, char equed, int ncols,
                   double* rowmax_out, double* colmax_out, double* diag_out, double* scaled_out, double* sym_scaled_out,
                   double* growth_out, int* zero_pivot_out);
int cflx_dbg_growth_cols(int mode, const cflx_share_layout* share, int ncols, const double* F, const double* A,
                         double* amax_out, double* fmax_out);
int cflx_dbg_inverse_share(int mode, const cflx_share_layout* share, int c0, int nc, int rows, const double* X, int ldx,
                           const int* perm, double* W_out, double* share_inout, int zero_fill);
int cflx_dbg_solve_local_share(int mode, const cflx_share_layout* share, int nrhs, int c0, int w, const double* B, int ldb,
                               double* Bk_out, const double* Xk, double* X_inout, int ldx);
int cflx_dbg_norm_share(int mode, const cflx_share_layout* share, const double* A, double* out);
int cflx_dbg_rbt_share(int op, const cflx_share_layout* share, int depth, const double* u, const double* v, int ncols,
                       double* share_inout, int ld);
int cflx_dbg_chol_validate_share(const cflx_share_layout* share, const double* A, int t, double* PT_out, double* sumsq_out);
int cflx_dbg_lu_validate_share(const cflx_share_layout* share, const double* C, int t, double* LT_out, double* U_out);
int cflx_dbg_chol_gather_cols(const cflx_share_layout* share, int gfirst, const double* pieces, double* Bc_out);
int cflx_dbg_refine_assemble(int mode, int Px, int Py, int Pz, int v, int M, int Ml, int Nl, int nn, int tn, int nrhs,
                             int ldn, const double* all, const double* B, double* R_out, double* ratio_out, double* W_out,
                             double* Q_out);
int cflx_dbg_refine_columns(int M, int ldn, int nrhs, const double* A, const double* D, const double* d, const int* sel,
                            double* max_out, double* stats_out, double* select_out, double* add_out, double* Y_out,
                            double* T_inout);
int cflx_dbg_det(int n, const double* d, const double* s1, const double* s2, int square, double* mant_out,
                 int64_t* exp_out, int* neg_out, int* first_zero_out, int* nonfinite_out);
int cflx_dbg_panel(int n, int v, const double* panel, int* perm_out, double* A00_out, double* LU_out, int reps,
                   double* ms_out);
int cflx_dbg_trsm(int n, int v, int nb, int64_t ld, const double* A00, const double* B, double* X_out, const double* R,
                  double* Y_out);
int cflx_dbg_diag_inverse(int v, int nb, const double* A00, double* Uinv_out, double* LinvT_out);
int cflx_dbg_potrf_tile(int v, const double* A, double* L_out, double* LT_out, int* info_out, int variant);
int cflx_dbg_solve_signs(const cflx_share_layout* share, int ldn, const double* sgn, double* Z_inout);
int cflx_dbg_ldlt_tile(int v, const double* A, double tiny, double* R_out, double* SRT_out, double* s_out, int* nrepl_out,
                       int* inertia_out, int* info_out, int variant);
int cflx_dbg_getrf_nopiv_tile(int v, const double* A, double tiny, double* LU_out, int* nrepl_out, int* info_out,
                              int variant);
int cflx_dbg_ozaki_gemm(int M, int N, int K, int row0, int col0, int max_ctas, const double* AT, const double* B,
                        const double* C, double* D, signed char* planesA_out, signed char* planesB_out, int* ea_out,
                        int* eb_out, int reps, double* ms_out, double* split_ms_out);
int cflx_dbg_wgmma_peak(int n, double* tmacs_out);
int cflx_dbg_push_pivots(int n_rows, int n_cols, double* A_inout, int npiv, const int* pivot_rows, int fnpr, int* gri_out,
                         double* a01_out);
int cflx_dbg_fp64_peak(int which, double* tflops_out);
int cflx_dbg_fp64_peak_ex(int which, double* burst_out, double* sustained_out);

#ifdef __cplusplus
}
#endif
#endif
```

Baseline: 26430.

## Read trailing GEMM C rows through a row table to fold pivot row moves

Adds an optional row-index table to the trailing-update GEMM and Ozaki GEMM so C rows can be gathered through indirection instead of first being physically moved. The pivot push is restructured: phase 1 only extracts A01 rows, and phases 2/3 copy both pivot and displaced rows through a doubled tmp buffer over a column window. This lets the LU step restrict row swaps to a column range and let the GEMM read unmoved rows directly, cutting row-copy traffic. It costs extra shared memory for the row table and indirect C loads, and widens the tmp buffer.

```diff
diff --git a/conflux_b200/__init__.py b/conflux_b200/__init__.py
--- a/conflux_b200/__init__.py
+++ b/conflux_b200/__init__.py
@@ -616,7 +616,7 @@
 
     @staticmethod
     def gemm_tn_window(AT, B, C, M, N, K, alpha=1.0, beta=0.0, at_off=(0, 0), b_off=(0, 0), c_off=(0, 0), in_place=True,
-                       reps=1):
+                       reps=1, crow=None):
         AT = np.ascontiguousarray(AT, dtype=np.float64)
         B = np.ascontiguousarray(B, dtype=np.float64)
         C = np.ascontiguousarray(C, dtype=np.float64)
@@ -627,6 +627,7 @@
                                      at_off[0] * AT.shape[1] + at_off[1], B.ctypes.data, B.shape[0], B.shape[1],
                                      b_off[0] * B.shape[1] + b_off[1], C.ctypes.data, C.shape[0], C.shape[1],
                                      int(c_off[0]), int(c_off[1]), float(alpha), float(beta), 1 if in_place else 0,
+                                     _ptr(None if crow is None else np.ascontiguousarray(crow, dtype=np.int32)),
                                      D.ctypes.data, Cout.ctypes.data, int(reps), ctypes.byref(ms)), "dbg_gemm_tn")
         return D, Cout, ms.value
 
@@ -983,6 +984,18 @@
         return dict(D=D, ms=ms.value, split_ms=sms.value, pa=pa, pb=pb, ea=ea, eb=eb)
 
     @staticmethod
+    def ozaki_gemm_rows(AT, B, C, c_off=0, crow=None):
+        AT = np.ascontiguousarray(AT, dtype=np.float64)
+        B = np.ascontiguousarray(B, dtype=np.float64)
+        C = np.ascontiguousarray(C, dtype=np.float64)
+        K, M = AT.shape
+        rows = None if crow is None else np.ascontiguousarray(crow, dtype=np.int32)
+        D = np.empty_like(C)
+        check(lib().cflx_dbg_ozaki_gemm_rows(M, B.shape[1], K, AT.ctypes.data, B.ctypes.data, C.ctypes.data, C.shape[0],
+                                             int(c_off), _ptr(rows), D.ctypes.data), "dbg_ozaki_gemm_rows")
+        return D
+
+    @staticmethod
     def push_pivots(A, pivot_rows, fnpr):
         A = np.array(A, dtype=np.float64, order="C")
         piv = np.ascontiguousarray(pivot_rows, dtype=np.int32)
diff --git a/conflux_b200/_lib.py b/conflux_b200/_lib.py
--- a/conflux_b200/_lib.py
+++ b/conflux_b200/_lib.py
@@ -24,7 +24,7 @@
     "cflx_lu_get_permutation", "cflx_lu_residual", "cflx_lu_validate", "cflx_lu_solve", "cflx_lu_solve_trans", "cflx_rhs_local_cols", "cflx_lu_solve_local", "cflx_lu_rcond", "cflx_lu_refine", "cflx_lu_refine_x", "cflx_lu_equilibrate", "cflx_lu_svx", "cflx_lu_equilibrate_b", "cflx_lu_svxx", "cflx_lu_inverse", "cflx_lu_det", "cflx_lu_launch_count", "cflx_lu_uses_ozaki", "cflx_lu_set_profiling", "cflx_lu_phase_ms", "cflx_lu_timeline",
     "cflx_lu_set_kernel_timing", "cflx_lu_trailing_stats", "cflx_lu_destroy", "cflx_chol_auto_grid", "cflx_chol_auto_tile", "cflx_chol_dims", "cflx_chol_init_matrix_host",
     "cflx_chol_create", "cflx_chol_info", "cflx_chol_set_local", "cflx_chol_factor", "cflx_chol_factor_ldlt", "cflx_chol_rbt", "cflx_chol_rbt_solve", "cflx_chol_rbt_apply_local", "cflx_chol_get_signs", "cflx_chol_get_input", "cflx_chol_get_local", "cflx_chol_validate",
-    "cflx_chol_solve", "cflx_chol_solve_local", "cflx_chol_rcond", "cflx_chol_refine", "cflx_chol_refine_x", "cflx_chol_equilibrate", "cflx_chol_svx", "cflx_chol_equilibrate_b", "cflx_chol_svxx", "cflx_chol_inverse", "cflx_chol_det", "cflx_chol_launch_count", "cflx_chol_destroy", "cflx_dbg_gemm_tn", "cflx_dbg_gemm_narrow", "cflx_dbg_gemm_narrow_tn", "cflx_dbg_gemm_narrow_window", "cflx_dbg_diag_solve", "cflx_dbg_residual", "cflx_dbg_residual_x", "cflx_dbg_equil", "cflx_dbg_growth_cols", "cflx_dbg_inverse_share", "cflx_dbg_solve_local_share", "cflx_dbg_norm_share", "cflx_dbg_rbt_share", "cflx_dbg_chol_validate_share", "cflx_dbg_lu_validate_share", "cflx_dbg_chol_gather_cols", "cflx_dbg_refine_assemble", "cflx_dbg_refine_columns", "cflx_dbg_det", "cflx_dbg_panel", "cflx_dbg_trsm", "cflx_dbg_diag_inverse", "cflx_dbg_potrf_tile", "cflx_dbg_ldlt_tile", "cflx_dbg_solve_signs", "cflx_dbg_getrf_nopiv_tile", "cflx_dbg_push_pivots", "cflx_dbg_ozaki_gemm", "cflx_dbg_wgmma_peak", "cflx_dbg_fp64_peak", "cflx_dbg_fp64_peak_ex",
+    "cflx_chol_solve", "cflx_chol_solve_local", "cflx_chol_rcond", "cflx_chol_refine", "cflx_chol_refine_x", "cflx_chol_equilibrate", "cflx_chol_svx", "cflx_chol_equilibrate_b", "cflx_chol_svxx", "cflx_chol_inverse", "cflx_chol_det", "cflx_chol_launch_count", "cflx_chol_destroy", "cflx_dbg_gemm_tn", "cflx_dbg_gemm_narrow", "cflx_dbg_gemm_narrow_tn", "cflx_dbg_gemm_narrow_window", "cflx_dbg_diag_solve", "cflx_dbg_residual", "cflx_dbg_residual_x", "cflx_dbg_equil", "cflx_dbg_growth_cols", "cflx_dbg_inverse_share", "cflx_dbg_solve_local_share", "cflx_dbg_norm_share", "cflx_dbg_rbt_share", "cflx_dbg_chol_validate_share", "cflx_dbg_lu_validate_share", "cflx_dbg_chol_gather_cols", "cflx_dbg_refine_assemble", "cflx_dbg_refine_columns", "cflx_dbg_det", "cflx_dbg_panel", "cflx_dbg_trsm", "cflx_dbg_diag_inverse", "cflx_dbg_potrf_tile", "cflx_dbg_ldlt_tile", "cflx_dbg_solve_signs", "cflx_dbg_getrf_nopiv_tile", "cflx_dbg_push_pivots", "cflx_dbg_ozaki_gemm", "cflx_dbg_ozaki_gemm_rows", "cflx_dbg_wgmma_peak", "cflx_dbg_fp64_peak", "cflx_dbg_fp64_peak_ex",
 ]
 
 
@@ -141,8 +141,7 @@
         L.cflx_init_matrix_host.argtypes = [ctypes.c_int] * 8 + [ctypes.c_void_p]
         _buf = [ctypes.c_void_p, ctypes.c_int, ctypes.c_int64]
         L.cflx_dbg_gemm_tn.argtypes = [ctypes.c_int] * 3 + _buf + [ctypes.c_int64] + _buf + [ctypes.c_int64] + _buf + [
-            ctypes.c_int] * 2 + [ctypes.c_double] * 2 + [ctypes.c_int, ctypes.c_void_p, ctypes.c_void_p, ctypes.c_int,
-                                                          c_double_p]
+            ctypes.c_int] * 2 + [ctypes.c_double] * 2 + [ctypes.c_int] + [ctypes.c_void_p] * 3 + [ctypes.c_int, c_double_p]
         L.cflx_dbg_gemm_narrow.argtypes = [ctypes.c_int] * 3 + [ctypes.c_void_p] * 3 + [ctypes.c_double] * 2 + [
             ctypes.c_void_p, ctypes.c_int, c_double_p]
         L.cflx_dbg_gemm_narrow_tn.argtypes = [ctypes.c_int] * 3 + [ctypes.c_void_p] * 3 + [ctypes.c_double] * 2 + [
@@ -185,6 +184,8 @@
         L.cflx_dbg_push_pivots.argtypes = [ctypes.c_int, ctypes.c_int, ctypes.c_void_p, ctypes.c_int, ctypes.c_void_p, ctypes.c_int,
                                            ctypes.c_void_p, ctypes.c_void_p]
         L.cflx_dbg_ozaki_gemm.argtypes = [ctypes.c_int] * 6 + [ctypes.c_void_p] * 8 + [ctypes.c_int, c_double_p, c_double_p]
+        L.cflx_dbg_ozaki_gemm_rows.argtypes = [ctypes.c_int] * 3 + [ctypes.c_void_p] * 3 + [ctypes.c_int] * 2 + [
+            ctypes.c_void_p] * 2
         L.cflx_dbg_wgmma_peak.argtypes = [ctypes.c_int, c_double_p]
         L.cflx_dbg_fp64_peak.argtypes = [ctypes.c_int, c_double_p]
         L.cflx_dbg_fp64_peak_ex.argtypes = [ctypes.c_int, c_double_p, c_double_p]
diff --git a/conflux_b200/csrc/chol.cu b/conflux_b200/csrc/chol.cu
--- a/conflux_b200/csrc/chol.cu
+++ b/conflux_b200/csrc/chol.cu
@@ -428,7 +428,7 @@
         g.ldd = Nl;
         g.alpha = -1.0; g.beta = 1.0;
         if (ch->use_ozaki && planes_buf == buf)
-            CFLX_TRY(launch_ozaki_gemm(&ch->oz, M, g.N, (li - my_first) * v, (lj - lj0) * v, g.D, Nl, ch->oz.sms - chol_leave_sms(), s));
+            CFLX_TRY(launch_ozaki_gemm(&ch->oz, M, g.N, (li - my_first) * v, (lj - lj0) * v, g.D, Nl, nullptr, nullptr, ch->oz.sms - chol_leave_sms(), s));
         else
             CFLX_TRY(launch_gemm_tn(g, s));
         ch->launches++;
diff --git a/conflux_b200/csrc/dbg.cu b/conflux_b200/csrc/dbg.cu
--- a/conflux_b200/csrc/dbg.cu
+++ b/conflux_b200/csrc/dbg.cu
@@ -212,8 +212,8 @@
 
 int cflx_dbg_gemm_tn(int M, int N, int K, const double* AT, int at_rows, int64_t ldat, int64_t at_off, const double* B,
                      int b_rows, int64_t ldb, int64_t b_off, const double* C, int c_rows, int64_t ldc, int row_off,
-                     int col_off, double alpha, double beta, int in_place, double* D_out, double* C_out, int reps,
-                     double* ms_out) {
+                     int col_off, double alpha, double beta, int in_place, const int* crow, double* D_out, double* C_out,
+                     int reps, double* ms_out) {
     CFLX_TRY(check_device());
     REFUSE_IF(M <= 0 || N <= 0 || K <= 0);
     REFUSE_IF(!AT || !B || !C);
@@ -222,8 +222,11 @@
     if ((at_off & 1) || (b_off & 1) || (col_off & 1) || at_off + (K - 1) * ldat + round_up(M, 2) > (int64_t)at_rows * ldat ||
         b_off + (K - 1) * ldb + N > (int64_t)b_rows * ldb || row_off + M > c_rows || col_off + N > ldc)
         return refuse(__func__, "window outside the buffers or misaligned");
+    for (int r = 0; crow && r < M; ++r)
+        if (crow[r] < 0 || crow[r] >= c_rows) return refuse(__func__, "row table entry outside C");
     const size_t a_n = (size_t)at_rows * ldat, b_n = (size_t)b_rows * ldb, c_n = (size_t)c_rows * ldc;
-    DevBuf<> dA, dB, dC, dC0, dD;
+    DevBuf<> dA, dB, dC, dC0, dD, drow;
+    if (crow) CFLX_TRY(stage(drow, M, crow));
     CFLX_TRY(stage(dA, a_n, AT));
     CFLX_TRY(stage(dB, b_n, B));
     CFLX_TRY(stage(dC, c_n));
@@ -239,7 +242,8 @@
     g.M = M; g.N = N; g.K = K;
     g.AT = dA.as<double>() + at_off; g.ldat = ldat;
     g.B = dB.as<double>() + b_off; g.ldb = ldb;
-    g.C = dC.as<double>() + c_at; g.ldc = ldc;
+    g.C = dC.as<double>() + (crow ? col_off : c_at); g.ldc = ldc;
+    g.crow = crow ? drow.as<int>() : nullptr;
     g.D = (in_place ? dC.as<double>() : dD.as<double>()) + c_at; g.ldd = ldc;
     g.alpha = alpha; g.beta = beta;
     CFLX_TRY(restore());
@@ -1033,7 +1037,7 @@
     const size_t a_n = (size_t)n_rows * n_cols;
     DevBuf<> dA, dtmp, da01, dplan, dgp, dgri, dgrit, digri;
     CFLX_TRY(stage(dA, a_n, A_inout));
-    CFLX_TRY(stage(dtmp, (size_t)v * n_cols));
+    CFLX_TRY(stage(dtmp, (size_t)2 * v * n_cols));
     CFLX_TRY(stage(da01, (size_t)v * n_cols));
     CFLX_TRY(stage<int>(dplan, 6 * (size_t)v + 8 + n_rows));
     CFLX_TRY(stage(dgp, v, pivot_rows));
@@ -1051,9 +1055,9 @@
     plan.rowsrc = pm;
     CFLX_TRY(launch_iota_gri(dgri.as<int>(), digri.as<int>(), n_rows, n_rows, 1, 0, 0));
     CFLX_TRY(launch_plan_moves(dgp.as<int>(), v, 1, 0, fnpr, n_rows, digri.as<int>(), plan, 0));
-    CFLX_TRY(launch_push_phase1(dA.as<double>(), n_cols, n_cols, 0, plan, v, dtmp.as<double>(), da01.as<double>(), n_cols, 0, 0));
-    CFLX_TRY(launch_push_phase2(dA.as<double>(), n_cols, n_cols, 0, plan, v, 0));
-    CFLX_TRY(launch_push_phase3(dA.as<double>(), n_cols, n_cols, 0, fnpr, plan, v, dtmp.as<double>(), 0));
+    CFLX_TRY(launch_push_phase1(dA.as<double>(), n_cols, n_cols, plan, v, da01.as<double>(), n_cols, 0, 0));
+    CFLX_TRY(launch_push_phase2(dA.as<double>(), n_cols, 0, n_cols, plan, v, dtmp.as<double>(), 0));
+    CFLX_TRY(launch_push_phase3(dA.as<double>(), n_cols, 0, n_cols, fnpr, plan, v, dtmp.as<double>(), 0));
     CFLX_TRY(launch_update_gri(dgri.as<int>(), dgrit.as<int>(), digri.as<int>(), plan.rowsrc, fnpr, n_rows, n_rows, 1, 0));
     CFLX_TRY(fetch(A_inout, dA.p, a_n));
     CFLX_TRY(fetch(gri_out, dgri.p, n_rows));
@@ -1062,17 +1066,15 @@
     return CFLX_OK;
 }
 
-int cflx_dbg_ozaki_gemm(int M, int N, int K, int row0, int col0, int max_ctas, const double* AT, const double* B,
-                        const double* C, double* D, signed char* planesA_out, signed char* planesB_out, int* ea_out,
-                        int* eb_out, int reps, double* ms_out, double* split_ms_out) {
-    CFLX_TRY(check_device());
-    REFUSE_IF(M <= 0 || N <= 0 || K <= 0 || (N & 1));
-    REFUSE_IF(row0 < 0 || col0 < 0 || max_ctas < 0);
-    REFUSE_IF(!AT || !B);
+namespace {
+int ozaki_window(int M, int N, int K, int row0, int col0, int max_ctas, const double* AT, const double* B, const double* C,
+                 int c_rows, int c_off, const int* crow, double* D, signed char* planesA_out, signed char* planesB_out,
+                 int* ea_out, int* eb_out, int reps, double* ms_out, double* split_ms_out) {
     const int Ma = row0 + M, Nb = col0 + N;
     const int64_t ldat = round_up(Ma, 2), ldb = Nb, ldc = N;
-    const size_t c_n = (size_t)M * ldc;
-    DevBuf<> dA, dB, dC, dC0;
+    const size_t c_n = (size_t)c_rows * ldc;
+    DevBuf<> dA, dB, dC, dC0, drow;
+    if (crow) CFLX_TRY(stage(drow, M, crow));
     CFLX_TRY(stage(dA, K * ldat));
     CFLX_TRY(stage(dB, K * ldb, B));
     CFLX_TRY(stage(dC, c_n));
@@ -1093,7 +1095,8 @@
         if (!rc && col0 > 0) rc = ozaki_split_b(&ws, dB.as<double>(), ldb, 0, col0, 0);
         if (!rc) rc = ozaki_split_b(&ws, dB.as<double>(), ldb, col0, N, 0);
         cudaEventRecord(ev[1]);
-        if (!rc) rc = launch_ozaki_gemm(&ws, M, N, row0, col0, dC.as<double>(), ldc, max_ctas, 0);
+        if (!rc) rc = launch_ozaki_gemm(&ws, M, N, row0, col0, dC.as<double>() + (int64_t)c_off * ldc, ldc, dC.as<double>(),
+                                            crow ? drow.as<int>() : nullptr, max_ctas, 0);
         cudaEventRecord(ev[2]);
         if (cudaEventSynchronize(ev[2]) != cudaSuccess) {
             set_last_error("ozaki kernel failed: %s", cudaGetErrorString(cudaGetLastError()));
@@ -1120,6 +1123,30 @@
     if (split_ms_out) *split_ms_out = ms_split / reps;
     return rc;
 }
+}
+
+int cflx_dbg_ozaki_gemm(int M, int N, int K, int row0, int col0, int max_ctas, const double* AT, const double* B,
+                        const double* C, double* D, signed char* planesA_out, signed char* planesB_out, int* ea_out,
+                        int* eb_out, int reps, double* ms_out, double* split_ms_out) {
+    CFLX_TRY(check_device());
+    REFUSE_IF(M <= 0 || N <= 0 || K <= 0 || (N & 1));
+    REFUSE_IF(row0 < 0 || col0 < 0 || max_ctas < 0);
+    REFUSE_IF(!AT || !B);
+    return ozaki_window(M, N, K, row0, col0, max_ctas, AT, B, C, M, 0, nullptr, D, planesA_out, planesB_out, ea_out,
+                        eb_out, reps, ms_out, split_ms_out);
+}
+
+int cflx_dbg_ozaki_gemm_rows(int M, int N, int K, const double* AT, const double* B, const double* C, int c_rows,
+                             int c_off, const int* crow, double* D) {
+    CFLX_TRY(check_device());
+    REFUSE_IF(M <= 0 || N <= 0 || K <= 0 || (N & 1));
+    REFUSE_IF(!AT || !B || !C || !D);
+    REFUSE_IF(c_off < 0 || c_off + M > c_rows);
+    for (int r = 0; crow && r < M; ++r)
+        if (crow[r] < 0 || crow[r] >= c_rows) return refuse(__func__, "row table entry outside C");
+    return ozaki_window(M, N, K, 0, 0, 0, AT, B, C, c_rows, c_off, crow, D, nullptr, nullptr, nullptr, nullptr, 1, nullptr,
+                        nullptr);
+}
 
 int cflx_dbg_wgmma_peak(int n, double* tmacs_out) {
     CFLX_TRY(check_device());
diff --git a/conflux_b200/csrc/gemm.cu b/conflux_b200/csrc/gemm.cu
--- a/conflux_b200/csrc/gemm.cu
+++ b/conflux_b200/csrc/gemm.cu
@@ -24,6 +24,8 @@
     asm("ld.global.v2.f64 {%0, %1}, [%2];" : "=d"(v.x), "=d"(v.y) : "l"(p));
     return v;
 }
+
+__device__ __forceinline__ int64_t c_row(const GemmArgs& g, int r) { return (int64_t)(g.crow ? g.crow[r] : r) * g.ldc; }
 
 template <int LDA, int LDB, int SA, int SB>
 __device__ __forceinline__ void load_operands(const GemmArgs& g, int kt0, int kt1, int m0, int n0, int wm, int wn,
@@ -122,6 +124,12 @@
         const int rr = lane & 15;
         const int nkt = (g.K + BK - 1) / BK;
         const bool use_c = (g.beta != 0.0);
+        int64_t coff[STAGES];
+#pragma unroll
+        for (int i = 0; i < STAGES; ++i) {
+            const int r = m0 + 64 * (lane >> 4) + 16 * i + rr;
+            coff[i] = (C::STAGE_C && use_c && r < g.M) ? c_row(g, r) : 0;
+        }
         for (int kt = 0; kt < nkt; ++kt) {
             const int s = kt % STAGES, u = kt / STAGES;
             if (u > 0) mbar_wait(&empty[s], (u - 1) & 1);
@@ -148,7 +156,7 @@
                     __syncwarp();
                     if (rr < rows)
                         bulk_g2s(sA + (wr * STAGES + s) * BK * LDA + rr * LDA + 4 * (rr & 1),
-                                 g.C + (int64_t)(r0 + rr) * g.ldc + n0, (uint32_t)(wn * sizeof(double)), bar);
+                                 g.C + coff[i] + n0, (uint32_t)(wn * sizeof(double)), bar);
                 }
         }
         return;
@@ -224,12 +232,13 @@
 #pragma unroll
         for (int sl = 0; sl < 8; ++sl) {
             const int row = row0 + 8 * sl;
+            const double* crow = (use_c && row < g.M) ? g.C + c_row(g, row) : nullptr;
             double2 cv[4];
 #pragma unroll
             for (int j = 0; j < 4; ++j) {
                 const int col = col0 + 8 * j;
                 cv[j] = make_double2(0.0, 0.0);
-                if (use_c && row < g.M && col < g.N) cv[j] = ld_c2(g.C + (int64_t)row * g.ldc + col);
+                if (crow && col < g.N) cv[j] = ld_c2(crow + col);
             }
 #pragma unroll
             for (int j = 0; j < 4; ++j) {
@@ -254,9 +263,10 @@
     static constexpr int NSLAB = BM / 16, SLAB = 16 * LDC, STAGE = BK * (LDA + LDB);
     static constexpr int NBAR = 2 * STAGES + NSLAB;
     static constexpr int SMEM_MAX = 227 * 1024;
-    static constexpr int RING_OFF = (SMEM_MAX - NBAR * 8 - STAGES * STAGE * 8) / 128 * 128;
+    static constexpr int RING_OFF = (SMEM_MAX - NBAR * 8 - BM * 4 - STAGES * STAGE * 8) / 128 * 128;
     static constexpr int BAR_OFF = RING_OFF + STAGES * STAGE * 8;
-    static constexpr int SMEM = BAR_OFF + NBAR * 8;
+    static constexpr int ROWS_OFF = BAR_OFF + NBAR * 8;
+    static constexpr int SMEM = ROWS_OFF + BM * 4;
     __host__ __device__ static constexpr uint32_t slab_stages(int j) {
         uint32_t m = 0;
         for (int s = 0; s < STAGES; ++s) {
@@ -287,6 +297,7 @@
     uint64_t* full = reinterpret_cast<uint64_t*>(smem_raw + W::BAR_OFF);
     uint64_t* empty = full + STAGES;
     uint64_t* cfull = empty + STAGES;
+    int* crows = reinterpret_cast<int*>(smem_raw + W::ROWS_OFF);
 
     const int warp = threadIdx.x >> 5, lane = threadIdx.x & 31;
     const int m0 = blockIdx.y * W::BM, n0 = blockIdx.x * W::BN;
@@ -317,6 +328,9 @@
                                                               lane);
             return;
         }
+        for (int i = lane; i < W::BM; i += 32)
+            crows[i] = m0 + i < g.M ? (g.crow ? g.crow[m0 + i] : m0 + i) : 0;
+        __syncwarp();
         uint32_t drained = ~0u << min(nkt, STAGES), issued = 0;
         auto issue_ready = [&] {
 #pragma unroll 1
@@ -327,7 +341,7 @@
                 if (lane == 0) mbar_arrive_expect_tx(&cfull[j], (uint32_t)(rows * wn * sizeof(double)));
                 __syncwarp();
                 if (lane < rows)
-                    bulk_g2s(ctile + j * W::SLAB + lane * W::LDC + 4 * (lane & 1), g.C + (int64_t)(r0 + lane) * g.ldc + n0,
+                    bulk_g2s(ctile + j * W::SLAB + lane * W::LDC + 4 * (lane & 1), g.C + (int64_t)crows[16 * j + lane] * g.ldc + n0,
                              (uint32_t)(wn * sizeof(double)), &cfull[j]);
             }
         };
diff --git a/conflux_b200/csrc/kernels.h b/conflux_b200/csrc/kernels.h
--- a/conflux_b200/csrc/kernels.h
+++ b/conflux_b200/csrc/kernels.h
@@ -16,6 +16,7 @@
     int64_t ldb;
     const double* C;
     int64_t ldc;
+    const int* crow;
     double* D;
     int64_t ldd;
     double alpha, beta;
@@ -38,7 +39,8 @@
 int ozaki_split_a(OzakiWorkspace* ws, const double* LT, int64_t ld, int n, cudaStream_t s);
 int ozaki_split_b(OzakiWorkspace* ws, const double* U, int64_t ld, int col0, int n, cudaStream_t s);
 int wgmma_peak_probe(int n, double* tmacs_out);
-int launch_ozaki_gemm(OzakiWorkspace* ws, int M, int N, int row0, int col0, double* C, int64_t ldc, int max_ctas, cudaStream_t s);
+int launch_ozaki_gemm(OzakiWorkspace* ws, int M, int N, int row0, int col0, double* C, int64_t ldc, const double* cbase,
+                      const int* crow, int max_ctas, cudaStream_t s);
 
 struct PanelWorkspace {
     DevBuf<uint2> slot_hdr;
@@ -78,10 +80,11 @@
 };
 int launch_plan_moves(const int* gpivots, int v, int Px, int pi, int fnpr, int Ml, const int* igri, MovePlan plan,
                       cudaStream_t stream);
-int launch_push_phase1(const double* A, int64_t lda, int ncols, int col_lo, MovePlan plan, int v, double* tmp,
-                       double* a01raw, int64_t ld01, int c0, cudaStream_t stream);
-int launch_push_phase2(double* A, int64_t lda, int ncols, int col_lo, MovePlan plan, int v, cudaStream_t stream);
-int launch_push_phase3(double* A, int64_t lda, int ncols, int col_lo, int fnpr, MovePlan plan, int v,
+int launch_push_phase1(const double* A, int64_t lda, int ncols, MovePlan plan, int v, double* a01raw, int64_t ld01, int c0,
+                       cudaStream_t stream);
+int launch_push_phase2(const double* A, int64_t lda, int col_lo, int col_hi, MovePlan plan, int v, double* tmp,
+                       cudaStream_t stream);
+int launch_push_phase3(double* A, int64_t lda, int col_lo, int col_hi, int fnpr, MovePlan plan, int v,
                        const double* tmp, cudaStream_t stream);
 int launch_update_gri(int* gri, int* gri_tmp, int* igri, const int* rowsrc, int fnpr, int Ml, int v, int Px,
                       cudaStream_t stream);
diff --git a/conflux_b200/csrc/lu.cu b/conflux_b200/csrc/lu.cu
--- a/conflux_b200/csrc/lu.cu
+++ b/conflux_b200/csrc/lu.cu
@@ -282,9 +282,10 @@
     const int64_t ldk = std::max<int64_t>(2, round_up(n_old, 2));
     int nR = 0;
     while ((1 << nR) < Px) ++nR;
+    const bool direct = (nR == 0) && (Pz == 1) && !lu->fixed;
     {
         PhaseTimer t(lu, RG_step0_copy, s);
-        CFLX_TRY(launch_extract_panel_T(lu->A11, Nl, fnpr, loff, n_old, v, lu->PT, ldk, s));
+        CFLX_TRY(launch_extract_panel_T(lu->A11, Nl, fnpr, loff, n_old, v, direct ? lu->W : lu->PT, ldk, s));
         lu->launches++;
     }
     if (Pz > 1 && n_old > 0) {
@@ -294,7 +295,7 @@
     if (pk != 0) return CFLX_OK;
     if (lu->fixed) return fixed_panel(lu, k, fnpr, n_old, ldk, A00, A00T, s);
     int my_half = 0;
-    {
+    if (!direct) {
         PhaseTimer t(lu, RG_step1_A10copy, s);
         CFLX_CUDA(cudaMemcpyAsync(lu->W, lu->PT, (size_t)v * ldk * sizeof(double), cudaMemcpyDeviceToDevice, s));
     }
@@ -316,7 +317,8 @@
         if (first_partner > Px - 1) first_partner = Px - 1;
         my_half = first_partner < pi ? 1 : 0;
         CFLX_TRY(launch_gather_winners(lu->PT, ldk, lu->gri + fnpr, n_old, lu->perm, v,
-                                       lu->candH + (size_t)my_half * v * v, v, lu->tagsH + my_half * v, 0, s));
+                                       direct ? nullptr : lu->candH + (size_t)my_half * v * v, v, lu->tagsH + my_half * v,
+                                       0, s));
         lu->launches++;
     }
     PhaseTimer t(lu, RG_step1_pivoting, s);
@@ -368,15 +370,16 @@
     g.ldat = ld2;
     g.B = lu->U + (int64_t)lu->pk * lu->nlayr * ldu + u_col_off;
     g.ldb = ldu;
-    g.C = lu->A11 + (int64_t)fnpr * lu->Nl + col_lo;
+    g.C = lu->A11 + col_lo;
     g.ldc = lu->Nl;
+    g.crow = lu->plan.rowsrc + fnpr;
     g.D = lu->A11 + (int64_t)fnpr * lu->Nl + col_lo;
     g.ldd = lu->Nl;
     g.alpha = -1.0;
     g.beta = 1.0;
     const int e = 4 * k + 2 * part;
     if (lu->time_gemm) CFLX_CUDA(cudaEventRecord(lu->ev[e], s));
-    if (lu->use_ozaki) CFLX_TRY(launch_ozaki_gemm(&lu->oz, g.M, g.N, 0, u_col_off, g.D, g.ldd, max_ctas, s));
+    if (lu->use_ozaki) CFLX_TRY(launch_ozaki_gemm(&lu->oz, g.M, g.N, 0, u_col_off, g.D, g.ldd, g.C, g.crow, max_ctas, s));
     else CFLX_TRY(launch_gemm_tn(g, s));
     if (lu->time_gemm) CFLX_CUDA(cudaEventRecord(lu->ev[e + 1], s));
     lu->ev_used[e / 2] = lu->time_gemm;
@@ -417,6 +420,8 @@
         CFLX_TRY(launch_record_pivots(lu->gpivots, v, lu->hist, k, s));
         lu->launches++;
     }
+    const int move_lo = layer0 ? 0 : loff;
+    const int move_hi = (on_col && layer0) ? loff : c0;
     {
         PhaseTimer t(lu, RG_step2_pushingpivots, s);
         CFLX_TRY(launch_plan_moves(lu->gpivots, v, Px, pi, fnpr_old, Ml, lu->igri, lu->plan, s));
@@ -425,14 +430,9 @@
             CFLX_CUDA(cudaMemcpyAsync(lu->h_npiv, lu->plan.npiv, sizeof(int), cudaMemcpyDeviceToHost, s));
             CFLX_CUDA(cudaEventRecord(lu->ev_npiv, s));
         }
-        const int col_lo = layer0 ? 0 : loff;
-        const int64_t ldu0 = std::max(2, ncols);
-        CFLX_TRY(launch_push_phase1(lu->A11, Nl, Nl, col_lo, lu->plan, v, lu->tmp, ncols > 0 ? lu->A01raw.p : nullptr, ldu0,
-                                    c0, s));
-        CFLX_TRY(launch_push_phase2(lu->A11, Nl, Nl, col_lo, lu->plan, v, s));
-        CFLX_TRY(launch_push_phase3(lu->A11, Nl, Nl, col_lo, fnpr_old, lu->plan, v, lu->tmp, s));
+        CFLX_TRY(launch_push_phase1(lu->A11, Nl, Nl, lu->plan, v, ncols > 0 ? lu->A01raw.p : nullptr, ncols, c0, s));
         CFLX_TRY(launch_update_gri(lu->gri, lu->gri_tmp, lu->igri, lu->plan.rowsrc, fnpr_old, Ml, v, Px, s));
-        lu->launches += 5;
+        lu->launches += 3;
     }
     const int64_t ldu = std::max(2, ncols);
     const bool fused_l = (nR == 0) && !lu->fixed;
@@ -469,7 +469,13 @@
         }
         return CFLX_OK;
     };
-    if (!split_u) CFLX_TRY(store_factors());
+    auto move_rows = [&]() -> int {
+        PhaseTimer t(lu, RG_step2_pushingpivots, s);
+        CFLX_TRY(launch_push_phase2(lu->A11, Nl, move_lo, move_hi, lu->plan, v, lu->tmp, s));
+        CFLX_TRY(launch_push_phase3(lu->A11, Nl, move_lo, move_hi, fnpr_old, lu->plan, v, lu->tmp, s));
+        lu->launches += 2;
+        return CFLX_OK;
+    };
     int npiv = v;
     if (lu->fixed) {
         npiv = lu->fix_npiv[k];
@@ -523,13 +529,16 @@
             CFLX_TRY(trsm_left_lower_unit(A00T, lu->LinvT, v, lu->nb, lu->A01raw + v, lu->U + v, ldu, ncols - v, s));
             lu->launches += 2 * (v / lu->nb) - 1;
         }
-        if (split_u) CFLX_TRY(store_factors());
         if (split_u && n_act > 0) CFLX_TRY(ozaki_planes_b(lu, w, ncols - w, ldu, s));
         const int leave = (side && lu->use_ozaki) ? lu->pws.cta_cap : 0;
         CFLX_TRY(trailing_gemm(lu, k, 1, fnpr, n_act, c0 + w, ncols - w, ld2, ldu, w, s, leave > 0 ? lu->oz.sms - leave : 0));
+        CFLX_TRY(store_factors());
+        CFLX_TRY(move_rows());
         if (side) CFLX_CUDA(cudaStreamWaitEvent(s, lu->ev_join, 0));
     } else {
         CFLX_TRY(trailing_gemm(lu, k, 0, fnpr, n_act, c0, ncols, ld2, ldu, 0, s));
+        CFLX_TRY(store_factors());
+        CFLX_TRY(move_rows());
     }
     return CFLX_OK;
 }
@@ -858,7 +867,7 @@
     lu->ldp_max = ldp;
     const size_t pan = (size_t)v * ldp, upan = (size_t)v * (lu->Nl + 2), vv = (size_t)v * v;
     CFLX_TRY(lu->PT.alloc(pan)); CFLX_TRY(lu->PT2.alloc(pan)); CFLX_TRY(lu->W.alloc(pan)); CFLX_TRY(lu->LT.alloc(pan));
-    CFLX_TRY(lu->A01raw.alloc(upan)); CFLX_TRY(lu->U.alloc(upan)); CFLX_TRY(lu->tmp.alloc((size_t)v * lu->Nl));
+    CFLX_TRY(lu->A01raw.alloc(upan)); CFLX_TRY(lu->U.alloc(upan)); CFLX_TRY(lu->tmp.alloc((size_t)2 * v * lu->Nl));
     CFLX_TRY(lu->A00.alloc(2 * vv)); CFLX_TRY(lu->A00T.alloc(2 * vv)); CFLX_TRY(lu->Uinv.alloc(vv));
     CFLX_TRY(lu->LinvT.alloc(vv)); CFLX_TRY(lu->candH.alloc(2 * vv)); CFLX_TRY(lu->S.alloc(2 * vv));
     CFLX_TRY(lu->W2.alloc(2 * vv)); CFLX_TRY(lu->bcast.alloc(vv + v));
diff --git a/conflux_b200/csrc/ozaki.cu b/conflux_b200/csrc/ozaki.cu
--- a/conflux_b200/csrc/ozaki.cu
+++ b/conflux_b200/csrc/ozaki.cu
@@ -91,6 +91,8 @@
     int b_row0;
     double* C;
     int64_t ldc;
+    const double* cbase;
+    const int* crow;
     const int* ea;
     const int* eb;
     int tiles_m, tiles_n;
@@ -205,15 +207,16 @@
             const int row = r0 + 8 * h;
             if (row >= g.M) continue;
             const double sr = -pow2i(g.ea[g.a_row0 + row] - 12);
-            double* crow = g.C + (int64_t)row * g.ldc;
+            double* drow = g.C + (int64_t)row * g.ldc;
+            const double* srow = g.crow ? g.cbase + (int64_t)g.crow[row] * g.ldc : drow;
 #pragma unroll
             for (int j = 0; j < 8; ++j) {
                 const int col = n0 + 8 * j + 2 * (lane & 3);
                 if (col >= g.N) continue;
-                double2 c = *reinterpret_cast<const double2*>(crow + col);
+                double2 c = *reinterpret_cast<const double2*>(srow + col);
                 c.x += (sum[4 * j + 2 * h] * sr) * pow2i(g.eb[g.b_row0 + col]);
                 c.y += (sum[4 * j + 2 * h + 1] * sr) * pow2i(g.eb[g.b_row0 + col + 1]);
-                *reinterpret_cast<double2*>(crow + col) = c;
+                *reinterpret_cast<double2*>(drow + col) = c;
             }
         }
     }
@@ -408,7 +411,8 @@
     CFLX_CUDA(cudaGetLastError());
     return CFLX_OK;
 }
-int launch_ozaki_gemm(OzakiWorkspace* ws, int M, int N, int row0, int col0, double* C, int64_t ldc, int max_ctas, cudaStream_t s) {
+int launch_ozaki_gemm(OzakiWorkspace* ws, int M, int N, int row0, int col0, double* C, int64_t ldc, const double* cbase,
+                      const int* crow, int max_ctas, cudaStream_t s) {
     if (M <= 0 || N <= 0) return CFLX_OK;
     if ((N & 1) || (ldc & 1) || col0 < 0 || row0 < 0 || row0 + M > ws->cap_a || col0 + N > ws->cap_b) {
         set_last_error("ozaki_gemm: unsupported window M=%d N=%d row0=%d col0=%d ldc=%lld", M, N, row0, col0, (long long)ldc);
@@ -419,6 +423,8 @@
     g.a_row0 = row0;
     g.b_row0 = col0;
     g.C = C; g.ldc = ldc;
+    g.cbase = cbase;
+    g.crow = crow;
     g.ea = ws->ea; g.eb = ws->eb;
     g.tiles_m = (M + OZ_BM - 1) / OZ_BM;
     g.tiles_n = (N + OZ_BN - 1) / OZ_BN;
diff --git a/conflux_b200/csrc/rows.cu b/conflux_b200/csrc/rows.cu
--- a/conflux_b200/csrc/rows.cu
+++ b/conflux_b200/csrc/rows.cu
@@ -43,7 +43,7 @@
     if (e >= (int64_t)v * v) return;
     const int c = (int)(e / v), i = (int)(e % v);
     const int src = perm[i];
-    out[(int64_t)c * ldo + dst0 + i] = src < n_valid ? PT[(int64_t)c * ldp + src] : 0.0;
+    if (out) out[(int64_t)c * ldo + dst0 + i] = src < n_valid ? PT[(int64_t)c * ldp + src] : 0.0;
     if (c == 0) out_tags[dst0 + i] = src < n_valid ? tags[src] : 0;
 }
 __global__ void gather_a00_kernel(const double* __restrict__ W, int64_t ldw, const int* __restrict__ perm, int v, int nb,
@@ -131,41 +131,36 @@
     double2* d2 = reinterpret_cast<double2*>(dst);
     for (int i = b + threadIdx.x; i < e; i += blockDim.x) d2[i] = s2[i];
 }
-__global__ void push_phase1_kernel(const double* __restrict__ A, int64_t lda, int ncols, int col_lo, MovePlan plan, int v,
-                                   double* __restrict__ tmp, double* __restrict__ a01raw, int64_t ld01, int c0) {
-    const int npiv = plan.npiv[0];
+__global__ void push_phase1_kernel(const double* __restrict__ A, int64_t lda, int ncols, MovePlan plan,
+                                   double* __restrict__ a01raw, int64_t ld01, int c0) {
+    if (a01raw == nullptr) return;
+    const int slot = blockIdx.y;
+    const int p = plan.slot2piv[slot];
+    const int len = ncols - c0;
+    double* dst = a01raw + (int64_t)slot * ld01;
+    if (p >= 0) {
+        copy_row_seg(dst, A + (int64_t)plan.cur_piv[p] * lda + c0, len, blockIdx.x, gridDim.x);
+    } else {
+        const int n2 = len >> 1;
+        const int per = (n2 + gridDim.x - 1) / gridDim.x;
+        const int b = blockIdx.x * per, e = min(n2, b + per);
+        double2* d2 = reinterpret_cast<double2*>(dst);
+        for (int i = b + threadIdx.x; i < e; i += blockDim.x) d2[i] = make_double2(0.0, 0.0);
+    }
+}
+__global__ void push_phase2_kernel(const double* __restrict__ A, int64_t lda, int col_lo, int col_hi, MovePlan plan, int v,
+                                   double* __restrict__ tmp) {
     const int y = blockIdx.y;
-    if (y < v) {
-        if (y >= npiv) return;
-        const int src = plan.cur_piv[y];
-        copy_row_seg(tmp + (int64_t)y * lda + col_lo, A + (int64_t)src * lda + col_lo, ncols - col_lo, blockIdx.x,
-                     gridDim.x);
-    } else if (a01raw != nullptr) {
-        const int slot = y - v;
-        const int p = plan.slot2piv[slot];
-        const int len = ncols - c0;
-        double* dst = a01raw + (int64_t)slot * ld01;
-        if (p >= 0) {
-            copy_row_seg(dst, A + (int64_t)plan.cur_piv[p] * lda + c0, len, blockIdx.x, gridDim.x);
-        } else {
-            const int n2 = len >> 1;
-            const int per = (n2 + gridDim.x - 1) / gridDim.x;
-            const int b = blockIdx.x * per, e = min(n2, b + per);
-            double2* d2 = reinterpret_cast<double2*>(dst);
-            for (int i = b + threadIdx.x; i < e; i += blockDim.x) d2[i] = make_double2(0.0, 0.0);
-        }
-    }
-}
-__global__ void push_phase2_kernel(double* __restrict__ A, int64_t lda, int ncols, int col_lo, MovePlan plan) {
-    if ((int)blockIdx.y >= plan.nel[0]) return;
-    const int src = plan.early[blockIdx.y], dst = plan.late[blockIdx.y];
-    copy_row_seg(A + (int64_t)dst * lda + col_lo, A + (int64_t)src * lda + col_lo, ncols - col_lo, blockIdx.x, gridDim.x);
-}
-__global__ void push_phase3_kernel(double* __restrict__ A, int64_t lda, int ncols, int col_lo, int fnpr, MovePlan plan,
-                                   const double* __restrict__ tmp) {
-    if ((int)blockIdx.y >= plan.npiv[0]) return;
-    copy_row_seg(A + (int64_t)(fnpr + blockIdx.y) * lda + col_lo, tmp + (int64_t)blockIdx.y * lda + col_lo, ncols - col_lo,
-                 blockIdx.x, gridDim.x);
+    if (y < v ? y >= plan.npiv[0] : y - v >= plan.nel[0]) return;
+    const int src = y < v ? plan.cur_piv[y] : plan.early[y - v];
+    copy_row_seg(tmp + (int64_t)y * lda + col_lo, A + (int64_t)src * lda + col_lo, col_hi - col_lo, blockIdx.x, gridDim.x);
+}
+__global__ void push_phase3_kernel(double* __restrict__ A, int64_t lda, int col_lo, int col_hi, int fnpr, MovePlan plan,
+                                   int v, const double* __restrict__ tmp) {
+    const int y = blockIdx.y;
+    if (y < v ? y >= plan.npiv[0] : y - v >= plan.nel[0]) return;
+    const int dst = y < v ? fnpr + y : plan.late[y - v];
+    copy_row_seg(A + (int64_t)dst * lda + col_lo, tmp + (int64_t)y * lda + col_lo, col_hi - col_lo, blockIdx.x, gridDim.x);
 }
 
 __global__ void gri_gather_kernel(const int* __restrict__ gri, int* __restrict__ gri_tmp, const int* __restrict__ rowsrc,
@@ -312,7 +307,7 @@
 }
 int launch_gather_winners(const double* PT, int64_t ldp, const int* tags, int n_valid, const int* perm, int v,
                           double* out_vals, int64_t ldo, int* out_tags, int dst0, cudaStream_t s) {
-    const int64_t tot = (int64_t)v * v;
+    const int64_t tot = out_vals ? (int64_t)v * v : v;
     gather_winners_kernel<<<(unsigned)((tot + 255) / 256), 256, 0, s>>>(PT, ldp, tags, n_valid, perm, v, out_vals, ldo,
                                                                         out_tags, dst0);
     POST_LAUNCH();
@@ -328,21 +323,22 @@
     plan_moves_kernel<<<1, 256, 2 * v * sizeof(int), s>>>(gpivots, v, Px, pi, fnpr, Ml, igri, plan);
     POST_LAUNCH();
 }
-int launch_push_phase1(const double* A, int64_t lda, int ncols, int col_lo, MovePlan plan, int v, double* tmp,
-                       double* a01raw, int64_t ld01, int c0, cudaStream_t s) {
-    dim3 grid(row_chunks(ncols), a01raw ? 2 * v : v);
-    push_phase1_kernel<<<grid, 256, 0, s>>>(A, lda, ncols, col_lo, plan, v, tmp, a01raw, ld01, c0);
-    POST_LAUNCH();
-}
-int launch_push_phase2(double* A, int64_t lda, int ncols, int col_lo, MovePlan plan, int v, cudaStream_t s) {
-    dim3 grid(row_chunks(ncols), v);
-    push_phase2_kernel<<<grid, 256, 0, s>>>(A, lda, ncols, col_lo, plan);
-    POST_LAUNCH();
-}
-int launch_push_phase3(double* A, int64_t lda, int ncols, int col_lo, int fnpr, MovePlan plan, int v, const double* tmp,
+int launch_push_phase1(const double* A, int64_t lda, int ncols, MovePlan plan, int v, double* a01raw, int64_t ld01, int c0,
                        cudaStream_t s) {
-    dim3 grid(row_chunks(ncols), v);
-    push_phase3_kernel<<<grid, 256, 0, s>>>(A, lda, ncols, col_lo, fnpr, plan, tmp);
+    dim3 grid(row_chunks(a01raw ? ncols - c0 : 0), v);
+    push_phase1_kernel<<<grid, 256, 0, s>>>(A, lda, ncols, plan, a01raw, ld01, c0);
+    POST_LAUNCH();
+}
+int launch_push_phase2(const double* A, int64_t lda, int col_lo, int col_hi, MovePlan plan, int v, double* tmp,
+                       cudaStream_t s) {
+    dim3 grid(row_chunks(col_hi - col_lo), 2 * v);
+    push_phase2_kernel<<<grid, 256, 0, s>>>(A, lda, col_lo, col_hi, plan, v, tmp);
+    POST_LAUNCH();
+}
+int launch_push_phase3(double* A, int64_t lda, int col_lo, int col_hi, int fnpr, MovePlan plan, int v, const double* tmp,
+                       cudaStream_t s) {
+    dim3 grid(row_chunks(col_hi - col_lo), 2 * v);
+    push_phase3_kernel<<<grid, 256, 0, s>>>(A, lda, col_lo, col_hi, fnpr, plan, v, tmp);
     POST_LAUNCH();
 }
 int launch_update_gri(int* gri, int* gri_tmp, int* igri, const int* rowsrc, int fnpr, int Ml, int v, int Px,
diff --git a/include/conflux_b200.h b/include/conflux_b200.h
--- a/include/conflux_b200.h
+++ b/include/conflux_b200.h
@@ -125,8 +125,8 @@
 
 int cflx_dbg_gemm_tn(int M, int N, int K, const double* AT, int at_rows, int64_t ldat, int64_t at_off, const double* B,
                      int b_rows, int64_t ldb, int64_t b_off, const double* C, int c_rows, int64_t ldc, int row_off,
-                     int col_off, double alpha, double beta, int in_place, double* D_out, double* C_out, int reps,
-                     double* ms_out);
+                     int col_off, double alpha, double beta, int in_place, const int* crow, double* D_out, double* C_out,
+                     int reps, double* ms_out);
 int cflx_dbg_gemm_narrow(int M, int N, int K, const double* A, const double* B, const double* C, double alpha, double beta,
                          double* D, int reps, double* ms_out);
 int cflx_dbg_gemm_narrow_tn(int M, int N, int K, const double* AT, const double* B, const double* C, double alpha,
@@ -180,6 +180,8 @@
 int cflx_dbg_ozaki_gemm(int M, int N, int K, int row0, int col0, int max_ctas, const double* AT, const double* B,
                         const double* C, double* D, signed char* planesA_out, signed char* planesB_out, int* ea_out,
                         int* eb_out, int reps, double* ms_out, double* split_ms_out);
+int cflx_dbg_ozaki_gemm_rows(int M, int N, int K, const double* AT, const double* B, const double* C, int c_rows,
+                             int c_off, const int* crow, double* D);
 int cflx_dbg_wgmma_peak(int n, double* tmacs_out);
 int cflx_dbg_push_pivots(int n_rows, int n_cols, double* A_inout, int npiv, const int* pivot_rows, int fnpr, int* gri_out,
                          double* a01_out);
```

After: 27010, median of 6. +2.2%, better.
